# VISION-SJTU/UniDefense

Hardware: AMD Instinct MI355X
Metric: images/sec fwd+bwd (256x256, EffNet-b4) (higher is better)
Workload: dtype f32

## Files before the change

unidefense_amd/csrc/bnref.h:

```cpp
#pragma once
#include "colgeom.h"

namespace {

constexpr int NT = UD_COL_NT;

template <typename T> constexpr int kRowUnroll = sizeof(T) == 2 ? 8 : 4;

__device__ __forceinline__ void atomic_add_f64(double* p, double v) { unsafeAtomicAdd(p, v); }

struct Bn4 { f32x4 mu, is, ga, be; };

__device__ __forceinline__ Bn4 bn_load(const ud_bn_ref& b, int g, int C4, int c4, bool update) {
    Bn4 o;
    const long i0 = ((long)(b.G == 1 ? 0 : g) * C4 + c4) * 4;
#pragma unroll
    for (int e = 0; e < 4; ++e) {
        double m, v;
        ud_bn_moments(b, i0 + e, c4 * 4 + e, m, v);
        o.mu[e] = (float)m;
        o.is[e] = rsqrtf((float)(v + (double)b.eps));
        if (update && b.sum && b.running_mean) {
            const int c = c4 * 4 + e;
            b.running_mean[c] = (1.f - b.momentum) * b.running_mean[c] + b.momentum * (float)m;
            b.running_var[c] = (1.f - b.momentum) * b.running_var[c] + b.momentum * (float)(v * b.unbias);
        }
    }
    o.ga = reinterpret_cast<const f32x4*>(b.gamma)[c4];
    o.be = reinterpret_cast<const f32x4*>(b.beta)[c4];
    return o;
}

__device__ __forceinline__ f32x4 bn_apply(const f32x4& a, const Bn4& b, int act) {
    f32x4 o;
#pragma unroll
    for (int e = 0; e < 4; ++e) o[e] = ud_act_fast(b.ga[e] * ((a[e] - b.mu[e]) * b.is[e]) + b.be[e], act);
    return o;
}

__device__ __forceinline__ float gate_factor(const float* alpha, int mode) {
    if (mode == 0 || !alpha) return 1.f;
    const float a = ud_sigmoid(alpha[0]);
    return mode == 1 ? a : 1.f - a;
}

__global__ __launch_bounds__(NT) void partials_to_acc(int nq, int G, int C, int P, const double* __restrict__ part,
                                                      double* __restrict__ a1, double* __restrict__ a2) {
    __shared__ double sm[2][NT];
    const int cl = threadIdx.x & 7, pl = threadIdx.x >> 3;
    const int idx = blockIdx.x * 8 + cl;
    const bool ok = idx < G * C;
    const long plane = (long)G * P * C;
    double a = 0.0, b = 0.0;
    if (ok) {
        const int g = idx / C, c = idx % C;
        const long base = (long)g * P * C + c, step = 32L * C;
        int p = pl;
        for (; p + 96 < P; p += 128) {
            const long o = base + (long)p * C;
            a += (part[o] + part[o + step]) + (part[o + 2 * step] + part[o + 3 * step]);
            if (nq == 2) b += (part[plane + o] + part[plane + o + step]) + (part[plane + o + 2 * step] + part[plane + o + 3 * step]);
        }
        for (; p < P; p += 32) {
            const long o = base + (long)p * C;
            a += part[o];
            if (nq == 2) b += part[plane + o];
        }
    }
    sm[0][threadIdx.x] = a;
    sm[1][threadIdx.x] = b;
    __syncthreads();
    if (ok && pl == 0) {
        for (int k = 1; k < 32; ++k) {
            a += sm[0][k * 8 + cl];
            b += sm[1][k * 8 + cl];
        }
        a1[idx] += a;
        if (nq == 2) a2[idx] += b;
    }
}

}
```

unidefense_amd/csrc/fft.hip:

```cpp
#include "ud_common.h"

#include <stdlib.h>

#include <type_traits>

namespace {

constexpr int NT = 512;

__device__ __forceinline__ float gate_factor_f(const float* alpha, int mode) {
    if (mode == 0 || !alpha) return 1.f;
    const float a = ud_sigmoid(alpha[0]);
    return mode == 1 ? a : 1.f - a;
}

__device__ constexpr float TW_RE[32] = {
    1.000000000e+00f, 9.951847267e-01f, 9.807852804e-01f, 9.569403357e-01f, 9.238795325e-01f, 8.819212643e-01f,
    8.314696123e-01f, 7.730104534e-01f, 7.071067812e-01f, 6.343932842e-01f, 5.555702330e-01f, 4.713967368e-01f,
    3.826834324e-01f, 2.902846773e-01f, 1.950903220e-01f, 9.801714033e-02f, 0.0f, -9.801714033e-02f,
    -1.950903220e-01f, -2.902846773e-01f, -3.826834324e-01f, -4.713967368e-01f, -5.555702330e-01f, -6.343932842e-01f,
    -7.071067812e-01f, -7.730104534e-01f, -8.314696123e-01f, -8.819212643e-01f, -9.238795325e-01f, -9.569403357e-01f,
    -9.807852804e-01f, -9.951847267e-01f};
__device__ constexpr float TW_IM[32] = {
    0.0f, -9.801714033e-02f, -1.950903220e-01f, -2.902846773e-01f, -3.826834324e-01f, -4.713967368e-01f,
    -5.555702330e-01f, -6.343932842e-01f, -7.071067812e-01f, -7.730104534e-01f, -8.314696123e-01f, -8.819212643e-01f,
    -9.238795325e-01f, -9.569403357e-01f, -9.807852804e-01f, -9.951847267e-01f, -1.000000000e+00f, -9.951847267e-01f,
    -9.807852804e-01f, -9.569403357e-01f, -9.238795325e-01f, -8.819212643e-01f, -8.314696123e-01f, -7.730104534e-01f,
    -7.071067812e-01f, -6.343932842e-01f, -5.555702330e-01f, -4.713967368e-01f, -3.826834324e-01f, -2.902846773e-01f,
    -1.950903220e-01f, -9.801714033e-02f};

template <int S>
__device__ __forceinline__ constexpr int brev2(int i) {
    int r = 0;
    for (int b = 1; b < S; b <<= 1) {
        r = (r << 1) | (i & 1);
        i >>= 1;
    }
    return r;
}

__device__ constexpr float TW80_RE[80] = {
    1.000000000e+00f, 9.969173337e-01f, 9.876883406e-01f, 9.723699204e-01f, 9.510565163e-01f, 9.238795325e-01f,
    8.910065242e-01f, 8.526401644e-01f, 8.090169944e-01f, 7.604059656e-01f, 7.071067812e-01f, 6.494480483e-01f,
    5.877852523e-01f, 5.224985647e-01f, 4.539904997e-01f, 3.826834324e-01f, 3.090169944e-01f, 2.334453639e-01f,
    1.564344650e-01f, 7.845909573e-02f, 6.123233996e-17f, -7.845909573e-02f, -1.564344650e-01f, -2.334453639e-01f,
    -3.090169944e-01f, -3.826834324e-01f, -4.539904997e-01f, -5.224985647e-01f, -5.877852523e-01f, -6.494480483e-01f,
    -7.071067812e-01f, -7.604059656e-01f, -8.090169944e-01f, -8.526401644e-01f, -8.910065242e-01f, -9.238795325e-01f,
    -9.510565163e-01f, -9.723699204e-01f, -9.876883406e-01f, -9.969173337e-01f, -1.000000000e+00f, -9.969173337e-01f,
    -9.876883406e-01f, -9.723699204e-01f, -9.510565163e-01f, -9.238795325e-01f, -8.910065242e-01f, -8.526401644e-01f,
    -8.090169944e-01f, -7.604059656e-01f, -7.071067812e-01f, -6.494480483e-01f, -5.877852523e-01f, -5.224985647e-01f,
    -4.539904997e-01f, -3.826834324e-01f, -3.090169944e-01f, -2.334453639e-01f, -1.564344650e-01f, -7.845909573e-02f,
    -1.836970199e-16f, 7.845909573e-02f, 1.564344650e-01f, 2.334453639e-01f, 3.090169944e-01f, 3.826834324e-01f,
    4.539904997e-01f, 5.224985647e-01f, 5.877852523e-01f, 6.494480483e-01f, 7.071067812e-01f, 7.604059656e-01f,
    8.090169944e-01f, 8.526401644e-01f, 8.910065242e-01f, 9.238795325e-01f, 9.510565163e-01f, 9.723699204e-01f,
    9.876883406e-01f, 9.969173337e-01f};
__device__ constexpr float TW80_IM[80] = {
    -0.000000000e+00f, -7.845909573e-02f, -1.564344650e-01f, -2.334453639e-01f, -3.090169944e-01f, -3.826834324e-01f,
    -4.539904997e-01f, -5.224985647e-01f, -5.877852523e-01f, -6.494480483e-01f, -7.071067812e-01f, -7.604059656e-01f,
    -8.090169944e-01f, -8.526401644e-01f, -8.910065242e-01f, -9.238795325e-01f, -9.510565163e-01f, -9.723699204e-01f,
    -9.876883406e-01f, -9.969173337e-01f, -1.000000000e+00f, -9.969173337e-01f, -9.876883406e-01f, -9.723699204e-01f,
    -9.510565163e-01f, -9.238795325e-01f, -8.910065242e-01f, -8.526401644e-01f, -8.090169944e-01f, -7.604059656e-01f,
    -7.071067812e-01f, -6.494480483e-01f, -5.877852523e-01f, -5.224985647e-01f, -4.539904997e-01f, -3.826834324e-01f,
    -3.090169944e-01f, -2.334453639e-01f, -1.564344650e-01f, -7.845909573e-02f, -1.224646799e-16f, 7.845909573e-02f,
    1.564344650e-01f, 2.334453639e-01f, 3.090169944e-01f, 3.826834324e-01f, 4.539904997e-01f, 5.224985647e-01f,
    5.877852523e-01f, 6.494480483e-01f, 7.071067812e-01f, 7.604059656e-01f, 8.090169944e-01f, 8.526401644e-01f,
    8.910065242e-01f, 9.238795325e-01f, 9.510565163e-01f, 9.723699204e-01f, 9.876883406e-01f, 9.969173337e-01f,
    1.000000000e+00f, 9.969173337e-01f, 9.876883406e-01f, 9.723699204e-01f, 9.510565163e-01f, 9.238795325e-01f,
    8.910065242e-01f, 8.526401644e-01f, 8.090169944e-01f, 7.604059656e-01f, 7.071067812e-01f, 6.494480483e-01f,
    5.877852523e-01f, 5.224985647e-01f, 4.539904997e-01f, 3.826834324e-01f, 3.090169944e-01f, 2.334453639e-01f,
    1.564344650e-01f, 7.845909573e-02f};

__device__ constexpr float TW48_RE[48] = {
    1.000000000e+00f, 9.914448614e-01f, 9.659258263e-01f, 9.238795325e-01f, 8.660254038e-01f, 7.933533403e-01f,
    7.071067812e-01f, 6.087614290e-01f, 5.000000000e-01f, 3.826834324e-01f, 2.588190451e-01f, 1.305261922e-01f,
    6.123233996e-17f, -1.305261922e-01f, -2.588190451e-01f, -3.826834324e-01f, -5.000000000e-01f, -6.087614290e-01f,
    -7.071067812e-01f, -7.933533403e-01f, -8.660254038e-01f, -9.238795325e-01f, -9.659258263e-01f, -9.914448614e-01f,
    -1.000000000e+00f, -9.914448614e-01f, -9.659258263e-01f, -9.238795325e-01f, -8.660254038e-01f, -7.933533403e-01f,
    -7.071067812e-01f, -6.087614290e-01f, -5.000000000e-01f, -3.826834324e-01f, -2.588190451e-01f, -1.305261922e-01f,
    -1.836970199e-16f, 1.305261922e-01f, 2.588190451e-01f, 3.826834324e-01f, 5.000000000e-01f, 6.087614290e-01f,
    7.071067812e-01f, 7.933533403e-01f, 8.660254038e-01f, 9.238795325e-01f, 9.659258263e-01f, 9.914448614e-01f};
__device__ constexpr float TW48_IM[48] = {
    -0.000000000e+00f, -1.305261922e-01f, -2.588190451e-01f, -3.826834324e-01f, -5.000000000e-01f, -6.087614290e-01f,
    -7.071067812e-01f, -7.933533403e-01f, -8.660254038e-01f, -9.238795325e-01f, -9.659258263e-01f, -9.914448614e-01f,
    -1.000000000e+00f, -9.914448614e-01f, -9.659258263e-01f, -9.238795325e-01f, -8.660254038e-01f, -7.933533403e-01f,
    -7.071067812e-01f, -6.087614290e-01f, -5.000000000e-01f, -3.826834324e-01f, -2.588190451e-01f, -1.305261922e-01f,
    -1.224646799e-16f, 1.305261922e-01f, 2.588190451e-01f, 3.826834324e-01f, 5.000000000e-01f, 6.087614290e-01f,
    7.071067812e-01f, 7.933533403e-01f, 8.660254038e-01f, 9.238795325e-01f, 9.659258263e-01f, 9.914448614e-01f,
    1.000000000e+00f, 9.914448614e-01f, 9.659258263e-01f, 9.238795325e-01f, 8.660254038e-01f, 7.933533403e-01f,
    7.071067812e-01f, 6.087614290e-01f, 5.000000000e-01f, 3.826834324e-01f, 2.588190451e-01f, 1.305261922e-01f};

template <int S>
struct Radix {
    static constexpr int R = (S % 5 == 0) ? 5 : (S % 3 == 0) ? 3 : 1;
    static constexpr bool MIXED = R > 1;
    static constexpr int P = S / R;
    static constexpr int L = R == 5 ? 80 : 48;
};
template <int S> __device__ __forceinline__ constexpr float tw_re(int m) { return Radix<S>::R == 5 ? TW80_RE[m] : TW48_RE[m]; }
template <int S> __device__ __forceinline__ constexpr float tw_im(int m) { return Radix<S>::R == 5 ? TW80_IM[m] : TW48_IM[m]; }

template <int S>
__device__ __forceinline__ constexpr int brev(int i) {
    if (Radix<S>::MIXED) return (i % Radix<S>::R) * Radix<S>::P + brev2<Radix<S>::P>(i / Radix<S>::R);
    return brev2<S>(i);
}

template <int S, int P, int OFF, bool INV>
__device__ __forceinline__ void fft_pow2(float (&re)[S], float (&im)[S]) {
#pragma unroll
    for (int len = 2; len <= P; len <<= 1) {
        const int hl = len >> 1;
        const int tstep = 64 / len;
#pragma unroll
        for (int i = 0; i < P; i += len) {
#pragma unroll
            for (int j = 0; j < hl; ++j) {
                const float wr = TW_RE[j * tstep];
                const float wi = INV ? -TW_IM[j * tstep] : TW_IM[j * tstep];
                const float xr = re[OFF + i + j + hl], xi = im[OFF + i + j + hl];
                const float tr = wr * xr - wi * xi;
                const float ti = wr * xi + wi * xr;
                const float ur = re[OFF + i + j], ui = im[OFF + i + j];
                re[OFF + i + j] = ur + tr;
                im[OFF + i + j] = ui + ti;
                re[OFF + i + j + hl] = ur - tr;
                im[OFF + i + j + hl] = ui - ti;
            }
        }
    }
}

template <int S, int P, int RR, bool INV>
struct SubFfts {
    static __device__ __forceinline__ void run(float (&re)[S], float (&im)[S]) {
        SubFfts<S, P, RR - 1, INV>::run(re, im);
        fft_pow2<S, P, (RR - 1) * P, INV>(re, im);
    }
};
template <int S, int P, bool INV>
struct SubFfts<S, P, 0, INV> {
    static __device__ __forceinline__ void run(float (&)[S], float (&)[S]) {}
};

template <int S, bool INV>
__device__ __forceinline__ void fft_inreg(float (&re)[S], float (&im)[S]) {
    constexpr int P = Radix<S>::P, R = Radix<S>::R, L = Radix<S>::L;
    if constexpr (!Radix<S>::MIXED) {
        fft_pow2<S, P, 0, INV>(re, im);
    } else {
        SubFfts<S, P, R, INV>::run(re, im);
        constexpr int TS = L / S;
#pragma unroll
        for (int k2 = 0; k2 < P; ++k2) {
            float yr[R], yi[R];
#pragma unroll
            for (int r = 0; r < R; ++r) {
                const int m = (r * k2 * TS) % L;
                const float wr = tw_re<S>(m), wi = INV ? -tw_im<S>(m) : tw_im<S>(m);
                const float xr = re[r * P + k2], xi = im[r * P + k2];
                yr[r] = wr * xr - wi * xi;
                yi[r] = wr * xi + wi * xr;
            }
#pragma unroll
            for (int k1 = 0; k1 < R; ++k1) {
                float ar = yr[0], ai = yi[0];
#pragma unroll
                for (int r = 1; r < R; ++r) {
                    const int m = ((L / R) * r * k1) % L;
                    const float wr = tw_re<S>(m), wi = INV ? -tw_im<S>(m) : tw_im<S>(m);
                    ar += wr * yr[r] - wi * yi[r];
                    ai += wr * yi[r] + wi * yr[r];
                }
                re[k1 * P + k2] = ar;
                im[k1 * P + k2] = ai;
            }
        }
    }
}

__device__ __forceinline__ void work_item(int xcd_remap, int& cgroup, int& n) {
    const int ngroups = gridDim.x;
    if (!xcd_remap) {
        cgroup = blockIdx.x;
        n = blockIdx.y;
        return;
    }
    const int W = gridDim.x * gridDim.y, L = blockIdx.y * gridDim.x + blockIdx.x;
    const int q = W >> 3, r = W & 7, xcd = L & 7;
    const int w = (xcd < r ? xcd * (q + 1) : r * (q + 1) + (xcd - r) * q) + (L >> 3);
    cgroup = w % ngroups;
    n = w / ngroups;
}

template <int S, int CB>
struct Lds {
    static constexpr int WH = S / 2 + 1;
    static constexpr int KSTRIDE = S * CB + (CB < 32 ? CB : 0);
    static constexpr int PLANE = WH * KSTRIDE;
    static constexpr size_t BYTES = 2ull * PLANE * sizeof(float);
};

struct PlanesOut {
    uint16_t* buf;
    long panel, plane;
    float* inv_scale;
    float pre;
    const double* energy;
};

struct DwOut {
    const float* wt;
    void* out;
};

template <typename T, int S, int CB, bool EX, int DW = 0>
__global__ __launch_bounds__(NT) void rfft2_kernel(const T* __restrict__ x, T* __restrict__ Y, int C,
                                                   float scale, float w_int, ud_bn_ref bn, int has_bn,
                                                   T* __restrict__ act_out, const float* __restrict__ gate_alpha,
                                                   int gate_mode, const double* __restrict__ gate_acc,
                                                   float* __restrict__ gate_grad, int xcd_remap,
                                                   uint32_t* __restrict__ amax, PlanesOut po, DwOut dwo) {
    using L = Lds<S, CB>;
    static_assert(DW == 0 || (size_t)S * S * CB * sizeof(float) <= L::BYTES, "the activated plane fits the transform's LDS planes");
    __shared__ float po_red[NT / 64];
    const bool po_raw = po.pre < 0.f;
    if (EX && po.buf && !po_raw) {
        float gm = 0.f;
        for (int i = threadIdx.x; i < C; i += NT) {
            if (po.energy) gm = fmaxf(gm, (float)po.energy[i]);
            else gm = fmaxf(gm, bn.gamma[i] * bn.gamma[i] + bn.beta[i] * bn.beta[i]);
        }
        gm = ud_wave_max(gm);
        if ((threadIdx.x & 63) == 0) po_red[threadIdx.x >> 6] = gm;
    }
    if (EX && gate_grad && blockIdx.x == 0 && blockIdx.y == 0 && threadIdx.x < 64) {
        const double tot = ud_wave_sum_d(gate_acc[threadIdx.x]);
        if (threadIdx.x == 0) {
            const double a = 1.0 / (1.0 + exp(-(double)gate_alpha[0]));
            gate_grad[0] = (float)(tot * a * (1.0 - a));
        }
    }
    extern __shared__ __attribute__((aligned(16))) float lds[];
    float* Lre = lds;
    float* Lim = lds + L::PLANE;
    const int t = threadIdx.x;
    const int c = t % CB, q = t / CB;
    int cgroup, n;
    work_item(xcd_remap, cgroup, n);
    const int ch = cgroup * CB + c;
    const bool cok = ch < C;
    float re[S], im[S];
    float va[DW ? S : 1];
    if (q < S) {
        const int chl = cok ? ch : C - 1;
        const T* src = x + (((long)n * S + q) * S) * C + chl;
#pragma unroll
        for (int w = 0; w < S; ++w) re[brev<S>(w)] = (float)src[(long)w * C];
        float mu = 0.f, is = 1.f, ga = 1.f, be = 0.f;
        if (EX && has_bn) {
            double m, vv;
            ud_bn_moments(bn, chl, chl, m, vv);
            mu = (float)m;
            is = (float)(1.0 / sqrt(vv + (double)bn.eps));
            ga = bn.gamma[chl];
            be = bn.beta[chl];
            if (n == 0 && q == 0 && cok && bn.sum && bn.running_mean) {
                bn.running_mean[ch] = (1.f - bn.momentum) * bn.running_mean[ch] + bn.momentum * (float)m;
                bn.running_var[ch] = (1.f - bn.momentum) * bn.running_var[ch] + bn.momentum * (float)(vv * bn.unbias);
            }
        }
        T* aout = (EX && act_out) ? act_out + (((long)n * S + q) * S) * C + ch : nullptr;
#pragma unroll
        for (int w = 0; w < S; ++w) {
            float v = re[brev<S>(w)];
            if (EX && has_bn) {
                v = ud_rounded<T>(ud_act(ga * ((v - mu) * is) + be, bn.act));
                if (aout && cok) aout[(long)w * C] = (T)v;
            }
            re[brev<S>(w)] = cok ? v : 0.f;
            im[brev<S>(w)] = 0.f;
            if (DW) va[w] = cok ? v : 0.f;
        }
        fft_inreg<S, false>(re, im);
#pragma unroll
        for (int kx = 0; kx <= S / 2; ++kx) {
            Lre[kx * L::KSTRIDE + q * CB + c] = re[kx];
            Lim[kx * L::KSTRIDE + q * CB + c] = im[kx];
        }
    }
    __syncthreads();
    float mabs = 0.f;
    if (q <= S / 2 && cok) {
#pragma unroll
        for (int h = 0; h < S; ++h) {
            re[brev<S>(h)] = Lre[q * L::KSTRIDE + h * CB + c];
            im[brev<S>(h)] = Lim[q * L::KSTRIDE + h * CB + c];
        }
        fft_inreg<S, false>(re, im);
        float f = (q == 0 || q == S / 2) ? scale : scale * w_int;
        float gf = 1.f;
        if (EX && gate_mode != 0) {
            const float a = ud_sigmoid(gate_alpha[0]);
            gf = (gate_mode == 1) ? a : 1.f - a;
            f *= gf;
        }
        if (EX && po.buf) {
            float ps = 1.f, pinv = 1.f;
            if (!po_raw) {
                float gm = po_red[0];
#pragma unroll
                for (int i = 1; i < NT / 64; ++i) gm = fmaxf(gm, po_red[i]);
                ud_h2_scale(__float_as_uint(po.pre * gf * sqrtf(gm) * 1.002f), ps, pinv);
            }
            if (blockIdx.x == 0 && blockIdx.y == 0 && q == 0 && c == 0) *po.inv_scale = pinv;
            f *= ps;
            const long row0 = ((long)n * S) * L::WH + q;
            const int cim = C + ch;
            uint16_t* pre_ = po.buf + (long)(ch >> 5) * po.panel + row0 * 32 + (ch & 31);
            uint16_t* pim_ = po.buf + (long)(cim >> 5) * po.panel + row0 * 32 + (cim & 31);
#pragma unroll
            for (int ky = 0; ky < S; ++ky) {
                const long o = (long)ky * L::WH * 32;
                if (po_raw) {
                    pre_[o] = __builtin_bit_cast(uint16_t, (_Float16)(re[ky] * f));
                    pim_[o] = __builtin_bit_cast(uint16_t, (_Float16)(im[ky] * f));
                    continue;
                }
                uint16_t a0, a1, b0, b1;
                ud_split_h2(re[ky] * f, a0, a1);
                ud_split_h2(im[ky] * f, b0, b1);
                pre_[o] = a0;
                pre_[o + po.plane] = a1;
                pim_[o] = b0;
                pim_[o + po.plane] = b1;
            }
        } else {
            T* dst = Y + (((long)n * S) * L::WH + q) * (2L * C) + ch;
#pragma unroll
            for (int ky = 0; ky < S; ++ky) {
                dst[(long)ky * L::WH * 2 * C] = (T)(re[ky] * f);
                dst[(long)ky * L::WH * 2 * C + C] = (T)(im[ky] * f);
                if (EX) mabs = fmaxf(mabs, fmaxf(fabsf(re[ky] * f), fabsf(im[ky] * f)));
            }
        }
    }
    if (EX) ud_absmax_commit(mabs, amax);
    if constexpr (DW != 0) {
        constexpr int P = (DW - 1) / 2;
        __syncthreads();
        float* A = lds;
        if (q < S) {
#pragma unroll
            for (int w = 0; w < S; ++w) A[(q * S + w) * CB + c] = va[w];
        }
        __syncthreads();
        if (q < S && cok) {
            float tp[DW * DW];
#pragma unroll
            for (int i = 0; i < DW * DW; ++i) tp[i] = dwo.wt[(long)i * C + ch];
            float acc[S];
#pragma unroll
            for (int w = 0; w < S; ++w) acc[w] = 0.f;
#pragma unroll
            for (int i = 0; i < DW; ++i) {
                const int ih = q + i - P;
                if (ih < 0 || ih >= S) continue;
                float in[S + DW - 1];
#pragma unroll
                for (int j = 0; j < S + DW - 1; ++j) in[j] = (j >= P && j < S + P) ? A[(ih * S + j - P) * CB + c] : 0.f;
#pragma unroll
                for (int w = 0; w < S; ++w)
#pragma unroll
                    for (int j = 0; j < DW; ++j) acc[w] += in[w + j] * tp[i * DW + j];
            }
            T* o = reinterpret_cast<T*>(dwo.out) + (((long)n * S + q) * S) * C + ch;
#pragma unroll
            for (int w = 0; w < S; ++w) o[(long)w * C] = (T)acc[w];
        }
    }
}

template <typename T, int S, int CB, bool MIX>
__global__ __launch_bounds__(NT) void irfft2_kernel(const T* __restrict__ Y, T* __restrict__ x, int C,
                                                    float scale, float w_int, const T* __restrict__ spat,
                                                    const float* __restrict__ alpha, T* __restrict__ freq_out,
                                                    double* __restrict__ sum, double* __restrict__ sumsq, int xcd_remap) {
    using L = Lds<S, CB>;
    extern __shared__ __attribute__((aligned(16))) float lds[];
    float* Lre = lds;
    float* Lim = lds + L::PLANE;
    const int t = threadIdx.x;
    const int c = t % CB, q = t / CB;
    int cgroup, n;
    work_item(xcd_remap, cgroup, n);
    const int ch = cgroup * CB + c;
    const bool cok = ch < C;
    float re[S], im[S];
    constexpr int NHELP = S - (S / 2 + 1);
    if (q > S / 2 && q < S) {
        const int kx = q - (S / 2 + 1);
        const T* src = Y + (((long)n * S) * L::WH + kx) * (2L * C) + ch + C;
#pragma unroll
        for (int ky = 0; ky < S; ++ky) re[ky] = cok ? (float)src[(long)ky * L::WH * 2 * C] : 0.f;
#pragma unroll
        for (int ky = 0; ky < S; ++ky) Lim[kx * L::KSTRIDE + ky * CB + c] = re[ky];
    } else if (q <= S / 2) {
        const T* src = Y + (((long)n * S) * L::WH + q) * (2L * C) + ch;
#pragma unroll
        for (int ky = 0; ky < S; ++ky) re[brev<S>(ky)] = cok ? (float)src[(long)ky * L::WH * 2 * C] : 0.f;
        if (q >= NHELP) {
#pragma unroll
            for (int ky = 0; ky < S; ++ky) im[brev<S>(ky)] = cok ? (float)src[(long)ky * L::WH * 2 * C + C] : 0.f;
        }
    }
    __syncthreads();
    if (q <= S / 2) {
        const float f = (q == 0 || q == S / 2) ? 1.f : w_int;
        if (q < NHELP) {
#pragma unroll
            for (int ky = 0; ky < S; ++ky) im[brev<S>(ky)] = Lim[q * L::KSTRIDE + ky * CB + c];
        }
#pragma unroll
        for (int k = 0; k < S; ++k) {
            re[k] *= f;
            im[k] *= f;
        }
        fft_inreg<S, true>(re, im);
#pragma unroll
        for (int h = 0; h < S; ++h) {
            Lre[q * L::KSTRIDE + h * CB + c] = re[h];
            Lim[q * L::KSTRIDE + h * CB + c] = im[h];
        }
    }
    __syncthreads();
    double tot1 = 0.0, tot2 = 0.0;
    if (cok && q < S) {
#pragma unroll
        for (int kx = 0; kx <= S / 2; ++kx) {
            const float zr = Lre[kx * L::KSTRIDE + q * CB + c];
            const float zi = Lim[kx * L::KSTRIDE + q * CB + c];
            re[brev<S>(kx)] = zr;
            im[brev<S>(kx)] = (kx == 0 || kx == S / 2) ? 0.f : zi;
            if (kx > 0 && kx < S / 2) {
                re[brev<S>(S - kx)] = zr;
                im[brev<S>(S - kx)] = -zi;
            }
        }
        fft_inreg<S, true>(re, im);
        const long o0 = (((long)n * S + q) * S) * C + ch;
        T* dst = x + o0;
        if (!MIX) {
#pragma unroll
            for (int w = 0; w < S; ++w) dst[(long)w * C] = (T)(re[w] * scale);
        } else {
            const float a = ud_sigmoid(alpha[0]);
            const T* sp = spat + o0;
            T* fo = freq_out + o0;
#pragma unroll
            for (int w = 0; w < S; ++w) {
                const float fr = re[w] * scale, spv = (float)sp[(long)w * C];
                const float y = ud_rounded<T>(spv * (1.f - a) + fr * a);
                fo[(long)w * C] = (T)(fr - spv);
                dst[(long)w * C] = (T)y;
                tot1 += (double)y;
                tot2 += (double)y * (double)y;
            }
        }
    }
    if (MIX && sum) {
        __syncthreads();
        double* red = reinterpret_cast<double*>(lds);
        const bool own = cok && q < S;
        if (own) {
            red[(q * CB + c) * 2] = tot1;
            red[(q * CB + c) * 2 + 1] = tot2;
        }
        __syncthreads();
        if (cok && q == 0) {
            double t1 = 0.0, t2 = 0.0;
            for (int r = 0; r < S; ++r) {
                t1 += red[(r * CB + c) * 2];
                t2 += red[(r * CB + c) * 2 + 1];
            }
            unsafeAtomicAdd(sum + ch, t1);
            unsafeAtomicAdd(sumsq + ch, t2);
        }
    }
}

inline int xcd_remap_on(int run_bytes) {
    return run_bytes < 128;
}

template <int S, int CB, int K>
struct LdsBwd {
    using L = Lds<S, CB>;
    static constexpr size_t PLANES = 2ull * S * S * CB * sizeof(float);
    static constexpr size_t FOLD = (size_t)S * K * K * CB * sizeof(float);
    static constexpr size_t BYTES = L::BYTES > PLANES ? (L::BYTES > FOLD ? L::BYTES : FOLD) : (PLANES > FOLD ? PLANES : FOLD);
};

template <typename T, int S, int CB, int K>
__global__ __launch_bounds__(NT, 4) void irfft2_dwbwd_kernel(const T* __restrict__ Y, int C, float scale, float w_int,
                                                         const T* __restrict__ dd, const T* __restrict__ x,
                                                         ud_bn_ref bn, const float* __restrict__ wt,
                                                         const float* __restrict__ gate_alpha, int gate_mode,
                                                         T* __restrict__ dz, double* __restrict__ s1,
                                                         double* __restrict__ s2, double* __restrict__ s3,
                                                         float* __restrict__ wpart, int xcd_remap) {
    using L = Lds<S, CB>;
    static_assert(S * CB == NT, "one row-thread per (h, c)");
    constexpr int P = (K - 1) / 2;
    extern __shared__ __attribute__((aligned(16))) float lds[];
    float* Lre = lds;
    float* Lim = lds + L::PLANE;
    const int t = threadIdx.x;
    const int c = t % CB, q = t / CB;
    int cgroup, n;
    work_item(xcd_remap, cgroup, n);
    const int ch = cgroup * CB + c;
    const bool cok = ch < C;
    const int chl = cok ? ch : C - 1;
    float re[S], im[S];
    constexpr int NHELP = S - (S / 2 + 1);
    if (q > S / 2) {
        const int kx = q - (S / 2 + 1);
        const T* src = Y + (((long)n * S) * L::WH + kx) * (2L * C) + chl + C;
#pragma unroll
        for (int ky = 0; ky < S; ++ky) re[ky] = cok ? (float)src[(long)ky * L::WH * 2 * C] : 0.f;
#pragma unroll
        for (int ky = 0; ky < S; ++ky) Lim[kx * L::KSTRIDE + ky * CB + c] = re[ky];
    } else {
        const T* src = Y + (((long)n * S) * L::WH + q) * (2L * C) + chl;
#pragma unroll
        for (int ky = 0; ky < S; ++ky) re[brev<S>(ky)] = cok ? (float)src[(long)ky * L::WH * 2 * C] : 0.f;
        if (q >= NHELP) {
#pragma unroll
            for (int ky = 0; ky < S; ++ky) im[brev<S>(ky)] = cok ? (float)src[(long)ky * L::WH * 2 * C + C] : 0.f;
        }
    }
    float ddr[S], er[S];
    {
        const long o = (((long)n * S + q) * S) * C + chl;
#pragma unroll
        for (int w = 0; w < S; ++w) {
            ddr[w] = (float)dd[o + (long)w * C];
            er[w] = (float)x[o + (long)w * C];
        }
    }
    __syncthreads();
    if (q <= S / 2) {
        const float f = (q == 0 || q == S / 2) ? 1.f : w_int;
        if (q < NHELP) {
#pragma unroll
            for (int ky = 0; ky < S; ++ky) im[brev<S>(ky)] = Lim[q * L::KSTRIDE + ky * CB + c];
        }
#pragma unroll
        for (int k = 0; k < S; ++k) {
            re[k] *= f;
            im[k] *= f;
        }
        fft_inreg<S, true>(re, im);
#pragma unroll
        for (int h = 0; h < S; ++h) {
            Lre[q * L::KSTRIDE + h * CB + c] = re[h];
            Lim[q * L::KSTRIDE + h * CB + c] = im[h];
        }
    }
    __syncthreads();
    {
#pragma unroll
        for (int kx = 0; kx <= S / 2; ++kx) {
            const float zr = Lre[kx * L::KSTRIDE + q * CB + c];
            const float zi = Lim[kx * L::KSTRIDE + q * CB + c];
            re[brev<S>(kx)] = zr;
            im[brev<S>(kx)] = (kx == 0 || kx == S / 2) ? 0.f : zi;
            if (kx > 0 && kx < S / 2) {
                re[brev<S>(S - kx)] = zr;
                im[brev<S>(S - kx)] = -zi;
            }
        }
        fft_inreg<S, true>(re, im);
    }
    float mu, is, ga, be;
    {
        double m, vv;
        ud_bn_moments(bn, chl, chl, m, vv);
        mu = (float)m;
        is = (float)(1.0 / sqrt(vv + (double)bn.eps));
        ga = bn.gamma[chl];
        be = bn.beta[chl];
    }
    __syncthreads();
    float* A = lds;
    float* D = lds + S * S * CB;
#pragma unroll
    for (int w = 0; w < S; ++w) {
        A[(q * S + w) * CB + c] = cok ? ud_act(ga * ((er[w] - mu) * is) + be, bn.act) : 0.f;
        D[(q * S + w) * CB + c] = cok ? ddr[w] : 0.f;
    }
    __syncthreads();
    float tp[K * K];
#pragma unroll
    for (int i = 0; i < K * K; ++i) tp[i] = wt[(long)i * C + chl];
    double v1 = 0.0, v2 = 0.0;
    float v3 = 0.f;
    {
        float acc[S];
#pragma unroll
        for (int w = 0; w < S; ++w) acc[w] = 0.f;
#pragma unroll
        for (int i = 0; i < K; ++i) {
            const int ih = q + i - P;
            if (ih < 0 || ih >= S) continue;
            float in[S + K - 1];
#pragma unroll
            for (int j = 0; j < S + K - 1; ++j) in[j] = (j >= P && j < S + P) ? D[(ih * S + j - P) * CB + c] : 0.f;
#pragma unroll
            for (int w = 0; w < S; ++w)
#pragma unroll
                for (int j = 0; j < K; ++j) acc[w] += in[w + j] * tp[K * K - 1 - (i * K + j)];
        }
        const float gs = gate_factor_f(gate_alpha, gate_mode);
        if (cok) {
            T* o = dz + (((long)n * S + q) * S) * C + ch;
#pragma unroll
            for (int w = 0; w < S; ++w) {
                const float xh = (er[w] - mu) * is;
                float d = acc[w] * gs + re[w] * scale;
                if (bn.act) d *= ud_act_grad_fast(ga * xh + be, bn.act);
                d = ud_rounded<T>(d);
                o[(long)w * C] = (T)d;
                v1 += (double)d;
                v2 += (double)d * (double)xh;
                v3 += d * d;
            }
        }
    }
    float accw[K * K];
#pragma unroll
    for (int i = 0; i < K * K; ++i) accw[i] = 0.f;
#pragma unroll
    for (int i = 0; i < K; ++i) {
        const int ih = q + i - P;
        if (ih < 0 || ih >= S) continue;
        float in[S + K - 1];
#pragma unroll
        for (int j = 0; j < S + K - 1; ++j) in[j] = (j >= P && j < S + P) ? A[(ih * S + j - P) * CB + c] : 0.f;
#pragma unroll
        for (int j = 0; j < K; ++j)
#pragma unroll
            for (int w = 0; w < S; ++w) accw[i * K + j] += in[w + j] * ddr[w];
    }
    __syncthreads();
    float* F = lds;
#pragma unroll
    for (int i = 0; i < K * K; ++i) F[(q * K * K + i) * CB + c] = cok ? accw[i] : 0.f;
    __syncthreads();
    for (int i = t; i < K * K * CB; i += NT) {
        const int tap = i / CB, cc = i % CB;
        float sum = 0.f;
#pragma unroll
        for (int r = 0; r < S; ++r) sum += F[(r * K * K + tap) * CB + cc];
        if (cgroup * CB + cc < C) wpart[((long)n * K * K + tap) * C + cgroup * CB + cc] = sum;
    }
    __syncthreads();
    double* red = reinterpret_cast<double*>(lds);
    red[(q * CB + c) * 3] = v1;
    red[(q * CB + c) * 3 + 1] = v2;
    red[(q * CB + c) * 3 + 2] = (double)v3 * 1.0001;
    __syncthreads();
    if (cok && q == 0) {
        double t1 = 0.0, t2 = 0.0, t3 = 0.0;
        for (int r = 0; r < S; ++r) {
            t1 += red[(r * CB + c) * 3];
            t2 += red[(r * CB + c) * 3 + 1];
            t3 += red[(r * CB + c) * 3 + 2];
        }
        unsafeAtomicAdd(s1 + ch, t1);
        unsafeAtomicAdd(s2 + ch, t2);
        if (s3) unsafeAtomicAdd(s3 + ch, t3);
    }
}

template <typename T, int S, int CB, int K>
int launch_irfft2_dwbwd(const T* Y, int N, int C, float scale, float w_int, const T* dd, const T* x,
                        const ud_bn_ref& bn, const float* wt, const float* gate_alpha, int gate_mode, T* dz, double* s1,
                        double* s2, double* s3, float* wpart, hipStream_t s) {
    using LB = LdsBwd<S, CB, K>;
    static bool attr_set = false;
    if (LB::BYTES > 65536 && !attr_set) {
        hipError_t e = hipFuncSetAttribute(reinterpret_cast<const void*>(&irfft2_dwbwd_kernel<T, S, CB, K>),
                                           hipFuncAttributeMaxDynamicSharedMemorySize, (int)LB::BYTES);
        if (e != hipSuccess) return -(int)e;
        attr_set = true;
    }
    dim3 grid((unsigned)ud_cdiv(C, CB), (unsigned)N);
    hipLaunchKernelGGL((irfft2_dwbwd_kernel<T, S, CB, K>), grid, dim3(NT), LB::BYTES, s, Y, C, scale, w_int, dd, x, bn, wt,
                       gate_alpha, gate_mode, dz, s1, s2, s3, wpart, xcd_remap_on(CB * (int)sizeof(float)));
    UD_LAUNCH_CHECK();
    return 0;
}

struct RfftEx {
    const ud_bn_ref* bn;
    void* act_out;
    const float* gate_alpha;
    int gate_mode;
    const double* gate_acc;
    float* gate_grad;
    uint32_t* absmax;
    PlanesOut planes = PlanesOut{nullptr, 0, 0, nullptr, 0.f, nullptr};
    DwOut dw = DwOut{nullptr, nullptr};
};

template <typename T, int S, int CB, bool EX, int DW = 0>
int launch_rfft2_t(const T* x, T* Y, int N, int C, float scale, float w_int, const RfftEx& ex, hipStream_t s) {
    using L = Lds<S, CB>;
    static bool attr_set = false;
    if (L::BYTES > 65536 && !attr_set) {
        hipError_t e = hipFuncSetAttribute(reinterpret_cast<const void*>(&rfft2_kernel<T, S, CB, EX, DW>),
                                           hipFuncAttributeMaxDynamicSharedMemorySize, (int)L::BYTES);
        if (e != hipSuccess) return -(int)e;
        attr_set = true;
    }
    dim3 grid((unsigned)ud_cdiv(C, CB), (unsigned)N);
    ud_bn_ref none{};
    hipLaunchKernelGGL((rfft2_kernel<T, S, CB, EX, DW>), grid, dim3(NT), L::BYTES, s, x, Y, C, scale, w_int,
                       ex.bn ? *ex.bn : none, ex.bn ? 1 : 0, (T*)ex.act_out, ex.gate_alpha, ex.gate_mode, ex.gate_acc,
                       ex.gate_grad, xcd_remap_on(CB * (int)sizeof(T)), ex.absmax, ex.planes, ex.dw);
    UD_LAUNCH_CHECK();
    return 0;
}

template <typename T, int S, int CB>
int launch_rfft2(const T* x, T* Y, int N, int C, float scale, float w_int, const RfftEx* ex, hipStream_t s) {
    if (ex) return launch_rfft2_t<T, S, CB, true>(x, Y, N, C, scale, w_int, *ex, s);
    return launch_rfft2_t<T, S, CB, false>(x, Y, N, C, scale, w_int, RfftEx{nullptr, nullptr, nullptr, 0, nullptr, nullptr, nullptr, PlanesOut{nullptr, 0, 0, nullptr, 0.f, nullptr}, DwOut{nullptr, nullptr}}, s);
}

struct IrfftMix {
    const void* spat;
    const float* alpha;
    void* freq_out;
    double* sum;
    double* sumsq;
};

template <typename T, int S, int CB, bool MIX>
int launch_irfft2_t(const T* Y, T* x, int N, int C, float scale, float w_int, const IrfftMix& m, hipStream_t s) {
    using L = Lds<S, CB>;
    static_assert(!MIX || L::BYTES >= (size_t)S * CB * 2 * sizeof(double), "LDS planes hold the row totals");
    static bool attr_set = false;
    if (L::BYTES > 65536 && !attr_set) {
        hipError_t e = hipFuncSetAttribute(reinterpret_cast<const void*>(&irfft2_kernel<T, S, CB, MIX>),
                                           hipFuncAttributeMaxDynamicSharedMemorySize, (int)L::BYTES);
        if (e != hipSuccess) return -(int)e;
        attr_set = true;
    }
    dim3 grid((unsigned)ud_cdiv(C, CB), (unsigned)N);
    hipLaunchKernelGGL((irfft2_kernel<T, S, CB, MIX>), grid, dim3(NT), L::BYTES, s, Y, x, C, scale, w_int,
                       (const T*)m.spat, m.alpha, (T*)m.freq_out, m.sum, m.sumsq, xcd_remap_on(CB * (int)sizeof(T)));
    UD_LAUNCH_CHECK();
    return 0;
}

template <typename T, int S, int CB>
int launch_irfft2(const T* Y, T* x, int N, int C, float scale, float w_int, const IrfftMix* m, hipStream_t s) {
    if (m) return launch_irfft2_t<T, S, CB, true>(Y, x, N, C, scale, w_int, *m, s);
    return launch_irfft2_t<T, S, CB, false>(Y, x, N, C, scale, w_int, IrfftMix{nullptr, nullptr, nullptr, nullptr, nullptr}, s);
}

constexpr int NT2 = 256;
constexpr int RPT = 4;

template <typename T, int S, bool EX>
__global__ __launch_bounds__(NT2) void rows_fwd_kernel(const T* __restrict__ x, float* __restrict__ Z, int C, ud_bn_ref bn,
                                                       int has_bn, T* __restrict__ act_out,
                                                       const float* __restrict__ gate_alpha,
                                                       const double* __restrict__ gate_acc, float* __restrict__ gate_grad) {
    constexpr int WH = S / 2 + 1;
    if (EX && gate_grad && blockIdx.x == 0 && blockIdx.y == 0 && blockIdx.z == 0 && threadIdx.x < 64) {
        const double tot = ud_wave_sum_d(gate_acc[threadIdx.x]);
        if (threadIdx.x == 0) {
            const double a = 1.0 / (1.0 + exp(-(double)gate_alpha[0]));
            gate_grad[0] = (float)(tot * a * (1.0 - a));
        }
    }
    const int ch = blockIdx.x * 64 + (threadIdx.x & 63);
    const int h = blockIdx.y * 4 + (threadIdx.x >> 6);
    const int n = blockIdx.z;
    if (ch >= C || h >= S) return;
    float mu = 0.f, is = 1.f, ga = 1.f, be = 0.f;
    if (EX && has_bn) {
        double m, vv;
        ud_bn_moments(bn, ch, ch, m, vv);
        mu = (float)m;
        is = (float)(1.0 / sqrt(vv + (double)bn.eps));
        ga = bn.gamma[ch];
        be = bn.beta[ch];
        if (n == 0 && h == 0 && bn.sum && bn.running_mean) {
            bn.running_mean[ch] = (1.f - bn.momentum) * bn.running_mean[ch] + bn.momentum * (float)m;
            bn.running_var[ch] = (1.f - bn.momentum) * bn.running_var[ch] + bn.momentum * (float)(vv * bn.unbias);
        }
    }
    const long o0 = (((long)n * S + h) * S) * C + ch;
    const T* src = x + o0;
    T* aout = (EX && act_out) ? act_out + o0 : nullptr;
    float re[S], im[S];
#pragma unroll
    for (int w = 0; w < S; ++w) re[brev<S>(w)] = (float)src[(long)w * C];
#pragma unroll
    for (int w = 0; w < S; ++w) {
        if (EX && has_bn) {
            const float v = ud_rounded<T>(ud_act(ga * ((re[brev<S>(w)] - mu) * is) + be, bn.act));
            if (aout) aout[(long)w * C] = (T)v;
            re[brev<S>(w)] = v;
        }
        im[brev<S>(w)] = 0.f;
    }
    fft_inreg<S, false>(re, im);
    float* dst = Z + (((long)n * S + h) * WH) * (2L * C) + ch;
#pragma unroll
    for (int kx = 0; kx <= S / 2; ++kx) {
        dst[(long)kx * 2 * C] = re[kx];
        dst[(long)kx * 2 * C + C] = im[kx];
    }
}

template <typename T, int S, bool EX>
__global__ __launch_bounds__(NT2) void cols_fwd_kernel(const float* __restrict__ Z, T* __restrict__ Y, int C, float scale,
                                                       float w_int, const float* __restrict__ gate_alpha, int gate_mode,
                                                       uint32_t* __restrict__ amax) {
    constexpr int WH = S / 2 + 1;
    const int ch = blockIdx.x * 64 + (threadIdx.x & 63);
    const int kx = blockIdx.y * 4 + (threadIdx.x >> 6);
    const int n = blockIdx.z;
    if (ch >= C || kx >= WH) {
        ud_absmax_commit(0.f, amax);
        return;
    }
    float mabs = 0.f;
    const float* src = Z + (((long)n * S) * WH + kx) * (2L * C) + ch;
    float re[S], im[S];
#pragma unroll
    for (int h = 0; h < S; ++h) {
        re[brev<S>(h)] = src[(long)h * WH * 2 * C];
        im[brev<S>(h)] = src[(long)h * WH * 2 * C + C];
    }
    fft_inreg<S, false>(re, im);
    float f = (kx == 0 || kx == S / 2) ? scale : scale * w_int;
    if (EX && gate_mode != 0) {
        const float a = ud_sigmoid(gate_alpha[0]);
        f *= (gate_mode == 1) ? a : 1.f - a;
    }
    T* dst = Y + (((long)n * S) * WH + kx) * (2L * C) + ch;
#pragma unroll
    for (int ky = 0; ky < S; ++ky) {
        dst[(long)ky * WH * 2 * C] = (T)(re[ky] * f);
        dst[(long)ky * WH * 2 * C + C] = (T)(im[ky] * f);
        mabs = fmaxf(mabs, fmaxf(fabsf(re[ky] * f), fabsf(im[ky] * f)));
    }
    ud_absmax_commit(mabs, amax);
}

template <typename T, int S>
__global__ __launch_bounds__(NT2) void cols_inv_kernel(const T* __restrict__ Y, float* __restrict__ Z, int C, float w_int) {
    constexpr int WH = S / 2 + 1;
    const int ch = blockIdx.x * 64 + (threadIdx.x & 63);
    const int kx = blockIdx.y * 4 + (threadIdx.x >> 6);
    const int n = blockIdx.z;
    if (ch >= C || kx >= WH) return;
    const T* src = Y + (((long)n * S) * WH + kx) * (2L * C) + ch;
    const float f = (kx == 0 || kx == S / 2) ? 1.f : w_int;
    float re[S], im[S];
#pragma unroll
    for (int ky = 0; ky < S; ++ky) {
        re[brev<S>(ky)] = (float)src[(long)ky * WH * 2 * C];
        im[brev<S>(ky)] = (float)src[(long)ky * WH * 2 * C + C];
    }
#pragma unroll
    for (int k = 0; k < S; ++k) {
        re[k] *= f;
        im[k] *= f;
    }
    fft_inreg<S, true>(re, im);
    float* dst = Z + (((long)n * S) * WH + kx) * (2L * C) + ch;
#pragma unroll
    for (int h = 0; h < S; ++h) {
        dst[(long)h * WH * 2 * C] = re[h];
        dst[(long)h * WH * 2 * C + C] = im[h];
    }
}

template <typename T, int S, bool MIX>
__global__ __launch_bounds__(NT2) void rows_inv_kernel(const float* __restrict__ Z, T* __restrict__ x, int C, float scale,
                                                       const T* __restrict__ spat, const float* __restrict__ alpha,
                                                       T* __restrict__ freq_out, double* __restrict__ sum,
                                                       double* __restrict__ sumsq) {
    constexpr int WH = S / 2 + 1;
    __shared__ double red[MIX ? 2 * NT2 : 1];
    const int lane = threadIdx.x & 63, rg = threadIdx.x >> 6;
    const int ch = blockIdx.x * 64 + lane;
    const int n = blockIdx.z;
    const bool cok = ch < C;
    double tot1 = 0.0, tot2 = 0.0;
    float a = 0.f;
    if (MIX) a = ud_sigmoid(alpha[0]);
    if (cok) {
#pragma unroll 1
        for (int r = 0; r < RPT; ++r) {
            const int h = (blockIdx.y * 4 + rg) * RPT + r;
            if (h >= S) break;
            const float* src = Z + (((long)n * S + h) * WH) * (2L * C) + ch;
            float re[S], im[S];
#pragma unroll
            for (int kx = 0; kx <= S / 2; ++kx) {
                const float zr = src[(long)kx * 2 * C];
                const float zi = src[(long)kx * 2 * C + C];
                re[brev<S>(kx)] = zr;
                im[brev<S>(kx)] = (kx == 0 || kx == S / 2) ? 0.f : zi;
                if (kx > 0 && kx < S / 2) {
                    re[brev<S>(S - kx)] = zr;
                    im[brev<S>(S - kx)] = -zi;
                }
            }
            fft_inreg<S, true>(re, im);
            const long o0 = (((long)n * S + h) * S) * C + ch;
            T* dst = x + o0;
            if (!MIX) {
#pragma unroll
                for (int w = 0; w < S; ++w) dst[(long)w * C] = (T)(re[w] * scale);
            } else {
                const T* sp = spat + o0;
                T* fo = freq_out + o0;
#pragma unroll
                for (int w = 0; w < S; ++w) {
                    const float fr = re[w] * scale, spv = (float)sp[(long)w * C];
                    const float y = ud_rounded<T>(spv * (1.f - a) + fr * a);
                    fo[(long)w * C] = (T)(fr - spv);
                    dst[(long)w * C] = (T)y;
                    tot1 += (double)y;
                    tot2 += (double)y * (double)y;
                }
            }
        }
    }
    if (MIX && sum) {
        red[threadIdx.x * 2] = tot1;
        red[threadIdx.x * 2 + 1] = tot2;
        __syncthreads();
        if (rg == 0 && cok) {
            double t1 = 0.0, t2 = 0.0;
#pragma unroll
            for (int g = 0; g < 4; ++g) {
                t1 += red[(g * 64 + lane) * 2];
                t2 += red[(g * 64 + lane) * 2 + 1];
            }
            unsafeAtomicAdd(sum + ch, t1);
            unsafeAtomicAdd(sumsq + ch, t2);
        }
    }
}

template <typename T, int S>
int rfft2_two_pass(const T* x, T* Y, float* Z, int N, int C, float scale, float w_int, const RfftEx* ex, hipStream_t s) {
    constexpr int WH = S / 2 + 1;
    const dim3 gr((unsigned)ud_cdiv(C, 64), (unsigned)(S / 4), (unsigned)N);
    const dim3 gc((unsigned)ud_cdiv(C, 64), (unsigned)ud_cdiv(WH, 4), (unsigned)N);
    ud_bn_ref none{};
    if (ex) {
        hipLaunchKernelGGL((rows_fwd_kernel<T, S, true>), gr, dim3(NT2), 0, s, x, Z, C, ex->bn ? *ex->bn : none,
                           ex->bn ? 1 : 0, (T*)ex->act_out, ex->gate_alpha, ex->gate_acc, ex->gate_grad);
        hipLaunchKernelGGL((cols_fwd_kernel<T, S, true>), gc, dim3(NT2), 0, s, Z, Y, C, scale, w_int, ex->gate_alpha,
                           ex->gate_mode, ex->absmax);
    } else {
        hipLaunchKernelGGL((rows_fwd_kernel<T, S, false>), gr, dim3(NT2), 0, s, x, Z, C, none, 0, (T*)nullptr,
                           (const float*)nullptr, (const double*)nullptr, (float*)nullptr);
        hipLaunchKernelGGL((cols_fwd_kernel<T, S, false>), gc, dim3(NT2), 0, s, Z, Y, C, scale, w_int,
                           (const float*)nullptr, 0, (uint32_t*)nullptr);
    }
    UD_LAUNCH_CHECK();
    return 0;
}

template <typename T, int S>
int irfft2_two_pass(const T* Y, T* x, float* Z, int N, int C, float scale, float w_int, const IrfftMix* m, hipStream_t s) {
    constexpr int WH = S / 2 + 1;
    const dim3 gc((unsigned)ud_cdiv(C, 64), (unsigned)ud_cdiv(WH, 4), (unsigned)N);
    const dim3 gr((unsigned)ud_cdiv(C, 64), (unsigned)ud_cdiv(S, 4 * RPT), (unsigned)N);
    hipLaunchKernelGGL((cols_inv_kernel<T, S>), gc, dim3(NT2), 0, s, Y, Z, C, w_int);
    if (m)
        hipLaunchKernelGGL((rows_inv_kernel<T, S, true>), gr, dim3(NT2), 0, s, Z, x, C, scale, (const T*)m->spat, m->alpha,
                           (T*)m->freq_out, m->sum, m->sumsq);
    else
        hipLaunchKernelGGL((rows_inv_kernel<T, S, false>), gr, dim3(NT2), 0, s, Z, x, C, scale, (const T*)nullptr,
                           (const float*)nullptr, (T*)nullptr, (double*)nullptr, (double*)nullptr);
    UD_LAUNCH_CHECK();
    return 0;
}

constexpr int NTW = 1024;
constexpr int CBW = 32;
struct LdsW {
    static constexpr int KSTRIDE = 32 * CBW;
    static constexpr int PLANE = 17 * KSTRIDE;
    static constexpr size_t BYTES = 2ull * PLANE * sizeof(float);
};

template <bool INV>
__device__ __forceinline__ void fft32_pair(float (&re)[16], float (&im)[16], int hh) {
    fft_inreg<16, INV>(re, im);
#pragma unroll
    for (int k = 0; k < 16; ++k) {
        const float wr = TW_RE[2 * k], wi = INV ? -TW_IM[2 * k] : TW_IM[2 * k];
        const float tr = wr * re[k] - wi * im[k], ti = wr * im[k] + wi * re[k];
        const float ar = hh ? tr : re[k], ai = hh ? ti : im[k];
        const float br = __shfl_xor(ar, 32, 64), bi = __shfl_xor(ai, 32, 64);
        re[k] = hh ? br - ar : ar + br;
        im[k] = hh ? bi - ai : ai + bi;
    }
}

template <typename T, bool EX>
__global__ __launch_bounds__(NTW) void rfft2_wave_kernel(const T* __restrict__ x, T* __restrict__ Y, int C, float scale,
                                                         float w_int, ud_bn_ref bn, int has_bn, T* __restrict__ act_out,
                                                         const float* __restrict__ gate_alpha, int gate_mode,
                                                         const double* __restrict__ gate_acc, float* __restrict__ gate_grad,
                                                         uint32_t* __restrict__ amax) {
    constexpr int S = 32, WH = 17;
    using L = LdsW;
    if (EX && gate_grad && blockIdx.x == 0 && blockIdx.y == 0 && threadIdx.x < 64) {
        const double tot = ud_wave_sum_d(gate_acc[threadIdx.x]);
        if (threadIdx.x == 0) {
            const double a = 1.0 / (1.0 + exp(-(double)gate_alpha[0]));
            gate_grad[0] = (float)(tot * a * (1.0 - a));
        }
    }
    extern __shared__ __attribute__((aligned(16))) float lds[];
    float* Lre = lds;
    float* Lim = lds + L::PLANE;
    const int lane = threadIdx.x & 63, wave = threadIdx.x >> 6;
    const int c = lane & 31, hh = lane >> 5;
    const int n = blockIdx.y;
    const int ch = blockIdx.x * CBW + c;
    const bool cok = ch < C;
    const int chl = cok ? ch : C - 1;
    float re[16], im[16];
    float v[2][16];
#pragma unroll
    for (int it = 0; it < 2; ++it) {
        const T* src = x + (((long)n * S + wave + 16 * it) * S + hh) * C + chl;
#pragma unroll
        for (int j = 0; j < 16; ++j) v[it][j] = (float)src[(long)(2 * j) * C];
    }
    float mu = 0.f, is = 1.f, ga = 1.f, be = 0.f;
    if (EX && has_bn) {
        double m, vv;
        ud_bn_moments(bn, chl, chl, m, vv);
        mu = (float)m;
        is = (float)(1.0 / sqrt(vv + (double)bn.eps));
        ga = bn.gamma[chl];
        be = bn.beta[chl];
        if (n == 0 && wave == 0 && hh == 0 && cok && bn.sum && bn.running_mean) {
            bn.running_mean[ch] = (1.f - bn.momentum) * bn.running_mean[ch] + bn.momentum * (float)m;
            bn.running_var[ch] = (1.f - bn.momentum) * bn.running_var[ch] + bn.momentum * (float)(vv * bn.unbias);
        }
    }
#pragma unroll
    for (int it = 0; it < 2; ++it) {
        const int q = wave + 16 * it;
        T* aout = (EX && act_out) ? act_out + (((long)n * S + q) * S + hh) * C + ch : nullptr;
#pragma unroll
        for (int j = 0; j < 16; ++j) {
            float u = v[it][j];
            if (EX && has_bn) {
                u = ud_rounded<T>(ud_act(ga * ((u - mu) * is) + be, bn.act));
                if (aout && cok) {
                    *aout = (T)u;
                    aout += 2L * C;
                }
            }
            re[brev<16>(j)] = cok ? u : 0.f;
            im[brev<16>(j)] = 0.f;
        }
        fft32_pair<false>(re, im, hh);
#pragma unroll
        for (int k = 0; k < 16; ++k) {
            if (hh == 0 || k == 0) {
                Lre[(k + 16 * hh) * L::KSTRIDE + q * CBW + c] = re[k];
                Lim[(k + 16 * hh) * L::KSTRIDE + q * CBW + c] = im[k];
            }
        }
    }
    __syncthreads();
    float mabs = 0.f;
    float gf = 1.f;
    if (EX && gate_mode != 0) {
        const float a = ud_sigmoid(gate_alpha[0]);
        gf = (gate_mode == 1) ? a : 1.f - a;
    }
#pragma unroll 1
    for (int kx = wave; kx < WH; kx += 16) {
#pragma unroll
        for (int j = 0; j < 16; ++j) {
            re[brev<16>(j)] = Lre[kx * L::KSTRIDE + (2 * j + hh) * CBW + c];
            im[brev<16>(j)] = Lim[kx * L::KSTRIDE + (2 * j + hh) * CBW + c];
        }
        fft32_pair<false>(re, im, hh);
        const float f = ((kx == 0 || kx == S / 2) ? scale : scale * w_int) * gf;
        if (cok) {
            T* dst = Y + (((long)n * S + 16 * hh) * WH + kx) * (2L * C) + ch;
#pragma unroll
            for (int k = 0; k < 16; ++k) {
                dst[0] = (T)(re[k] * f);
                dst[C] = (T)(im[k] * f);
                dst += (long)WH * 2 * C;
                if (EX) mabs = fmaxf(mabs, fmaxf(fabsf(re[k] * f), fabsf(im[k] * f)));
            }
        }
    }
    if (EX) ud_absmax_commit(mabs, amax);
}

template <typename T, bool MIX>
__global__ __launch_bounds__(NTW) void irfft2_wave_kernel(const T* __restrict__ Y, T* __restrict__ x, int C, float scale,
                                                          float w_int, const T* __restrict__ spat,
                                                          const float* __restrict__ alpha, T* __restrict__ freq_out,
                                                          double* __restrict__ sum, double* __restrict__ sumsq) {
    constexpr int S = 32, WH = 17;
    using L = LdsW;
    extern __shared__ __attribute__((aligned(16))) float lds[];
    float* Lre = lds;
    float* Lim = lds + L::PLANE;
    const int lane = threadIdx.x & 63, wave = threadIdx.x >> 6;
    const int c = lane & 31, hh = lane >> 5;
    const int n = blockIdx.y;
    const int ch = blockIdx.x * CBW + c;
    const bool cok = ch < C;
    const int chl = cok ? ch : C - 1;
    float re[16], im[16];
#pragma unroll 1
    for (int kx = wave; kx < WH; kx += 16) {
        const T* src = Y + (((long)n * S + hh) * WH + kx) * (2L * C) + chl;
        const float f = (kx == 0 || kx == S / 2) ? 1.f : w_int;
#pragma unroll
        for (int j = 0; j < 16; ++j) {
            re[brev<16>(j)] = (float)src[(long)(2 * j) * WH * 2 * C];
            im[brev<16>(j)] = (float)src[(long)(2 * j) * WH * 2 * C + C];
        }
#pragma unroll
        for (int k = 0; k < 16; ++k) {
            re[k] = cok ? re[k] * f : 0.f;
            im[k] = cok ? im[k] * f : 0.f;
        }
        fft32_pair<true>(re, im, hh);
#pragma unroll
        for (int k = 0; k < 16; ++k) {
            Lre[kx * L::KSTRIDE + (k + 16 * hh) * CBW + c] = re[k];
            Lim[kx * L::KSTRIDE + (k + 16 * hh) * CBW + c] = im[k];
        }
    }
    __syncthreads();
    double tot1 = 0.0, tot2 = 0.0;
    float a = 0.f;
    if (MIX) a = ud_sigmoid(alpha[0]);
#pragma unroll 1
    for (int h = wave; h < S; h += 16) {
#pragma unroll
        for (int j = 0; j < 16; ++j) {
            const int kx = 2 * j + hh;
            const int kk = kx <= S / 2 ? kx : S - kx;
            const float zr = Lre[kk * L::KSTRIDE + h * CBW + c];
            float zi = Lim[kk * L::KSTRIDE + h * CBW + c];
            zi = (kk == 0 || kk == S / 2) ? 0.f : (kx <= S / 2 ? zi : -zi);
            re[brev<16>(j)] = zr;
            im[brev<16>(j)] = zi;
        }
        fft32_pair<true>(re, im, hh);
        if (cok) {
            const long plane = (long)n * S * S * C;
            unsigned o = (unsigned)((h * S + 16 * hh) * C + ch);
            T* dst = x + plane;
            if (!MIX) {
#pragma unroll
                for (int k = 0; k < 16; ++k) dst[o + (unsigned)(k * C)] = (T)(re[k] * scale);
            } else {
                const T* sp = spat + plane;
                T* fo = freq_out + plane;
#pragma unroll
                for (int k = 0; k < 16; ++k) {
                    const unsigned ok = o + (unsigned)(k * C);
                    const float fr = re[k] * scale, spv = (float)sp[ok];
                    const float y = ud_rounded<T>(spv * (1.f - a) + fr * a);
                    fo[ok] = (T)(fr - spv);
                    dst[ok] = (T)y;
                    tot1 += (double)y;
                    tot2 += (double)y * (double)y;
                }
            }
        }
    }
    if (MIX && sum) {
        tot1 += __shfl_xor(tot1, 32, 64);
        tot2 += __shfl_xor(tot2, 32, 64);
        __syncthreads();
        double* red = reinterpret_cast<double*>(lds);
        if (hh == 0) {
            red[(wave * CBW + c) * 2] = tot1;
            red[(wave * CBW + c) * 2 + 1] = tot2;
        }
        __syncthreads();
        if (wave == 0 && hh == 0 && cok) {
            double t1 = 0.0, t2 = 0.0;
            for (int r = 0; r < 16; ++r) {
                t1 += red[(r * CBW + c) * 2];
                t2 += red[(r * CBW + c) * 2 + 1];
            }
            unsafeAtomicAdd(sum + ch, t1);
            unsafeAtomicAdd(sumsq + ch, t2);
        }
    }
}

template <typename K>
int wave_lds_attr(K kernel) {
    hipError_t e = hipFuncSetAttribute(reinterpret_cast<const void*>(kernel), hipFuncAttributeMaxDynamicSharedMemorySize,
                                       (int)LdsW::BYTES);
    return e == hipSuccess ? 0 : -(int)e;
}

template <typename T, bool EX>
int launch_rfft2_wave_t(const T* x, T* Y, int N, int C, float scale, float w_int, const RfftEx& ex, hipStream_t s) {
    static int attr = wave_lds_attr(&rfft2_wave_kernel<T, EX>);
    if (attr) return attr;
    dim3 grid((unsigned)ud_cdiv(C, CBW), (unsigned)N);
    ud_bn_ref none{};
    hipLaunchKernelGGL((rfft2_wave_kernel<T, EX>), grid, dim3(NTW), LdsW::BYTES, s, x, Y, C, scale, w_int, ex.bn ? *ex.bn : none,
                       ex.bn ? 1 : 0, (T*)ex.act_out, ex.gate_alpha, ex.gate_mode, ex.gate_acc, ex.gate_grad, ex.absmax);
    UD_LAUNCH_CHECK();
    return 0;
}
template <typename T>
int launch_rfft2_wave(const T* x, T* Y, int N, int C, float scale, float w_int, const RfftEx* ex, hipStream_t s) {
    if (ex) return launch_rfft2_wave_t<T, true>(x, Y, N, C, scale, w_int, *ex, s);
    return launch_rfft2_wave_t<T, false>(x, Y, N, C, scale, w_int, RfftEx{nullptr, nullptr, nullptr, 0, nullptr, nullptr, nullptr, PlanesOut{nullptr, 0, 0, nullptr, 0.f, nullptr}, DwOut{nullptr, nullptr}}, s);
}
template <typename T, bool MIX>
int launch_irfft2_wave_t(const T* Y, T* x, int N, int C, float scale, float w_int, const IrfftMix& m, hipStream_t s) {
    static int attr = wave_lds_attr(&irfft2_wave_kernel<T, MIX>);
    if (attr) return attr;
    dim3 grid((unsigned)ud_cdiv(C, CBW), (unsigned)N);
    hipLaunchKernelGGL((irfft2_wave_kernel<T, MIX>), grid, dim3(NTW), LdsW::BYTES, s, Y, x, C, scale, w_int, (const T*)m.spat,
                       m.alpha, (T*)m.freq_out, m.sum, m.sumsq);
    UD_LAUNCH_CHECK();
    return 0;
}
template <typename T>
int launch_irfft2_wave(const T* Y, T* x, int N, int C, float scale, float w_int, const IrfftMix* m, hipStream_t s) {
    if (m) return launch_irfft2_wave_t<T, true>(Y, x, N, C, scale, w_int, *m, s);
    return launch_irfft2_wave_t<T, false>(Y, x, N, C, scale, w_int, IrfftMix{nullptr, nullptr, nullptr, nullptr, nullptr}, s);
}

int g_fft32_wave = [] {
    const char* e = getenv("UD_FFT32_WAVE");
    return (e && (e[0] == '0' || e[0] == '1')) ? e[0] - '0' : -1;
}();
inline bool fft32_wave_on(int N, int C) {
    if (g_fft32_wave >= 0) return g_fft32_wave != 0;
    return C % CBW == 0 && (long)N * (C / CBW) <= 256;
}

template <typename T>
int rfft2_dispatch(const T* x, T* Y, int N, int S, int C, float scale, float w_interior, const RfftEx* ex,
                   hipStream_t s) {
    switch (S) {
        case 8: return launch_rfft2<T, 8, 64>(x, Y, N, C, scale, w_interior, ex, s);
        case 16: return launch_rfft2<T, 16, 32>(x, Y, N, C, scale, w_interior, ex, s);
        case 32:
            if (fft32_wave_on(N, C) && !(ex && ex->planes.buf)) return launch_rfft2_wave<T>(x, Y, N, C, scale, w_interior, ex, s);
            return launch_rfft2<T, 32, 16>(x, Y, N, C, scale, w_interior, ex, s);
        case 64: return launch_rfft2<T, 64, 8>(x, Y, N, C, scale, w_interior, ex, s);
        case 12: return launch_rfft2<T, 12, 42>(x, Y, N, C, scale, w_interior, ex, s);
        case 24: return launch_rfft2<T, 24, 21>(x, Y, N, C, scale, w_interior, ex, s);
        case 48: return launch_rfft2<T, 48, 10>(x, Y, N, C, scale, w_interior, ex, s);
        default: break;
    }
    if constexpr (std::is_same<T, float>::value) {
        switch (S) {
            case 10: return launch_rfft2<T, 10, 51>(x, Y, N, C, scale, w_interior, ex, s);
            case 20: return launch_rfft2<T, 20, 25>(x, Y, N, C, scale, w_interior, ex, s);
            case 40: return launch_rfft2<T, 40, 12>(x, Y, N, C, scale, w_interior, ex, s);
            case 80: return launch_rfft2<T, 80, 5>(x, Y, N, C, scale, w_interior, ex, s);
            default: break;
        }
    }
    return UD_EINVAL;
}

template <typename T>
int irfft2_dispatch(const T* Y, T* x, int N, int S, int C, float scale, float w_interior, const IrfftMix* m,
                    hipStream_t s) {
    switch (S) {
        case 8: return launch_irfft2<T, 8, 64>(Y, x, N, C, scale, w_interior, m, s);
        case 16: return launch_irfft2<T, 16, 32>(Y, x, N, C, scale, w_interior, m, s);
        case 32:
            if (fft32_wave_on(N, C)) return launch_irfft2_wave<T>(Y, x, N, C, scale, w_interior, m, s);
            return launch_irfft2<T, 32, 16>(Y, x, N, C, scale, w_interior, m, s);
        case 64: return launch_irfft2<T, 64, 8>(Y, x, N, C, scale, w_interior, m, s);
        case 12: return launch_irfft2<T, 12, 42>(Y, x, N, C, scale, w_interior, m, s);
        case 24: return launch_irfft2<T, 24, 21>(Y, x, N, C, scale, w_interior, m, s);
        case 48: return launch_irfft2<T, 48, 10>(Y, x, N, C, scale, w_interior, m, s);
        default: break;
    }
    if constexpr (std::is_same<T, float>::value) {
        switch (S) {
            case 10: return launch_irfft2<T, 10, 51>(Y, x, N, C, scale, w_interior, m, s);
            case 20: return launch_irfft2<T, 20, 25>(Y, x, N, C, scale, w_interior, m, s);
            case 40: return launch_irfft2<T, 40, 12>(Y, x, N, C, scale, w_interior, m, s);
            case 80: return launch_irfft2<T, 80, 5>(Y, x, N, C, scale, w_interior, m, s);
            default: break;
        }
    }
    return UD_EINVAL;
}

}

extern "C" {

int ud_fft32_set_wave(int mode) {
    const int prev = g_fft32_wave < 0 ? 0 : g_fft32_wave == 0 ? 1 : 2;
    if (mode < 0 || mode > 2) return UD_EINVAL;
    g_fft32_wave = mode - 1 < 0 ? -1 : mode - 1;
    return prev;
}

int ud_rfft2(const void* x, void* Y, int N, int S, int C, float scale, float w_interior, int f16, ud_stream_t stream) {
    if (N < 1 || C < 1) return UD_EINVAL;
    UD_STORAGE_DISPATCH(f16, return rfft2_dispatch<T>((const T*)x, (T*)Y, N, S, C, scale, w_interior, nullptr,
                                                      (hipStream_t)stream));
}

int ud_irfft2(const void* Y, void* x, int N, int S, int C, float scale, float w_interior, int f16, ud_stream_t stream) {
    if (N < 1 || C < 1) return UD_EINVAL;
    UD_STORAGE_DISPATCH(f16, return irfft2_dispatch<T>((const T*)Y, (T*)x, N, S, C, scale, w_interior, nullptr,
                                                       (hipStream_t)stream));
}

int ud_rfft2_ex(const void* x, void* Y, int N, int S, int C, float scale, float w_interior, const ud_bn_ref* bn,
                void* act_out, const float* gate_alpha, int gate_mode, const double* gate_acc, float* gate_grad,
                int f16, uint32_t* absmax, ud_stream_t stream) {
    if (N < 1 || C < 1 || !x || !Y) return UD_EINVAL;
    if (gate_mode < 0 || gate_mode > 2 || (gate_mode != 0 && !gate_alpha)) return UD_EINVAL;
    if (bn && bn->G != 1) return UD_EINVAL;
    if (act_out && !bn) return UD_EINVAL;
    if (gate_grad && (!gate_acc || !gate_alpha)) return UD_EINVAL;
    RfftEx ex{bn, act_out, gate_alpha, gate_mode, gate_acc, gate_grad, absmax};
    UD_STORAGE_DISPATCH(f16, return rfft2_dispatch<T>((const T*)x, (T*)Y, N, S, C, scale, w_interior, &ex,
                                                      (hipStream_t)stream));
}

int ud_rfft2_ex_planes(const void* x, uint16_t* planes, long panel_stride, long plane_stride, float* inv_scale, float bound_pre,
                       const double* energy, int N, int S, int C, float scale, float w_interior, const ud_bn_ref* bn,
                       void* act_out, const float* gate_alpha, int gate_mode, const double* gate_acc, float* gate_grad,
                       const float* dw_wt, void* dw_out, int dw_k, ud_stream_t stream) {
    if (dw_k != 0 && (!dw_wt || !dw_out || (dw_k != 3 && dw_k != 5) || (S != 8 && S != 16 && S != 32))) return UD_EINVAL;
    if (N < 1 || C < 4 || (2 * C) % 32 || !x || !planes || !inv_scale || !(bound_pre > 0.f)) return UD_EINVAL;
    if (S != 8 && S != 16 && S != 32 && S != 12 && S != 24 && S != 48) return UD_EINVAL;
    if (gate_mode < 0 || gate_mode > 2 || (gate_mode != 0 && !gate_alpha)) return UD_EINVAL;
    if (bn && bn->G != 1) return UD_EINVAL;
    if (!bn && !energy) return UD_EINVAL;
    if (act_out && !bn) return UD_EINVAL;
    if (gate_grad && (!gate_acc || !gate_alpha)) return UD_EINVAL;
    const long rows = (long)N * S * (S / 2 + 1);
    if (panel_stride < rows * 32 || panel_stride % 8 || plane_stride % 8 || plane_stride < (long)(2 * C / 32) * panel_stride)
        return UD_EINVAL;
    RfftEx ex{bn, act_out, gate_alpha, gate_mode, gate_acc, gate_grad, nullptr,
              PlanesOut{planes, panel_stride, plane_stride, inv_scale, bound_pre, energy}, DwOut{dw_wt, dw_out}};
    hipStream_t st = (hipStream_t)stream;
    const float* xf = (const float*)x;
    if (dw_k == 3) {
        if (S == 8) return launch_rfft2_t<float, 8, 64, true, 3>(xf, nullptr, N, C, scale, w_interior, ex, st);
        if (S == 16) return launch_rfft2_t<float, 16, 32, true, 3>(xf, nullptr, N, C, scale, w_interior, ex, st);
        return launch_rfft2_t<float, 32, 16, true, 3>(xf, nullptr, N, C, scale, w_interior, ex, st);
    }
    if (dw_k == 5) {
        if (S == 8) return launch_rfft2_t<float, 8, 64, true, 5>(xf, nullptr, N, C, scale, w_interior, ex, st);
        if (S == 16) return launch_rfft2_t<float, 16, 32, true, 5>(xf, nullptr, N, C, scale, w_interior, ex, st);
        return launch_rfft2_t<float, 32, 16, true, 5>(xf, nullptr, N, C, scale, w_interior, ex, st);
    }
    return rfft2_dispatch<float>(xf, (float*)nullptr, N, S, C, scale, w_interior, &ex, st);
}

int ud_rfft2_ex_plane_half(const void* x, uint16_t* plane, long panel_stride, float* inv_scale, int N, int S, int C, float scale,
                           float w_interior, const ud_bn_ref* bn, void* act_out, const float* gate_alpha, int gate_mode,
                           const double* gate_acc, float* gate_grad, const float* dw_wt, void* dw_out, int dw_k,
                           ud_stream_t stream) {
    if (dw_k != 0 && (!dw_wt || !dw_out || (dw_k != 3 && dw_k != 5) || (S != 8 && S != 16 && S != 32))) return UD_EINVAL;
    if (N < 1 || C < 4 || (2 * C) % 32 || !x || !plane || !inv_scale) return UD_EINVAL;
    if (S != 8 && S != 16 && S != 32 && S != 12 && S != 24 && S != 48) return UD_EINVAL;
    if (gate_mode < 0 || gate_mode > 2 || (gate_mode != 0 && !gate_alpha)) return UD_EINVAL;
    if (bn && bn->G != 1) return UD_EINVAL;
    if (act_out && !bn) return UD_EINVAL;
    if (gate_grad && (!gate_acc || !gate_alpha)) return UD_EINVAL;
    const long rows = (long)N * S * (S / 2 + 1);
    if (panel_stride < rows * 32 || panel_stride % 8) return UD_EINVAL;
    RfftEx ex{bn, act_out, gate_alpha, gate_mode, gate_acc, gate_grad, nullptr,
              PlanesOut{plane, panel_stride, 0, inv_scale, -1.f, nullptr}, DwOut{dw_wt, dw_out}};
    hipStream_t st = (hipStream_t)stream;
    const _Float16* xh = (const _Float16*)x;
    if (dw_k == 3) {
        if (S == 8) return launch_rfft2_t<_Float16, 8, 64, true, 3>(xh, nullptr, N, C, scale, w_interior, ex, st);
        if (S == 16) return launch_rfft2_t<_Float16, 16, 32, true, 3>(xh, nullptr, N, C, scale, w_interior, ex, st);
        return launch_rfft2_t<_Float16, 32, 16, true, 3>(xh, nullptr, N, C, scale, w_interior, ex, st);
    }
    if (dw_k == 5) {
        if (S == 8) return launch_rfft2_t<_Float16, 8, 64, true, 5>(xh, nullptr, N, C, scale, w_interior, ex, st);
        if (S == 16) return launch_rfft2_t<_Float16, 16, 32, true, 5>(xh, nullptr, N, C, scale, w_interior, ex, st);
        return launch_rfft2_t<_Float16, 32, 16, true, 5>(xh, nullptr, N, C, scale, w_interior, ex, st);
    }
    return rfft2_dispatch<_Float16>(xh, (_Float16*)nullptr, N, S, C, scale, w_interior, &ex, st);
}

int ud_irfft2_dwbwd(const void* Y, int N, int S, int C, float scale, float w_interior, const void* dd, const void* x,
                    const ud_bn_ref* bn, const float* wt, int K, const float* gate_alpha, int gate_mode, void* dz, double* s1,
                    double* s2, double* s3, float* wpart, int f16, ud_stream_t stream) {
    if (ud_bn_eval_form(bn)) return UD_EINVAL;
    if (N < 1 || C < 1 || !Y || !dd || !x || !bn || bn->G != 1 || !wt || !dz || !s1 || !s2 || !wpart) return UD_EINVAL;
    if (gate_mode < 0 || gate_mode > 2 || (gate_mode != 0 && !gate_alpha)) return UD_EINVAL;
    hipStream_t st = (hipStream_t)stream;
#define UD_IDW(SS, CC, KK)                                                                                                       \
    UD_STORAGE_DISPATCH(f16, return (launch_irfft2_dwbwd<T, SS, CC, KK>((const T*)Y, N, C, scale, w_interior, (const T*)dd,     \
                                                                        (const T*)x, *bn, wt, gate_alpha, gate_mode, (T*)dz, s1, \
                                                                        s2, s3, wpart, st)))
    if (S == 8 && K == 5) UD_IDW(8, 64, 5);
    if (S == 8 && K == 3) UD_IDW(8, 64, 3);
    if (S == 16 && K == 5) UD_IDW(16, 32, 5);
    if (S == 16 && K == 3) UD_IDW(16, 32, 3);
#undef UD_IDW
    return UD_EINVAL;
}

int ud_irfft2_mix(const void* Y, void* y, int N, int S, int C, float scale, float w_interior, const void* spat,
                  const float* alpha, void* freq_out, double* sum, double* sumsq, int f16, ud_stream_t stream) {
    if (N < 1 || C < 1 || !Y || !y || !spat || !alpha || !freq_out || !sum != !sumsq) return UD_EINVAL;
    IrfftMix m{spat, alpha, freq_out, sum, sumsq};
    UD_STORAGE_DISPATCH(f16, return irfft2_dispatch<T>((const T*)Y, (T*)y, N, S, C, scale, w_interior, &m,
                                                       (hipStream_t)stream));
}

long ud_fft2_two_pass_ws_floats(int N, int S, int C) {
    if (N < 1 || C < 1 || (S != 32 && S != 64)) return 0;
    return (long)N * S * (S / 2 + 1) * 2 * C;
}

int ud_rfft2_two_pass(const void* x, void* Y, float* ws, int N, int S, int C, float scale, float w_interior,
                      const ud_bn_ref* bn, void* act_out, const float* gate_alpha, int gate_mode, const double* gate_acc,
                      float* gate_grad, int f16, uint32_t* absmax, ud_stream_t stream) {
    if (N < 1 || C < 1 || !x || !Y || !ws || (S != 32 && S != 64)) return UD_EINVAL;
    if (gate_mode < 0 || gate_mode > 2 || (gate_mode != 0 && !gate_alpha)) return UD_EINVAL;
    if (bn && bn->G != 1) return UD_EINVAL;
    if (act_out && !bn) return UD_EINVAL;
    if (gate_grad && (!gate_acc || !gate_alpha)) return UD_EINVAL;
    RfftEx exv{bn, act_out, gate_alpha, gate_mode, gate_acc, gate_grad, absmax};
    const RfftEx* ex = (bn || gate_mode != 0 || gate_grad || absmax) ? &exv : nullptr;
    hipStream_t s = (hipStream_t)stream;
    UD_STORAGE_DISPATCH(f16, if (S == 64) return rfft2_two_pass<T, 64>((const T*)x, (T*)Y, ws, N, C, scale, w_interior, ex, s);
                        return rfft2_two_pass<T, 32>((const T*)x, (T*)Y, ws, N, C, scale, w_interior, ex, s));
}

int ud_irfft2_two_pass(const void* Y, void* y, float* ws, int N, int S, int C, float scale, float w_interior,
                       const void* spat, const float* alpha, void* freq_out, double* sum, double* sumsq, int f16,
                       ud_stream_t stream) {
    if (N < 1 || C < 1 || !Y || !y || !ws || (S != 32 && S != 64)) return UD_EINVAL;
    if (spat && (!alpha || !freq_out || !sum != !sumsq)) return UD_EINVAL;
    IrfftMix mv{spat, alpha, freq_out, sum, sumsq};
    const IrfftMix* m = spat ? &mv : nullptr;
    hipStream_t s = (hipStream_t)stream;
    UD_STORAGE_DISPATCH(f16, if (S == 64) return irfft2_two_pass<T, 64>((const T*)Y, (T*)y, ws, N, C, scale, w_interior, m, s);
                        return irfft2_two_pass<T, 32>((const T*)Y, (T*)y, ws, N, C, scale, w_interior, m, s));
}

}
```

unidefense_amd/csrc/fused.hip:

```cpp
#include "bnref.h"

namespace {

struct Rows {
    int r, r_end;
    long idx, step;
};
__device__ __forceinline__ Rows rows_of(const RedGeom& q, int ri, int c4) {
    Rows w;
    const int g = blockIdx.z, p = blockIdx.x;
    const int r_begin = p * q.rows_per_chunk;
    w.r_end = r_begin + q.rows_per_chunk;
    if (w.r_end > q.R) w.r_end = q.R;
    w.step = (long)q.rpi * q.C4;
    w.r = r_begin + ri;
    w.idx = (long)g * q.R * q.C4 + (long)w.r * q.C4 + c4;
    return w;
}

__device__ __forceinline__ bool is_updater(int ri) { return blockIdx.x == 0 && blockIdx.z == 0 && ri == 0; }

template <int NQ>
__device__ __forceinline__ void red_out(const RedGeom& q, int ri, bool active, int c4, double (&v)[8], double* a1,
                                        double* a2, double* part, bool per_group) {
    block_fold<NQ>(q, ri, active, v);
    if (!(active && ri == 0)) return;
    if (part) {
        const long o = (((long)blockIdx.z * q.P + blockIdx.x) * q.C4 + c4) * 4;
        const long plane = (long)q.G * q.P * q.C4 * 4;
#pragma unroll
        for (int e = 0; e < 4; ++e) {
            part[o + e] = v[e];
            if (NQ == 8) part[plane + o + e] = v[4 + e];
        }
    } else {
        const long o = ((long)(per_group ? blockIdx.z : 0) * q.C4 + c4) * 4;
#pragma unroll
        for (int e = 0; e < 4; ++e) {
            atomic_add_f64(a1 + o + e, v[e]);
            if (NQ == 8) atomic_add_f64(a2 + o + e, v[4 + e]);
        }
    }
}

template <typename T>
__global__ __launch_bounds__(NT) void colstats_kernel(RedGeom q, const T* __restrict__ x, double* __restrict__ sum,
                                                      double* __restrict__ sumsq, double* __restrict__ part) {
    int ri, c4;
    const bool active = thread_coords(q, ri, c4);
    const In4<T> x4{x};
    double v[8] = {0, 0, 0, 0, 0, 0, 0, 0};
    if (active) {
        Rows w = rows_of(q, ri, c4);
        for (; w.r + 3 * q.rpi < w.r_end; w.r += 4 * q.rpi, w.idx += 4 * w.step) {
            f32x4 a0 = x4[w.idx], a1 = x4[w.idx + w.step], a2 = x4[w.idx + 2 * w.step], a3 = x4[w.idx + 3 * w.step];
#pragma unroll
            for (int e = 0; e < 4; ++e) {
                const double d0 = a0[e], d1 = a1[e], d2 = a2[e], d3 = a3[e];
                v[e] += (d0 + d1) + (d2 + d3);
                v[4 + e] += (d0 * d0 + d1 * d1) + (d2 * d2 + d3 * d3);
            }
        }
        for (; w.r < w.r_end; w.r += q.rpi, w.idx += w.step) {
            f32x4 a = x4[w.idx];
#pragma unroll
            for (int e = 0; e < 4; ++e) {
                const double d = a[e];
                v[e] += d;
                v[4 + e] += d * d;
            }
        }
    }
    red_out<8>(q, ri, active, c4, v, sum, sumsq, part, true);
}

template <typename T, bool DOT>
__global__ __launch_bounds__(NT) void colsum_bn_kernel(RedGeom q, const T* __restrict__ x,
                                                       const T* __restrict__ dy, ud_bn_ref bn,
                                                       double* __restrict__ out, double* __restrict__ part,
                                                       uint32_t* __restrict__ amax) {
    int ri, c4;
    const bool active = thread_coords(q, ri, c4);
    const In4<T> x4{x}, d4{dy};
    double v[8] = {0, 0, 0, 0, 0, 0, 0, 0};
    float mo = 0.f;
    if (active) {
        const Bn4 cb = bn_load(bn, blockIdx.z, q.C4, c4, !DOT && is_updater(ri));
        Rows w = rows_of(q, ri, c4);
#pragma unroll kRowUnroll<T>
        for (; w.r < w.r_end; w.r += q.rpi, w.idx += w.step) {
            f32x4 a = bn_apply(x4[w.idx], cb, bn.act);
            if (DOT) {
                f32x4 d = d4[w.idx];
#pragma unroll
                for (int e = 0; e < 4; ++e) v[e] += (double)d[e] * (double)a[e];
            } else {
#pragma unroll
                for (int e = 0; e < 4; ++e) v[e] += (double)a[e];
                mo = fmaxf(mo, fmaxf(fmaxf(fabsf(a[0]), fabsf(a[1])), fmaxf(fabsf(a[2]), fabsf(a[3]))));
            }
        }
    }
    red_out<4>(q, ri, active, c4, v, out, nullptr, part, true);
    if (!DOT) ud_absmax_commit(mo, amax);
}

__global__ __launch_bounds__(NT) void fc_fwd_d_kernel(const double* __restrict__ xsum, float xscale,
                                                      const float* __restrict__ W, const float* __restrict__ b,
                                                      float* __restrict__ y, int N, int I, int O) {
    const int wave = (blockIdx.x * NT + threadIdx.x) >> 6, lane = threadIdx.x & 63;
    if (wave >= N * O) return;
    const int n = wave / O, o = wave % O;
    float acc = 0.f;
#pragma unroll 4
    for (int i = lane; i < I; i += 64) acc += ((float)xsum[(long)n * I + i] * xscale) * W[(long)o * I + i];
    acc = ud_wave_sum(acc);
    if (lane == 0) y[(long)n * O + o] = acc + (b ? b[o] : 0.f);
}

template <typename T>
__global__ __launch_bounds__(NT) void se_scale_bn_kernel(RedGeom q, const T* __restrict__ x, ud_bn_ref bn,
                                                         const float* __restrict__ s, T* __restrict__ y,
                                                         uint32_t* __restrict__ amax) {
    int ri, c4;
    float m = 0.f;
    if (thread_coords(q, ri, c4)) {
        const In4<T> x4{x};
        const Out4<T> y4{y};
        const Bn4 cb = bn_load(bn, blockIdx.z, q.C4, c4, false);
        f32x4 gate = reinterpret_cast<const f32x4*>(s)[(long)blockIdx.z * q.C4 + c4];
#pragma unroll
        for (int e = 0; e < 4; ++e) gate[e] = ud_sigmoid_fast(gate[e]);
        Rows w = rows_of(q, ri, c4);
#pragma unroll kRowUnroll<T>
        for (; w.r < w.r_end; w.r += q.rpi, w.idx += w.step) {
            const f32x4 v = bn_apply(x4[w.idx], cb, bn.act) * gate;
            y4.st(w.idx, v);
            m = fmaxf(m, fmaxf(fmaxf(fabsf(v[0]), fabsf(v[1])), fmaxf(fabsf(v[2]), fabsf(v[3]))));
        }
    }
    ud_absmax_commit(m, amax);
}

__global__ __launch_bounds__(NT) void se_scale_bn_planes_kernel(RedGeom q, const float* __restrict__ x, ud_bn_ref bn,
                                                                const float* __restrict__ s, uint16_t* __restrict__ planes,
                                                                long panel, long plane, const uint32_t* __restrict__ amax_in,
                                                                float* __restrict__ inv_scale) {
    uint32_t mb = 0;
#pragma unroll
    for (int i = 0; i < 4; ++i) mb = max(mb, amax_in[(threadIdx.x & 63) + 64 * i]);
#pragma unroll
    for (int o = 32; o > 0; o >>= 1) mb = max(mb, (uint32_t)__shfl_xor((int)mb, o, 64));
    float ps, pinv;
    ud_h2_scale(mb, ps, pinv);
    if (blockIdx.x == 0 && blockIdx.y == 0 && blockIdx.z == 0 && threadIdx.x == 0) *inv_scale = pinv;
    int ri, c4;
    if (!thread_coords(q, ri, c4)) return;
    const In4<float> x4{x};
    const Bn4 cb = bn_load(bn, blockIdx.z, q.C4, c4, false);
    f32x4 gate = reinterpret_cast<const f32x4*>(s)[(long)blockIdx.z * q.C4 + c4];
#pragma unroll
    for (int e = 0; e < 4; ++e) gate[e] = ud_sigmoid_fast(gate[e]) * ps;
    Rows w = rows_of(q, ri, c4);
    uint16_t* o = planes + (long)(c4 >> 3) * panel + (c4 & 7) * 4;
    long row = (long)blockIdx.z * q.R + w.r;
#pragma unroll 4
    for (; w.r < w.r_end; w.r += q.rpi, w.idx += w.step, row += q.rpi) {
        const f32x4 v = bn_apply(x4[w.idx], cb, bn.act) * gate;
        uint16_t h0[4], h1[4];
#pragma unroll
        for (int e = 0; e < 4; ++e) ud_split_h2(v[e], h0[e], h1[e]);
        typedef unsigned short u16x4 __attribute__((ext_vector_type(4)));
        *reinterpret_cast<u16x4*>(o + row * 32) = u16x4{h0[0], h0[1], h0[2], h0[3]};
        *reinterpret_cast<u16x4*>(o + row * 32 + plane) = u16x4{h1[0], h1[1], h1[2], h1[3]};
    }
}

__global__ __launch_bounds__(NT) void se_scale_bn_plane_half_kernel(RedGeom q, const _Float16* __restrict__ x, ud_bn_ref bn,
                                                                    const float* __restrict__ s, uint16_t* __restrict__ plane,
                                                                    long panel, float* __restrict__ inv_scale) {
    if (blockIdx.x == 0 && blockIdx.y == 0 && blockIdx.z == 0 && threadIdx.x == 0) *inv_scale = 1.f;
    int ri, c4;
    if (!thread_coords(q, ri, c4)) return;
    typedef unsigned short u16x4 __attribute__((ext_vector_type(4)));
    const In4<_Float16> x4{x};
    const Bn4 cb = bn_load(bn, blockIdx.z, q.C4, c4, false);
    f32x4 gate = reinterpret_cast<const f32x4*>(s)[(long)blockIdx.z * q.C4 + c4];
#pragma unroll
    for (int e = 0; e < 4; ++e) gate[e] = ud_sigmoid_fast(gate[e]);
    Rows w = rows_of(q, ri, c4);
    uint16_t* o = plane + (long)(c4 >> 3) * panel + (c4 & 7) * 4;
    const int npad = (c4 == q.C4 - 1) ? 7 - (c4 & 7) : 0;
    long row = (long)blockIdx.z * q.R + w.r;
#pragma unroll 4
    for (; w.r < w.r_end; w.r += q.rpi, w.idx += w.step, row += q.rpi) {
        const f32x4 v = bn_apply(x4[w.idx], cb, bn.act) * gate;
        Quad<_Float16>::st(reinterpret_cast<_Float16*>(o + row * 32), 0, v);
        for (int z = 1; z <= npad; ++z) *reinterpret_cast<u16x4*>(o + row * 32 + 4 * z) = u16x4{0, 0, 0, 0};
    }
}

struct ResPlanes {
    uint16_t* buf;
    long panel, plane;
    float* inv_scale;
    const uint32_t* skip_amax;
};

template <typename T, int PL = 0>
__global__ __launch_bounds__(NT) void residual_bn_kernel(RedGeom q, const T* __restrict__ x, ud_bn_ref bn,
                                                         const float* __restrict__ keep, float inv_keep,
                                                         const T* __restrict__ skip, T* __restrict__ out,
                                                         uint32_t* __restrict__ amax, ResPlanes rp) {
    float ps = 1.f;
    if constexpr (PL == 1) {
        __shared__ float pl_red[NT / 64];
        const float rc = sqrtf((float)(1.0 / bn.inv_count));
        float gm = 0.f;
        for (int i = threadIdx.x; i < q.C4 * 4; i += NT) gm = fmaxf(gm, fabsf(bn.gamma[i]) * rc + fabsf(bn.beta[i]));
        gm *= keep ? inv_keep : 1.f;
        gm = ud_wave_max(gm);
        if ((threadIdx.x & 63) == 0) pl_red[threadIdx.x >> 6] = gm;
        __syncthreads();
        gm = pl_red[0];
#pragma unroll
        for (int i = 1; i < NT / 64; ++i) gm = fmaxf(gm, pl_red[i]);
        float sk = 0.f;
        if (rp.skip_amax) {
            uint32_t mb = rp.skip_amax[threadIdx.x & 255];
            sk = __uint_as_float(mb);
            sk = ud_wave_max(sk);
            __syncthreads();
            if ((threadIdx.x & 63) == 0) pl_red[threadIdx.x >> 6] = sk;
            __syncthreads();
            sk = pl_red[0];
#pragma unroll
            for (int i = 1; i < NT / 64; ++i) sk = fmaxf(sk, pl_red[i]);
        }
        float pinv;
        ud_h2_scale(__float_as_uint((gm + sk) * 1.001f), ps, pinv);
        if (blockIdx.x == 0 && blockIdx.y == 0 && blockIdx.z == 0 && threadIdx.x == 0) *rp.inv_scale = pinv;
    }
    int ri, c4;
    float m = 0.f;
    if (thread_coords(q, ri, c4)) {
        const In4<T> x4{x}, k4{skip};
        const Out4<T> o4{out};
        const Bn4 cb = bn_load(bn, blockIdx.z, q.C4, c4, is_updater(ri));
        const float sc = keep ? keep[blockIdx.z] * inv_keep : 1.f;
        Rows w = rows_of(q, ri, c4);
        uint16_t* po = PL ? rp.buf + (long)(c4 >> 3) * rp.panel + (c4 & 7) * 4 : nullptr;
        const int npad = (PL && c4 == q.C4 - 1) ? 7 - (c4 & 7) : 0;
        long prow = (long)blockIdx.z * q.R + w.r;
#pragma unroll kRowUnroll<T>
        for (; w.r < w.r_end; w.r += q.rpi, w.idx += w.step, prow += q.rpi) {
            f32x4 v = bn_apply(x4[w.idx], cb, bn.act) * sc;
            if (skip) v += k4[w.idx];
            o4.st(w.idx, v);
            m = fmaxf(m, fmaxf(fmaxf(fabsf(v[0]), fabsf(v[1])), fmaxf(fabsf(v[2]), fabsf(v[3]))));
            if constexpr (PL == 1) {
                typedef unsigned short u16x4 __attribute__((ext_vector_type(4)));
                uint16_t h0[4], h1[4];
#pragma unroll
                for (int e = 0; e < 4; ++e) ud_split_h2(v[e] * ps, h0[e], h1[e]);
                *reinterpret_cast<u16x4*>(po + prow * 32) = u16x4{h0[0], h0[1], h0[2], h0[3]};
                *reinterpret_cast<u16x4*>(po + prow * 32 + rp.plane) = u16x4{h1[0], h1[1], h1[2], h1[3]};
                for (int z = 1; z <= npad; ++z) {
                    *reinterpret_cast<u16x4*>(po + prow * 32 + 4 * z) = u16x4{0, 0, 0, 0};
                    *reinterpret_cast<u16x4*>(po + prow * 32 + 4 * z + rp.plane) = u16x4{0, 0, 0, 0};
                }
            }
        }
    }
    ud_absmax_commit(m, amax);
}

template <typename T>
__global__ __launch_bounds__(NT) void bn_apply_kernel(RedGeom q, const T* __restrict__ x, ud_bn_ref bn,
                                                      T* __restrict__ y) {
    int ri, c4;
    if (!thread_coords(q, ri, c4)) return;
    const In4<T> x4{x};
    const Out4<T> y4{y};
    const Bn4 cb = bn_load(bn, blockIdx.z, q.C4, c4, is_updater(ri));
    Rows w = rows_of(q, ri, c4);
#pragma unroll kRowUnroll<T>
    for (; w.r < w.r_end; w.r += q.rpi, w.idx += w.step) y4.st(w.idx, bn_apply(x4[w.idx], cb, bn.act));
}

__device__ __forceinline__ void dz_terms(const f32x4& a, const f32x4& d, const Bn4& cb, int act, bool is_dz, float sc,
                                         f32x4& dz, f32x4& xh) {
#pragma unroll
    for (int e = 0; e < 4; ++e) {
        xh[e] = (a[e] - cb.mu[e]) * cb.is[e];
        float g = d[e];
        if (!is_dz) {
            g *= sc;
            if (act) g *= ud_act_grad_fast(cb.ga[e] * xh[e] + cb.be[e], act);
        }
        dz[e] = g;
    }
}

template <typename T>
__global__ __launch_bounds__(NT) void normbwd_sums_kernel(RedGeom q, const T* __restrict__ x,
                                                          const T* __restrict__ dy, const float* __restrict__ keep,
                                                          float inv_keep, ud_bn_ref bn, int dy_is_dz,
                                                          double* __restrict__ s1, double* __restrict__ s2,
                                                          double* __restrict__ s3, double* __restrict__ part) {
    int ri, c4;
    const bool active = thread_coords(q, ri, c4);
    const In4<T> x4{x}, d4{dy};
    double v[8] = {0, 0, 0, 0, 0, 0, 0, 0};
    f32x4 en = {0.f, 0.f, 0.f, 0.f};
    if (active) {
        const Bn4 cb = bn_load(bn, blockIdx.z, q.C4, c4, false);
        const float sc = keep ? keep[blockIdx.z] * inv_keep : 1.f;
        Rows w = rows_of(q, ri, c4);
#pragma unroll kRowUnroll<T>
        for (; w.r < w.r_end; w.r += q.rpi, w.idx += w.step) {
            f32x4 dz, xh;
            dz_terms(x4[w.idx], d4[w.idx], cb, bn.act, dy_is_dz != 0, sc, dz, xh);
#pragma unroll
            for (int e = 0; e < 4; ++e) {
                v[e] += (double)dz[e];
                v[4 + e] += (double)dz[e] * (double)xh[e];
            }
            en += dz * dz;
        }
    }
    if (s3) {
        double ev[8] = {(double)en[0] * 1.0001, (double)en[1] * 1.0001, (double)en[2] * 1.0001, (double)en[3] * 1.0001, 0, 0, 0, 0};
        block_fold<4>(q, ri, active, ev);
        if (active && ri == 0) {
#pragma unroll
            for (int e = 0; e < 4; ++e) atomic_add_f64(s3 + (long)c4 * 4 + e, ev[e]);
        }
    }
    red_out<8>(q, ri, active, c4, v, s1, s2, part, false);
}

struct PlanesDst {
    uint16_t* buf;
    long panel, plane;
    float* inv_scale;
    const double* energy;
};

template <typename T, bool MIX, int PL = 0>
__global__ __launch_bounds__(NT) void normbwd_apply_kernel(RedGeom q, const T* __restrict__ x,
                                                           const T* __restrict__ dy, const float* __restrict__ keep,
                                                           float inv_keep, ud_bn_ref bn, int dy_is_dz,
                                                           const double* __restrict__ s1, const double* __restrict__ s2,
                                                           const double* __restrict__ s1l, const double* __restrict__ s2l,
                                                           const T* __restrict__ freq,
                                                           T* __restrict__ dx, double* __restrict__ dalpha_acc,
                                                           float* __restrict__ dgamma, float* __restrict__ dbeta,
                                                           uint32_t* __restrict__ amax, double* __restrict__ energy,
                                                           PlanesDst pd) {
    float ps = 1.f;
    if constexpr (PL == 2) {
        if (blockIdx.x == 0 && blockIdx.y == 0 && blockIdx.z == 0 && threadIdx.x == 0) *pd.inv_scale = 1.f;
    }
    if constexpr (PL == 1) {
        __shared__ float pl_red[NT / 64];
        float gm = 0.f;
        for (int i = threadIdx.x; i < q.C4 * 4; i += NT) {
            const double m = bn.sum[i] * bn.inv_count;
            double vv = bn.sumsq[i] * bn.inv_count - m * m;
            if (vv < 0.0) vv = 0.0;
            const float gi = bn.gamma[i] * rsqrtf((float)(vv + (double)bn.eps));
            gm = fmaxf(gm, gi * gi * (float)pd.energy[i]);
        }
        gm = ud_wave_max(gm);
        if ((threadIdx.x & 63) == 0) pl_red[threadIdx.x >> 6] = gm;
        __syncthreads();
        gm = pl_red[0];
#pragma unroll
        for (int i = 1; i < NT / 64; ++i) gm = fmaxf(gm, pl_red[i]);
        float pinv;
        ud_h2_scale(__float_as_uint(sqrtf(gm) * 1.002f), ps, pinv);
        if (blockIdx.x == 0 && blockIdx.y == 0 && blockIdx.z == 0 && threadIdx.x == 0) *pd.inv_scale = pinv;
    }
    int ri, c4;
    const bool active = thread_coords(q, ri, c4);
    const In4<T> x4{x}, d4{dy}, fr4{freq};
    const Out4<T> o4{dx};
    double acc = 0.0;
    float mo = 0.f;
    f32x4 en = {0.f, 0.f, 0.f, 0.f};
    if (active) {
        const Bn4 cb = bn_load(bn, blockIdx.z, q.C4, c4, false);
        const float sc = keep ? keep[blockIdx.z] * inv_keep : 1.f;
        f32x4 t1, t2;
#pragma unroll
        for (int e = 0; e < 4; ++e) {
            t1[e] = (float)s1[c4 * 4 + e] * (float)bn.inv_count;
            t2[e] = (float)s2[c4 * 4 + e] * (float)bn.inv_count;
        }
        if (is_updater(ri)) {
#pragma unroll
            for (int e = 0; e < 4; ++e) {
                if (dbeta) dbeta[c4 * 4 + e] = (float)s1l[c4 * 4 + e];
                if (dgamma) dgamma[c4 * 4 + e] = (float)s2l[c4 * 4 + e];
            }
        }
        Rows w = rows_of(q, ri, c4);
        uint16_t* po = PL ? pd.buf + (long)(c4 >> 3) * pd.panel + (c4 & 7) * 4 : nullptr;
        const int npad = (PL && c4 == q.C4 - 1) ? 7 - (c4 & 7) : 0;
        long prow = (long)blockIdx.z * q.R + w.r;
#pragma unroll kRowUnroll<T>
        for (; w.r < w.r_end; w.r += q.rpi, w.idx += w.step, prow += q.rpi) {
            f32x4 dz, xh, o;
            dz_terms(x4[w.idx], d4[w.idx], cb, bn.act, dy_is_dz != 0, sc, dz, xh);
#pragma unroll
            for (int e = 0; e < 4; ++e) o[e] = cb.ga[e] * cb.is[e] * (dz[e] - t1[e] - xh[e] * t2[e]);
            if constexpr (PL == 2) {
                typedef unsigned short u16x4 __attribute__((ext_vector_type(4)));
                Quad<T>::st(reinterpret_cast<T*>(po + prow * 32), 0, o);
                for (int z = 1; z <= npad; ++z) *reinterpret_cast<u16x4*>(po + prow * 32 + 4 * z) = u16x4{0, 0, 0, 0};
                continue;
            }
            if constexpr (PL == 1) {
                typedef unsigned short u16x4 __attribute__((ext_vector_type(4)));
                uint16_t h0[4], h1[4];
#pragma unroll
                for (int e = 0; e < 4; ++e) ud_split_h2(o[e] * ps, h0[e], h1[e]);
                *reinterpret_cast<u16x4*>(po + prow * 32) = u16x4{h0[0], h0[1], h0[2], h0[3]};
                *reinterpret_cast<u16x4*>(po + prow * 32 + pd.plane) = u16x4{h1[0], h1[1], h1[2], h1[3]};
                for (int z = 1; z <= npad; ++z) {
                    *reinterpret_cast<u16x4*>(po + prow * 32 + 4 * z) = u16x4{0, 0, 0, 0};
                    *reinterpret_cast<u16x4*>(po + prow * 32 + 4 * z + pd.plane) = u16x4{0, 0, 0, 0};
                }
                continue;
            }
            o4.st(w.idx, o);
            mo = fmaxf(mo, fmaxf(fmaxf(fabsf(o[0]), fabsf(o[1])), fmaxf(fabsf(o[2]), fabsf(o[3]))));
            if (MIX) {
                f32x4 f = fr4[w.idx];
#pragma unroll
                for (int e = 0; e < 4; ++e) acc += (double)ud_rounded<T>(o[e]) * (double)f[e];
                en += o * o;
            }
        }
    }
    if (MIX && energy) {
        double v[8] = {(double)en[0] * 1.0001, (double)en[1] * 1.0001, (double)en[2] * 1.0001, (double)en[3] * 1.0001, 0, 0, 0, 0};
        block_fold<4>(q, ri, active, v);
        if (active && ri == 0) {
#pragma unroll
            for (int e = 0; e < 4; ++e) atomic_add_f64(energy + (long)c4 * 4 + e, v[e]);
        }
    }
    if (MIX) {
        __shared__ double sm[NT / 64];
        acc = ud_wave_sum_d(acc);
        if ((threadIdx.x & 63) == 0) sm[threadIdx.x >> 6] = acc;
        __syncthreads();
        if (threadIdx.x == 0) {
            double tot = 0.0;
            for (int i = 0; i < NT / 64; ++i) tot += sm[i];
            atomic_add_f64(dalpha_acc + ((blockIdx.x + 7 * blockIdx.y + 13 * blockIdx.z) & 63), tot);
        }
    }
    ud_absmax_commit(mo, amax);
}

__global__ void gate_grad_from_acc_kernel(const double* __restrict__ acc, const float* __restrict__ alpha,
                                          float* __restrict__ out) {
    double t = ud_wave_sum_d(acc[threadIdx.x]);
    if (threadIdx.x == 0) {
        const double a = 1.0 / (1.0 + exp(-(double)alpha[0]));
        out[0] = (float)(t * a * (1.0 - a));
    }
}

template <typename T>
__global__ __launch_bounds__(NT) void se_scale_bwd_bn_kernel(RedGeom q, const T* __restrict__ dc,
                                                             const T* __restrict__ x, ud_bn_ref bn,
                                                             const float* __restrict__ s, const float* __restrict__ dpool,
                                                             float inv_hw, T* __restrict__ dzo,
                                                             double* __restrict__ s1, double* __restrict__ s2,
                                                             double* __restrict__ part) {
    int ri, c4;
    const bool active = thread_coords(q, ri, c4);
    const In4<T> x4{x}, d4{dc};
    const Out4<T> o4{dzo};
    double v[8] = {0, 0, 0, 0, 0, 0, 0, 0};
    if (active) {
        const Bn4 cb = bn_load(bn, blockIdx.z, q.C4, c4, false);
        f32x4 gate = reinterpret_cast<const f32x4*>(s)[(long)blockIdx.z * q.C4 + c4];
        f32x4 dp = reinterpret_cast<const f32x4*>(dpool)[(long)blockIdx.z * q.C4 + c4] * inv_hw;
#pragma unroll
        for (int e = 0; e < 4; ++e) gate[e] = ud_sigmoid_fast(gate[e]);
        Rows w = rows_of(q, ri, c4);
#pragma unroll kRowUnroll<T>
        for (; w.r < w.r_end; w.r += q.rpi, w.idx += w.step) {
            f32x4 a = x4[w.idx], d = d4[w.idx], dz;
#pragma unroll
            for (int e = 0; e < 4; ++e) {
                const float xh = (a[e] - cb.mu[e]) * cb.is[e];
                float g = d[e] * gate[e] + dp[e];
                if (bn.act) g *= ud_act_grad_fast(cb.ga[e] * xh + cb.be[e], bn.act);
                g = ud_rounded<T>(g);
                dz[e] = g;
                v[e] += (double)g;
                v[4 + e] += (double)g * (double)xh;
            }
            o4.st(w.idx, dz);
        }
    }
    red_out<8>(q, ri, active, c4, v, s1, s2, part, false);
}

template <typename T>
__global__ __launch_bounds__(NT) void se_scale_bwd_bn_eval_kernel(RedGeom q, const T* __restrict__ dc, const T* __restrict__ x,
                                                                  ud_bn_ref bn, const float* __restrict__ s,
                                                                  const float* __restrict__ dpool, float inv_hw,
                                                                  T* __restrict__ ddo) {
    int ri, c4;
    if (!thread_coords(q, ri, c4)) return;
    const In4<T> x4{x}, d4{dc};
    const Out4<T> o4{ddo};
    const Bn4 cb = bn_load(bn, blockIdx.z, q.C4, c4, false);
    f32x4 gate = reinterpret_cast<const f32x4*>(s)[(long)blockIdx.z * q.C4 + c4];
    const f32x4 dp = reinterpret_cast<const f32x4*>(dpool)[(long)blockIdx.z * q.C4 + c4] * inv_hw;
    const f32x4 k = cb.ga * cb.is;
#pragma unroll
    for (int e = 0; e < 4; ++e) gate[e] = ud_sigmoid_fast(gate[e]);
    Rows w = rows_of(q, ri, c4);
#pragma unroll kRowUnroll<T>
    for (; w.r < w.r_end; w.r += q.rpi, w.idx += w.step) {
        const f32x4 a = x4[w.idx], d = d4[w.idx];
        f32x4 o;
#pragma unroll
        for (int e = 0; e < 4; ++e) {
            float g = d[e] * gate[e] + dp[e];
            if (bn.act) g *= ud_act_grad_fast(cb.ga[e] * ((a[e] - cb.mu[e]) * cb.is[e]) + cb.be[e], bn.act);
            o[e] = g * k[e];
        }
        o4.st(w.idx, o);
    }
}

template <typename T>
__global__ __launch_bounds__(NT) void bn_eval_bwd_kernel(RedGeom q, const T* __restrict__ dy, const T* __restrict__ x, ud_bn_ref bn,
                                                         T* __restrict__ dx) {
    int ri, c4;
    if (!thread_coords(q, ri, c4)) return;
    const In4<T> x4{x}, d4{dy};
    const Out4<T> o4{dx};
    const Bn4 cb = bn_load(bn, blockIdx.z, q.C4, c4, false);
    const f32x4 k = cb.ga * cb.is;
    Rows w = rows_of(q, ri, c4);
    if (bn.act) {
#pragma unroll kRowUnroll<T>
        for (; w.r < w.r_end; w.r += q.rpi, w.idx += w.step) {
            const f32x4 a = x4[w.idx];
            f32x4 o = d4[w.idx] * k;
#pragma unroll
            for (int e = 0; e < 4; ++e) o[e] *= ud_act_grad_fast(cb.ga[e] * ((a[e] - cb.mu[e]) * cb.is[e]) + cb.be[e], bn.act);
            o4.st(w.idx, o);
        }
    } else {
#pragma unroll kRowUnroll<T>
        for (; w.r < w.r_end; w.r += q.rpi, w.idx += w.step) o4.st(w.idx, d4[w.idx] * k);
    }
}

__device__ __forceinline__ float dpre_of(const double* dgate, const float* s2, long i) {
    const float g = ud_sigmoid_fast(s2[i]);
    return (float)dgate[i] * g * (1.f - g);
}

template <int IP>
__global__ __launch_bounds__(NT) void se_bwd_a_kernel(const double* __restrict__ dgate, const float* __restrict__ s2,
                                                      const float* __restrict__ s1, const float* __restrict__ We,
                                                      double* __restrict__ ds1_acc, float* __restrict__ dWe,
                                                      float* __restrict__ dbe, int N, int C, int Cs) {
    constexpr int NSL = NT / IP;
    constexpr int CH = 32 * NSL;
    __shared__ float sh[NT];
    __shared__ float red[NT];
    const int i = threadIdx.x % IP, sl = threadIdx.x / IP;
    const int chunks = (C + CH - 1) / CH;
    if ((int)blockIdx.x < N * chunks) {
        const int n = blockIdx.x / chunks, c0 = (blockIdx.x % chunks) * CH;
        const int cn = min(CH, C - c0);
        if ((int)threadIdx.x < cn) sh[threadIdx.x] = dpre_of(dgate, s2, (long)n * C + c0 + threadIdx.x);
        __syncthreads();
        float acc = 0.f;
        if (i < Cs) {
#pragma unroll 4
            for (int c = sl; c < cn; c += NSL) acc += sh[c] * We[(long)(c0 + c) * Cs + i];
        }
        red[threadIdx.x] = acc;
        __syncthreads();
        if (sl == 0 && i < Cs) {
            for (int k = 1; k < NSL; ++k) acc += red[k * IP + i];
            unsafeAtomicAdd(ds1_acc + (long)n * Cs + i, (double)acc);
        }
        return;
    }
    const int wb = blockIdx.x - N * chunks;
    const int c = wb * NSL + sl;
    const bool own = c < C && i < Cs;
    float acc = 0.f, accb = 0.f;
    for (int n0 = 0; n0 < N; n0 += IP) {
        const int nn = min(IP, N - n0);
        __syncthreads();
        {
            const int cc = c;
            sh[sl * IP + i] = (cc < C && i < nn) ? dpre_of(dgate, s2, (long)(n0 + i) * C + cc) : 0.f;
        }
        __syncthreads();
        if (own) {
#pragma unroll 8
            for (int n = 0; n < nn; ++n) {
                const float g = sh[sl * IP + n];
                acc += g * ud_act_fast(s1[(long)(n0 + n) * Cs + i], 1);
                accb += g;
            }
        }
    }
    if (!own) return;
    dWe[(long)c * Cs + i] = acc;
    if (i == 0) dbe[c] = accb;
}

__global__ __launch_bounds__(NT) void se_bwd_b_kernel(const double* __restrict__ ds1_acc, const float* __restrict__ s1,
                                                      const float* __restrict__ Wr, const double* __restrict__ pool,
                                                      float pool_scale, float* __restrict__ dpool,
                                                      float* __restrict__ dWr, float* __restrict__ dbr, int N, int C,
                                                      int Cs) {
    __shared__ float sh[NT];
    const int c = blockIdx.x * NT + threadIdx.x;
    if ((int)blockIdx.y < N) {
        const int n = blockIdx.y;
        if ((int)threadIdx.x < Cs)
            sh[threadIdx.x] = (float)ds1_acc[(long)n * Cs + threadIdx.x] * ud_act_grad_fast(s1[(long)n * Cs + threadIdx.x], 1);
        __syncthreads();
        if (c >= C) return;
        float acc = 0.f;
#pragma unroll 8
        for (int i = 0; i < Cs; ++i) acc += sh[i] * Wr[(long)i * C + c];
        dpool[(long)n * C + c] = acc;
        return;
    }
    const int i = blockIdx.y - N;
    if ((int)threadIdx.x < N)
        sh[threadIdx.x] = (float)ds1_acc[(long)threadIdx.x * Cs + i] * ud_act_grad_fast(s1[(long)threadIdx.x * Cs + i], 1);
    __syncthreads();
    if (blockIdx.x == 0 && threadIdx.x == 0) {
        float b = 0.f;
        for (int n = 0; n < N; ++n) b += sh[n];
        dbr[i] = b;
    }
    if (c >= C) return;
    float acc = 0.f;
#pragma unroll 8
    for (int n = 0; n < N; ++n) acc += sh[n] * ((float)pool[(long)n * C + c] * pool_scale);
    dWr[(long)i * C + c] = acc;
}

struct DwGeom {
    int N, H, W, C4, Ho, Wo, stride, pad_t, pad_l;
};
constexpr int TW = 8;

template <typename T, int K, bool STRIP, bool BN>
__global__ __launch_bounds__(NT) void dw_bwd_data_ex_kernel(RedGeom q, DwGeom d, const T* __restrict__ dy,
                                                            const float* __restrict__ gate_alpha, int gate_mode,
                                                            const float* __restrict__ wt, const T* __restrict__ add,
                                                            const T* __restrict__ x, ud_bn_ref bn,
                                                            T* __restrict__ out, double* __restrict__ s1,
                                                            double* __restrict__ s2, double* __restrict__ part) {
    constexpr int TWB = STRIP ? TW : 1;
    constexpr int NCOL = TWB + K - 1;
    int ri, c4;
    const bool active = thread_coords(q, ri, c4);
    const In4<T> dy4{dy}, add4{add}, x4{x};
    const f32x4* w4 = reinterpret_cast<const f32x4*>(wt);
    const Out4<T> o4{out};
    double v[8] = {0, 0, 0, 0, 0, 0, 0, 0};
    if (active) {
        Bn4 cb;
        if (BN) cb = bn_load(bn, 0, q.C4, c4, false);
        const float gs = gate_factor(gate_alpha, gate_mode);
        const int WB = (d.W + TWB - 1) / TWB;
        Rows it = rows_of(q, ri, c4);
        for (; it.r < it.r_end; it.r += q.rpi) {
            const int wb = it.r % WB;
            const int t2 = it.r / WB;
            const int h = t2 % d.H, n = t2 / d.H;
            const int w0 = wb * TWB;
            f32x4 acc[TWB];
#pragma unroll
            for (int t = 0; t < TWB; ++t) acc[t] = f32x4{0, 0, 0, 0};
            if (STRIP) {
                const int col0 = w0 + d.pad_l - (K - 1);
#pragma unroll
                for (int kh = 0; kh < K; ++kh) {
                    const int ho = h + d.pad_t - kh;
                    if (ho < 0 || ho >= d.Ho) continue;
                    const In4<T> row = dy4 + ((((long)n * d.Ho + ho) * d.Wo) * q.C4 + c4);
                    f32x4 g[NCOL], w[K];
#pragma unroll
                    for (int j = 0; j < NCOL; ++j) {
                        const int wo = col0 + j;
                        g[j] = (wo >= 0 && wo < d.Wo) ? row[(long)wo * q.C4] : f32x4{0, 0, 0, 0};
                    }
#pragma unroll
                    for (int kw = 0; kw < K; ++kw) w[kw] = w4[(kh * K + kw) * q.C4 + c4];
#pragma unroll
                    for (int t = 0; t < TWB; ++t)
#pragma unroll
                        for (int kw = 0; kw < K; ++kw) acc[t] += g[t - kw + K - 1] * w[kw];
                }
            } else {
#pragma unroll
                for (int kh = 0; kh < K; ++kh) {
                    const int th = h + d.pad_t - kh;
                    if (th < 0 || (th % d.stride) != 0) continue;
                    const int ho = th / d.stride;
                    if (ho >= d.Ho) continue;
#pragma unroll
                    for (int kw = 0; kw < K; ++kw) {
                        const int tw = w0 + d.pad_l - kw;
                        if (tw < 0 || (tw % d.stride) != 0) continue;
                        const int wo = tw / d.stride;
                        if (wo >= d.Wo) continue;
                        acc[0] += dy4[(((long)n * d.Ho + ho) * d.Wo + wo) * q.C4 + c4] * w4[(kh * K + kw) * q.C4 + c4];
                    }
                }
            }
            const long o0 = (((long)n * d.H + h) * d.W + w0) * q.C4 + c4;
#pragma unroll
            for (int t = 0; t < TWB; ++t) {
                if (w0 + t >= d.W) continue;
                const long o = o0 + (long)t * q.C4;
                f32x4 da = acc[t] * gs;
                if (add) da += add4[o];
                if (BN) {
                    const f32x4 a = x4[o];
#pragma unroll
                    for (int e = 0; e < 4; ++e) {
                        const float xh = (a[e] - cb.mu[e]) * cb.is[e];
                        float g = da[e];
                        if (bn.act) g *= ud_act_grad_fast(cb.ga[e] * xh + cb.be[e], bn.act);
                        g = ud_rounded<T>(g);
                        da[e] = g;
                        v[e] += (double)g;
                        v[4 + e] += (double)g * (double)xh;
                    }
                }
                o4.st(o, da);
            }
        }
    }
    if (BN) red_out<8>(q, ri, active, c4, v, s1, s2, part, false);
}

template <typename T, int K, int S>
__global__ __launch_bounds__(NT) void dw_bwd_weight_rows_ex(DwGeom q, int C, int rows_per_group, const T* __restrict__ x,
                                      const T* __restrict__ dy, float* __restrict__ part) {
    constexpr int CPL = sizeof(T) == 2 ? 2 : 1;
    typedef T VT __attribute__((ext_vector_type(CPL == 2 ? 2 : 1)));
    typedef float VF __attribute__((ext_vector_type(CPL == 2 ? 2 : 1)));
    const int c = (blockIdx.y * blockDim.x + threadIdx.x) * CPL;
    if (c >= C) return;
    const int p = blockIdx.x;
    const int rows_total = q.N * q.Ho;
    const int row0 = p * rows_per_group;
    int row1 = row0 + rows_per_group;
    if (row1 > rows_total) row1 = rows_total;
    const VF zero = {};
    auto ld = [](const T* ptr) { return __builtin_convertvector(*reinterpret_cast<const VT*>(ptr), VF); };
    VF acc[K * K];
#pragma unroll
    for (int i = 0; i < K * K; ++i) acc[i] = zero;
    for (int row = row0; row < row1; ++row) {
        const int n = row / q.Ho, ho = row % q.Ho;
        const int ih0 = ho * S - q.pad_t;
        const T* xr[K];
        bool vh[K];
#pragma unroll
        for (int kh = 0; kh < K; ++kh) {
            const int ih = ih0 + kh;
            vh[kh] = (ih >= 0) && (ih < q.H);
            xr[kh] = x + (((long)n * q.H + (vh[kh] ? ih : 0)) * q.W) * C + c;
        }
        VF w[K][K];
#pragma unroll
        for (int kh = 0; kh < K; ++kh)
#pragma unroll
            for (int kw = 0; kw < K; ++kw) {
                const int iw = kw - q.pad_l;
                w[kh][kw] = (vh[kh] && iw >= 0 && iw < q.W) ? ld(xr[kh] + (long)iw * C) : zero;
            }
        const T* dyr = dy + ((long)row * q.Wo) * C + c;
#pragma unroll 4
        for (int wo = 0; wo < q.Wo; ++wo) {
            const VF g = ld(dyr + (long)wo * C);
#pragma unroll
            for (int kh = 0; kh < K; ++kh)
#pragma unroll
                for (int kw = 0; kw < K; ++kw) acc[kh * K + kw] += g * w[kh][kw];
#pragma unroll
            for (int kh = 0; kh < K; ++kh) {
#pragma unroll
                for (int kw = 0; kw + S < K; ++kw) w[kh][kw] = w[kh][kw + S];
#pragma unroll
                for (int j = 0; j < S; ++j) {
                    const int iw = (wo + 1) * S - q.pad_l + (K - S) + j;
                    w[kh][K - S + j] = (vh[kh] && iw >= 0 && iw < q.W) ? ld(xr[kh] + (long)iw * C) : zero;
                }
            }
        }
    }
    float* out = part + (long)p * (K * K) * C + c;
#pragma unroll
    for (int i = 0; i < K * K; ++i) *reinterpret_cast<VF*>(out + (long)i * C) = acc[i];
}

__global__ __launch_bounds__(NT) void dw_bwd_weight_finalize_ex(int nparts, int KK, int C, const float* __restrict__ part,
                                                                const float* __restrict__ gate_alpha, int gate_mode,
                                                                float* __restrict__ dw) {
    const int KKC = KK * C;
    __shared__ double sm[16][16][4];
    const int lane = threadIdx.x & 15, sl = threadIdx.x >> 4;
    const int i = (blockIdx.x * 16 + lane) * 4;
    double a[4] = {0.0, 0.0, 0.0, 0.0};
    if (i < KKC) {
        const f32x4* p4 = reinterpret_cast<const f32x4*>(part + i);
        const long step = (long)KKC / 4;
        int p = sl;
        for (; p + 48 < nparts; p += 64) {
            const f32x4 v0 = p4[(long)p * step], v1 = p4[(long)(p + 16) * step];
            const f32x4 v2 = p4[(long)(p + 32) * step], v3 = p4[(long)(p + 48) * step];
#pragma unroll
            for (int e = 0; e < 4; ++e) a[e] += ((double)v0[e] + (double)v1[e]) + ((double)v2[e] + (double)v3[e]);
        }
        for (; p < nparts; p += 16) {
            const f32x4 v = p4[(long)p * step];
#pragma unroll
            for (int e = 0; e < 4; ++e) a[e] += (double)v[e];
        }
    }
#pragma unroll
    for (int e = 0; e < 4; ++e) sm[sl][lane][e] = a[e];
    __syncthreads();
    if (sl < 4 && i < KKC) {
        double t = 0.0;
#pragma unroll
        for (int k = 0; k < 16; ++k) t += sm[k][lane][sl];
        const int o = i + sl, tap = o / C, c = o % C;
        dw[(long)c * KK + tap] = (float)(t * (double)gate_factor(gate_alpha, gate_mode));
    }
}

inline bool dw_geom_ok(const DwGeom& q, int K) {
    return q.N > 0 && q.H > 0 && q.W > 0 && q.C4 > 0 && q.Ho > 0 && q.Wo > 0 && (q.stride == 1 || q.stride == 2) &&
           (K == 3 || K == 5);
}

inline bool shape_ok(int G, int R, int C) { return G >= 1 && R >= 1 && C >= 4 && C % 4 == 0; }

struct RedPlan {
    RedGeom q;
    bool use_part;
};
inline RedPlan plan_reduce(int G, int R, int C, bool per_group, const double* ws, int min_rows = 8,
                           int row_elems = 1) {
    constexpr int lim = 64;
    constexpr long big_elems = 1L << 20;
    RedGeom qa = make_geom_ex(G, R, C, 1024, lim, min_rows);
    const long contrib = per_group ? qa.P : (long)qa.G * qa.P;
    const bool big = !per_group && (long)G * R * row_elems * (C / 4) >= big_elems;
    if ((contrib <= lim && !big) || !ws) return RedPlan{qa, false};
    return RedPlan{make_geom_ex(G, R, C, 2048, 512, min_rows), true};
}
inline int finish_reduce(const RedPlan& pl, int nq, bool per_group, int C, const double* ws, double* a1, double* a2,
                         hipStream_t s) {
    if (!pl.use_part) return 0;
    const int G = per_group ? pl.q.G : 1;
    const int P = per_group ? pl.q.P : pl.q.G * pl.q.P;
    hipLaunchKernelGGL(partials_to_acc, dim3(ud_cdiv((long)G * C, 8)), dim3(NT), 0, s, nq, G, C, P, ws, a1, a2);
    UD_LAUNCH_CHECK();
    return 0;
}
inline RedGeom geom_ew(int G, int R, int C, int min_rows = 4) { return make_geom_ex(G, R, C, 2048, 4096, min_rows, 128); }

}

extern "C" {

long ud_fused_reduce_ws_doubles(int G, int R, int C, int per_group, int min_rows) {
    if (!shape_ok(G, R, C) || min_rows < 1) return UD_EINVAL;
    static double dummy;
    RedPlan pl = plan_reduce(G, R, C, per_group != 0, &dummy, min_rows);
    return pl.use_part ? 2L * pl.q.G * pl.q.P * C : 0;
}

int ud_stat_slots_fold(const double* slot_sum, const double* slot_sumsq, int slots, int N, double* acc_sum,
                       double* acc_sumsq, ud_stream_t stream) {
    if (!slot_sum || !slot_sumsq || slots < 1 || N < 1 || !acc_sum || !acc_sumsq) return UD_EINVAL;
    hipStream_t s = (hipStream_t)stream;
    if (slot_sumsq == slot_sum + (long)slots * N) {
        hipLaunchKernelGGL(partials_to_acc, dim3(ud_cdiv(N, 8)), dim3(NT), 0, s, 2, 1, N, slots, slot_sum, acc_sum, acc_sumsq);
    } else {
        hipLaunchKernelGGL(partials_to_acc, dim3(ud_cdiv(N, 8)), dim3(NT), 0, s, 1, 1, N, slots, slot_sum, acc_sum, nullptr);
        hipLaunchKernelGGL(partials_to_acc, dim3(ud_cdiv(N, 8)), dim3(NT), 0, s, 1, 1, N, slots, slot_sumsq, acc_sumsq, nullptr);
    }
    UD_LAUNCH_CHECK();
    return 0;
}

int ud_colstats(const void* x, int G, int R, int C, double* sum, double* sumsq, double* ws, int f16,
                ud_stream_t stream) {
    if (!shape_ok(G, R, C) || !x || !sum || !sumsq) return UD_EINVAL;
    hipStream_t s = (hipStream_t)stream;
    RedPlan pl = plan_reduce(G, R, C, G != 1, ws);
    UD_STORAGE_DISPATCH(f16, hipLaunchKernelGGL(colstats_kernel<T>, red_grid(pl.q), dim3(NT), 0, s, pl.q, (const T*)x, sum,
                                                sumsq, pl.use_part ? ws : nullptr));
    UD_LAUNCH_CHECK();
    return finish_reduce(pl, 2, G != 1, C, ws, sum, sumsq, s);
}

int ud_colsum_bn(const void* x, const ud_bn_ref* bn, int G, int R, int C, double* out, double* ws, int f16,
                 ud_stream_t stream) {
    if (!shape_ok(G, R, C) || !x || !bn || !out) return UD_EINVAL;
    hipStream_t s = (hipStream_t)stream;
    RedPlan pl = plan_reduce(G, R, C, true, ws);
    UD_STORAGE_DISPATCH(f16, hipLaunchKernelGGL((colsum_bn_kernel<T, false>), red_grid(pl.q), dim3(NT), 0, s, pl.q,
                                                (const T*)x, (const T*)nullptr, *bn, out, pl.use_part ? ws : nullptr,
                                                (uint32_t*)nullptr));
    UD_LAUNCH_CHECK();
    return finish_reduce(pl, 1, true, C, ws, out, nullptr, s);
}

int ud_colsum_bn_amax(const void* x, const ud_bn_ref* bn, int G, int R, int C, double* out, double* ws, uint32_t* absmax,
                      ud_stream_t stream) {
    if (!shape_ok(G, R, C) || !x || !bn || !out || !absmax) return UD_EINVAL;
    hipStream_t s = (hipStream_t)stream;
    RedPlan pl = plan_reduce(G, R, C, true, ws);
    hipLaunchKernelGGL((colsum_bn_kernel<float, false>), red_grid(pl.q), dim3(NT), 0, s, pl.q, (const float*)x,
                       (const float*)nullptr, *bn, out, pl.use_part ? ws : nullptr, absmax);
    UD_LAUNCH_CHECK();
    return finish_reduce(pl, 1, true, C, ws, out, nullptr, s);
}

int ud_coldot_bn(const void* dy, const void* x, const ud_bn_ref* bn, int G, int R, int C, double* out, double* ws,
                 int f16, ud_stream_t stream) {
    if (ud_bn_eval_form(bn)) return UD_EINVAL;
    if (!shape_ok(G, R, C) || !x || !dy || !bn || !out) return UD_EINVAL;
    hipStream_t s = (hipStream_t)stream;
    RedPlan pl = plan_reduce(G, R, C, true, ws);
    UD_STORAGE_DISPATCH(f16, hipLaunchKernelGGL((colsum_bn_kernel<T, true>), red_grid(pl.q), dim3(NT), 0, s, pl.q,
                                                (const T*)x, (const T*)dy, *bn, out, pl.use_part ? ws : nullptr,
                                                (uint32_t*)nullptr));
    UD_LAUNCH_CHECK();
    return finish_reduce(pl, 1, true, C, ws, out, nullptr, s);
}

int ud_fc_fwd_d(const double* xsum, float xscale, const float* W, const float* b, float* y, int N, int I, int O,
                ud_stream_t stream) {
    if (N < 1 || I < 1 || O < 1 || !xsum || !W || !y) return UD_EINVAL;
    long waves = (long)N * O;
    hipLaunchKernelGGL(fc_fwd_d_kernel, dim3(ud_cdiv(waves * 64, NT)), dim3(NT), 0, (hipStream_t)stream, xsum, xscale, W,
                       b, y, N, I, O);
    UD_LAUNCH_CHECK();
    return 0;
}

int ud_bn_apply(const void* x, const ud_bn_ref* bn, void* y, int G, int R, int C, int f16, ud_stream_t stream) {
    if (!shape_ok(G, R, C) || !x || !bn || !y) return UD_EINVAL;
    RedGeom q = geom_ew(G, R, C);
    UD_STORAGE_DISPATCH(f16, hipLaunchKernelGGL(bn_apply_kernel<T>, red_grid(q), dim3(NT), 0, (hipStream_t)stream, q,
                                                (const T*)x, *bn, (T*)y));
    UD_LAUNCH_CHECK();
    return 0;
}

int ud_se_scale_bn(const void* x, const ud_bn_ref* bn, const float* s, void* y, int G, int R, int C, int f16,
                   uint32_t* absmax, ud_stream_t stream) {
    if (!shape_ok(G, R, C) || !x || !bn || !s || !y) return UD_EINVAL;
    RedGeom q = geom_ew(G, R, C);
    UD_STORAGE_DISPATCH(f16, hipLaunchKernelGGL(se_scale_bn_kernel<T>, red_grid(q), dim3(NT), 0, (hipStream_t)stream, q,
                                                (const T*)x, *bn, s, (T*)y, absmax));
    UD_LAUNCH_CHECK();
    return 0;
}

int ud_se_scale_bn_planes(const void* x, const ud_bn_ref* bn, const float* s, uint16_t* planes, long panel_stride,
                          long plane_stride, float* inv_scale, const uint32_t* amax_in, int G, int R, int C,
                          ud_stream_t stream) {
    if (!shape_ok(G, R, C) || C % 32 || !x || !bn || !s || !planes || !inv_scale || !amax_in) return UD_EINVAL;
    if (panel_stride < (long)G * R * 32 || panel_stride % 8 || plane_stride % 8 || plane_stride < (long)(C / 32) * panel_stride)
        return UD_EINVAL;
    RedGeom q = geom_ew(G, R, C);
    hipLaunchKernelGGL(se_scale_bn_planes_kernel, red_grid(q), dim3(NT), 0, (hipStream_t)stream, q, (const float*)x, *bn, s,
                       planes, panel_stride, plane_stride, amax_in, inv_scale);
    UD_LAUNCH_CHECK();
    return 0;
}

int ud_residual_bn(const void* x, const ud_bn_ref* bn, const float* keep, float inv_keep, const void* skip,
                   void* out, int G, int R, int C, int f16, uint32_t* absmax, ud_stream_t stream) {
    if (!shape_ok(G, R, C) || !x || !bn || !out) return UD_EINVAL;
    RedGeom q = geom_ew(G, R, C);
    UD_STORAGE_DISPATCH(f16, hipLaunchKernelGGL(residual_bn_kernel<T>, red_grid(q), dim3(NT), 0, (hipStream_t)stream, q,
                                                (const T*)x, *bn, keep, inv_keep, (const T*)skip, (T*)out, absmax, ResPlanes{}));
    UD_LAUNCH_CHECK();
    return 0;
}

int ud_residual_bn_planes(const float* x, const ud_bn_ref* bn, const float* keep, float inv_keep, const float* skip,
                          const uint32_t* skip_absmax, float* out, uint16_t* planes, long panel_stride, long plane_stride,
                          float* inv_scale, int G, int R, int C, uint32_t* absmax, ud_stream_t stream) {
    if (!shape_ok(G, R, C) || !x || !bn || !out || !planes || !inv_scale || panel_stride < 32L * G * R ||
        plane_stride < panel_stride * ((C + 31) / 32) || (skip && !skip_absmax))
        return UD_EINVAL;
    RedGeom q = geom_ew(G, R, C);
    hipLaunchKernelGGL((residual_bn_kernel<float, 1>), red_grid(q), dim3(NT), 0, (hipStream_t)stream, q, x, *bn, keep, inv_keep,
                       skip, out, absmax, ResPlanes{planes, panel_stride, plane_stride, inv_scale, skip ? skip_absmax : nullptr});
    UD_LAUNCH_CHECK();
    return 0;
}

int ud_se_scale_bn_plane_half(const void* x, const ud_bn_ref* bn, const float* s, uint16_t* plane, long panel_stride,
                              float* inv_scale, int G, int R, int C, ud_stream_t stream) {
    if (!shape_ok(G, R, C) || !x || !bn || !s || !plane || !inv_scale || (bn->G != 1 && bn->G != G)) return UD_EINVAL;
    if (panel_stride < 32L * G * R) return UD_EINVAL;
    RedGeom q = geom_ew(G, R, C);
    hipLaunchKernelGGL(se_scale_bn_plane_half_kernel, red_grid(q), dim3(NT), 0, (hipStream_t)stream, q, (const _Float16*)x, *bn, s,
                       plane, panel_stride, inv_scale);
    UD_LAUNCH_CHECK();
    return 0;
}

int ud_normbwd_sums(const void* x, const void* dy, const float* keep, float inv_keep, const ud_bn_ref* bn,
                    int dy_is_dz, int G, int R, int C, double* s1, double* s2, double* s3, double* ws, int f16,
                    ud_stream_t stream) {
    if (ud_bn_eval_form(bn)) return UD_EINVAL;
    if (!shape_ok(G, R, C) || !x || !dy || !bn || !s1 || !s2 || bn->G != 1) return UD_EINVAL;
    hipStream_t s = (hipStream_t)stream;
    RedPlan pl = plan_reduce(G, R, C, false, ws);
    UD_STORAGE_DISPATCH(f16, hipLaunchKernelGGL(normbwd_sums_kernel<T>, red_grid(pl.q), dim3(NT), 0, s, pl.q, (const T*)x,
                                                (const T*)dy, keep, inv_keep, *bn, dy_is_dz, s1, s2, s3,
                                                pl.use_part ? ws : nullptr));
    UD_LAUNCH_CHECK();
    return finish_reduce(pl, 2, false, C, ws, s1, s2, s);
}

int ud_normbwd_apply(const void* x, const void* dy, const float* keep, float inv_keep, const ud_bn_ref* bn,
                     int dy_is_dz, const double* s1, const double* s2, const double* s1_local,
                     const double* s2_local, int G, int R, int C, void* dx, float* dgamma, float* dbeta, int f16,
                     uint32_t* absmax, ud_stream_t stream) {
    if (ud_bn_eval_form(bn)) return UD_EINVAL;
    if (!shape_ok(G, R, C) || !x || !dy || !bn || !s1 || !s2 || !dx || bn->G != 1) return UD_EINVAL;
    if ((dgamma || dbeta) && (!s1_local || !s2_local)) return UD_EINVAL;
    RedGeom q = geom_ew(G, R, C);
    UD_STORAGE_DISPATCH(f16, hipLaunchKernelGGL((normbwd_apply_kernel<T, false>), red_grid(q), dim3(NT), 0,
                                                (hipStream_t)stream, q, (const T*)x, (const T*)dy, keep, inv_keep, *bn,
                                                dy_is_dz, s1, s2, s1_local, s2_local, (const T*)nullptr, (T*)dx,
                                                (double*)nullptr, dgamma, dbeta, absmax, (double*)nullptr,
                                                PlanesDst{nullptr, 0, 0, nullptr, nullptr}));
    UD_LAUNCH_CHECK();
    return 0;
}

int ud_normbwd_apply_planes(const float* x, const float* dy, const float* keep, float inv_keep, const ud_bn_ref* bn,
                            int dy_is_dz, const double* s1, const double* s2, const double* s1_local,
                            const double* s2_local, const double* energy, int G, int R, int C, uint16_t* planes,
                            long panel_stride, long plane_stride, float* inv_scale, float* dgamma, float* dbeta,
                            ud_stream_t stream) {
    if (ud_bn_eval_form(bn)) return UD_EINVAL;
    if (!shape_ok(G, R, C) || !x || !dy || !bn || !s1 || !s2 || !energy || !planes || !inv_scale || bn->G != 1 || !bn->gamma)
        return UD_EINVAL;
    if ((dgamma || dbeta) && (!s1_local || !s2_local)) return UD_EINVAL;
    const long rows = (long)G * R;
    if (panel_stride < 32 * rows || plane_stride < (long)ud_cdiv(C, 32) * panel_stride) return UD_EINVAL;
    RedGeom q = geom_ew(G, R, C);
    hipLaunchKernelGGL((normbwd_apply_kernel<float, false, 1>), red_grid(q), dim3(NT), 0, (hipStream_t)stream, q, x, dy, keep,
                       inv_keep, *bn, dy_is_dz, s1, s2, s1_local, s2_local, (const float*)nullptr, (float*)nullptr,
                       (double*)nullptr, dgamma, dbeta, (uint32_t*)nullptr, (double*)nullptr,
                       PlanesDst{planes, panel_stride, plane_stride, inv_scale, energy});
    UD_LAUNCH_CHECK();
    return 0;
}

int ud_normbwd_apply_plane_half(const void* x, const void* dy, const float* keep, float inv_keep, const ud_bn_ref* bn,
                                int dy_is_dz, const double* s1, const double* s2, const double* s1_local,
                                const double* s2_local, int G, int R, int C, uint16_t* plane, long panel_stride,
                                float* inv_scale, float* dgamma, float* dbeta, ud_stream_t stream) {
    if (ud_bn_eval_form(bn)) return UD_EINVAL;
    if (!shape_ok(G, R, C) || !x || !dy || !bn || !s1 || !s2 || !plane || !inv_scale || bn->G != 1) return UD_EINVAL;
    if ((dgamma || dbeta) && (!s1_local || !s2_local)) return UD_EINVAL;
    if (panel_stride < 32L * G * R) return UD_EINVAL;
    RedGeom q = geom_ew(G, R, C);
    hipLaunchKernelGGL((normbwd_apply_kernel<_Float16, false, 2>), red_grid(q), dim3(NT), 0, (hipStream_t)stream, q,
                       (const _Float16*)x, (const _Float16*)dy, keep, inv_keep, *bn, dy_is_dz, s1, s2, s1_local, s2_local,
                       (const _Float16*)nullptr, (_Float16*)nullptr, (double*)nullptr, dgamma, dbeta, (uint32_t*)nullptr,
                       (double*)nullptr, PlanesDst{plane, panel_stride, 0, inv_scale, nullptr});
    UD_LAUNCH_CHECK();
    return 0;
}

int ud_normbwd_apply_mix(const void* x, const void* dz, const ud_bn_ref* bn, const double* s1, const double* s2,
                         const double* s1_local, const double* s2_local, const void* diff, int G, int R, int C,
                         void* dd, double* dalpha_acc, float* dgamma, float* dbeta, double* energy, int f16,
                         ud_stream_t stream) {
    if (ud_bn_eval_form(bn)) return UD_EINVAL;
    if (!shape_ok(G, R, C) || !x || !dz || !bn || !s1 || !s2 || !dd || !diff || !dalpha_acc || bn->G != 1)
        return UD_EINVAL;
    if ((dgamma || dbeta) && (!s1_local || !s2_local)) return UD_EINVAL;
    RedGeom q = make_geom_ex(G, R, C, 512, 4096, 4);
    UD_STORAGE_DISPATCH(f16, hipLaunchKernelGGL((normbwd_apply_kernel<T, true>), red_grid(q), dim3(NT), 0,
                                                (hipStream_t)stream, q, (const T*)x, (const T*)dz, (const float*)nullptr,
                                                1.f, *bn, 1, s1, s2, s1_local, s2_local, (const T*)diff, (T*)dd,
                                                dalpha_acc, dgamma, dbeta, (uint32_t*)nullptr, energy,
                                                PlanesDst{nullptr, 0, 0, nullptr, nullptr}));
    UD_LAUNCH_CHECK();
    return 0;
}

int ud_gate_grad_from_acc(const double* acc, const float* alpha, float* out, ud_stream_t stream) {
    if (!acc || !alpha || !out) return UD_EINVAL;
    hipLaunchKernelGGL(gate_grad_from_acc_kernel, dim3(1), dim3(64), 0, (hipStream_t)stream, acc, alpha, out);
    UD_LAUNCH_CHECK();
    return 0;
}

int ud_se_bwd_a(const double* dgate, const float* s2, const float* s1, const float* We, double* ds1_acc, float* dWe,
                float* dbe, int N, int C, int Cs, ud_stream_t stream) {
    if (N < 1 || C < 1 || Cs < 1 || Cs > 128 || !dgate || !s2 || !s1 || !We || !ds1_acc || (!dWe != !dbe)) return UD_EINVAL;
    hipStream_t s = (hipStream_t)stream;
    const int role1 = N * ud_cdiv(C, Cs <= 64 ? 32 * (NT / 64) : 32 * (NT / 128));
    const bool wg = dWe != nullptr;
    if (Cs <= 64) {
        dim3 grid((unsigned)(role1 + (wg ? ud_cdiv(C, NT / 64) : 0)));
        hipLaunchKernelGGL(se_bwd_a_kernel<64>, grid, dim3(NT), 0, s, dgate, s2, s1, We, ds1_acc, dWe, dbe, N, C, Cs);
    } else {
        dim3 grid((unsigned)(role1 + (wg ? ud_cdiv(C, NT / 128) : 0)));
        hipLaunchKernelGGL(se_bwd_a_kernel<128>, grid, dim3(NT), 0, s, dgate, s2, s1, We, ds1_acc, dWe, dbe, N, C, Cs);
    }
    UD_LAUNCH_CHECK();
    return 0;
}

int ud_se_bwd_b(const double* ds1_acc, const float* s1, const float* Wr, const double* pool, float pool_scale,
                float* dpool, float* dWr, float* dbr, int N, int C, int Cs, ud_stream_t stream) {
    const bool wg = dWr != nullptr;
    if (N < 1 || N > NT || C < 1 || Cs < 1 || Cs > NT || !ds1_acc || !s1 || !Wr || !dpool || (!dWr != !dbr) || (wg && !pool))
        return UD_EINVAL;
    dim3 grid((unsigned)ud_cdiv(C, NT), (unsigned)(N + (wg ? Cs : 0)));
    hipLaunchKernelGGL(se_bwd_b_kernel, grid, dim3(NT), 0, (hipStream_t)stream, ds1_acc, s1, Wr, pool, pool_scale, dpool,
                       dWr, dbr, N, C, Cs);
    UD_LAUNCH_CHECK();
    return 0;
}

int ud_se_scale_bwd_bn(const void* dc, const void* x, const ud_bn_ref* bn, const float* s, const float* dpool,
                       float inv_hw, void* dz, double* s1, double* s2, double* ws, int G, int R, int C, int f16,
                       ud_stream_t stream) {
    if (ud_bn_eval_form(bn)) return UD_EINVAL;
    if (!shape_ok(G, R, C) || !dc || !x || !bn || !s || !dpool || !dz || !s1 || !s2 || bn->G != 1) return UD_EINVAL;
    hipStream_t st = (hipStream_t)stream;
    RedPlan pl = plan_reduce(G, R, C, false, ws);
    UD_STORAGE_DISPATCH(f16, hipLaunchKernelGGL(se_scale_bwd_bn_kernel<T>, red_grid(pl.q), dim3(NT), 0, st, pl.q,
                                                (const T*)dc, (const T*)x, *bn, s, dpool, inv_hw, (T*)dz, s1, s2,
                                                pl.use_part ? ws : nullptr));
    UD_LAUNCH_CHECK();
    return finish_reduce(pl, 2, false, C, ws, s1, s2, st);
}

static RedGeom coldot_eval_geom(int G, int R, int C) { return make_geom_ex(G, R, C, 1024, 64, 8); }

long ud_coldot_bn_eval_ws_doubles(int G, int R, int C) {
    if (!shape_ok(G, R, C)) return UD_EINVAL;
    const RedGeom q = coldot_eval_geom(G, R, C);
    return q.P > 1 ? (long)q.G * q.P * C : 0;
}

int ud_coldot_bn_eval(const void* dy, const void* x, const ud_bn_ref* bn, int G, int R, int C, double* out, double* ws,
                      int f16, ud_stream_t stream) {
    if (!ud_bn_eval_form(bn) || bn->G != 1) return UD_EINVAL;
    if (!shape_ok(G, R, C) || !x || !dy || !out) return UD_EINVAL;
    const RedGeom q = coldot_eval_geom(G, R, C);
    const bool use_part = q.P > 1;
    if (use_part && !ws) return UD_EINVAL;
    hipStream_t s = (hipStream_t)stream;
    UD_STORAGE_DISPATCH(f16, hipLaunchKernelGGL((colsum_bn_kernel<T, true>), red_grid(q), dim3(NT), 0, s, q, (const T*)x,
                                                (const T*)dy, *bn, out, use_part ? ws : nullptr, (uint32_t*)nullptr));
    UD_LAUNCH_CHECK();
    if (use_part) {
        hipLaunchKernelGGL(partials_to_acc, dim3(ud_cdiv((long)G * C, 8)), dim3(NT), 0, s, 1, G, C, q.P, ws, out, nullptr);
        UD_LAUNCH_CHECK();
    }
    return 0;
}

int ud_se_scale_bwd_bn_eval(const void* dc, const void* x, const ud_bn_ref* bn, const float* s, const float* dpool,
                            float inv_hw, void* dd, int G, int R, int C, int f16, ud_stream_t stream) {
    if (!ud_bn_eval_form(bn) || bn->G != 1) return UD_EINVAL;
    if (!shape_ok(G, R, C) || !dc || !x || !s || !dpool || !dd) return UD_EINVAL;
    RedGeom q = geom_ew(G, R, C);
    UD_STORAGE_DISPATCH(f16, hipLaunchKernelGGL(se_scale_bwd_bn_eval_kernel<T>, red_grid(q), dim3(NT), 0, (hipStream_t)stream, q,
                                                (const T*)dc, (const T*)x, *bn, s, dpool, inv_hw, (T*)dd));
    UD_LAUNCH_CHECK();
    return 0;
}

int ud_bn_eval_bwd(const void* dy, const void* x, const ud_bn_ref* bn, void* dx, int G, int R, int C, int f16,
                   ud_stream_t stream) {
    if (!ud_bn_eval_form(bn) || bn->G != 1) return UD_EINVAL;
    if (!shape_ok(G, R, C) || !dy || !dx || (bn->act && !x) || bn->act < 0 || bn->act > 2) return UD_EINVAL;
    RedGeom q = geom_ew(G, R, C);
    UD_STORAGE_DISPATCH(f16, hipLaunchKernelGGL(bn_eval_bwd_kernel<T>, red_grid(q), dim3(NT), 0, (hipStream_t)stream, q,
                                                (const T*)dy, (const T*)x, *bn, (T*)dx));
    UD_LAUNCH_CHECK();
    return 0;
}

static long dw_bwd_items(int N, int H, int W, int stride) {
    return stride == 1 ? (long)N * H * ((W + TW - 1) / TW) : (long)N * H * W;
}
long ud_dwconv_bwd_data_bn_ws_doubles(int N, int H, int W, int C, int stride) {
    const long items = dw_bwd_items(N, H, W, stride);
    if (items < 1 || items > 0x7fffffffL || C % 4 || C < 4) return UD_EINVAL;
    static double dummy;
    RedPlan pl = plan_reduce(1, (int)items, C, false, &dummy, stride == 1 ? 1 : 4, stride == 1 ? TW : 1);
    return pl.use_part ? 2L * pl.q.G * pl.q.P * C : 0;
}

}

template <typename T>
static int dw_bwd_data_launch(const T* dy, const float* gate_alpha, int gate_mode, const float* wt, const T* add,
                              const T* x, const ud_bn_ref* bn, T* out, double* s1, double* s2, double* ws, int N,
                              int H, int W, int C, int Ho, int Wo, int K, int stride, int pad_t, int pad_l, hipStream_t s) {
    if (C % 4 || !dy || !wt || !out) return UD_EINVAL;
    DwGeom d{N, H, W, C / 4, Ho, Wo, stride, pad_t, pad_l};
    if (!dw_geom_ok(d, K)) return UD_EINVAL;
    const bool strip = stride == 1;
    const long items = dw_bwd_items(N, H, W, stride);
    if (items > 0x7fffffffL) return UD_EINVAL;
    ud_bn_ref none{};
    const bool has_bn = bn != nullptr;
    if (has_bn && (!x || !s1 || !s2 || bn->G != 1)) return UD_EINVAL;
    RedPlan pl{make_geom_ex(1, (int)items, C, 2048, 8192, strip ? 1 : 4), false};
    if (has_bn) pl = plan_reduce(1, (int)items, C, false, ws, strip ? 1 : 4, strip ? TW : 1);
    const RedGeom& q = pl.q;
    double* part = pl.use_part ? ws : nullptr;
    const ud_bn_ref& b = has_bn ? *bn : none;
#define UD_DW_BWD(KK, ST, BB)                                                                                        \
    hipLaunchKernelGGL((dw_bwd_data_ex_kernel<T, KK, ST, BB>), red_grid(q), dim3(NT), 0, s, q, d, dy, gate_alpha,    \
                       gate_mode, wt, add, x, b, out, s1, s2, part)
    if (K == 3) {
        if (strip) { if (has_bn) UD_DW_BWD(3, true, true); else UD_DW_BWD(3, true, false); }
        else { if (has_bn) UD_DW_BWD(3, false, true); else UD_DW_BWD(3, false, false); }
    } else {
        if (strip) { if (has_bn) UD_DW_BWD(5, true, true); else UD_DW_BWD(5, true, false); }
        else { if (has_bn) UD_DW_BWD(5, false, true); else UD_DW_BWD(5, false, false); }
    }
#undef UD_DW_BWD
    UD_LAUNCH_CHECK();
    return has_bn ? finish_reduce(pl, 2, false, C, ws, s1, s2, s) : 0;
}

extern "C" {

int ud_dwconv_bwd_data_bn(const void* dy, const float* gate_alpha, int gate_mode, const float* wt, const void* add,
                          const void* x, const ud_bn_ref* bn, void* dz, double* s1, double* s2, double* ws, int N,
                          int H, int W, int C, int Ho, int Wo, int K, int stride, int pad_t, int pad_l, int f16,
                          ud_stream_t stream) {
    if (ud_bn_eval_form(bn)) return UD_EINVAL;
    if (!bn) return UD_EINVAL;
    UD_STORAGE_DISPATCH(f16, return dw_bwd_data_launch<T>((const T*)dy, gate_alpha, gate_mode, wt, (const T*)add,
                                                          (const T*)x, bn, (T*)dz, s1, s2, ws, N, H, W, C, Ho, Wo, K,
                                                          stride, pad_t, pad_l, (hipStream_t)stream));
}

int ud_dwconv_bwd_data_ex(const void* dy, const float* gate_alpha, int gate_mode, const float* wt, const void* add,
                          void* dx, int N, int H, int W, int C, int Ho, int Wo, int K, int stride, int pad_t,
                          int pad_l, int f16, ud_stream_t stream) {
    UD_STORAGE_DISPATCH(f16, return dw_bwd_data_launch<T>((const T*)dy, gate_alpha, gate_mode, wt, (const T*)add,
                                                          (const T*)nullptr, nullptr, (T*)dx, nullptr, nullptr, nullptr,
                                                          N, H, W, C, Ho, Wo, K, stride, pad_t, pad_l,
                                                          (hipStream_t)stream));
}

int ud_dwconv_bwd_weight_ex(const void* x, const void* dy, const float* gate_alpha, int gate_mode, float* dwt,
                            float* part, int chunks, int N, int H, int W, int C, int Ho, int Wo, int K, int stride,
                            int pad_t, int pad_l, int f16, ud_stream_t stream) {
    if (C % 4 || chunks < 1 || !x || !dy || !dwt || !part) return UD_EINVAL;
    DwGeom q{N, H, W, C / 4, Ho, Wo, stride, pad_t, pad_l};
    if (!dw_geom_ok(q, K)) return UD_EINVAL;
    hipStream_t s = (hipStream_t)stream;
    const int rows_total = N * Ho;
    if (chunks > rows_total) return UD_EINVAL;
    const int rpg = (rows_total + chunks - 1) / chunks;
    const int lanes = f16 ? C / 2 : C;
    int bt = ((lanes < NT ? lanes : NT) + 63) / 64 * 64;
    dim3 grid((unsigned)chunks, (unsigned)ud_cdiv(lanes, bt), 1);
#define UD_DW_WG(KK, SS)                                                                                              \
    UD_STORAGE_DISPATCH(f16, hipLaunchKernelGGL((dw_bwd_weight_rows_ex<T, KK, SS>), grid, dim3(bt), 0, s, q, C, rpg,         \
                                                (const T*)x, (const T*)dy, part))
    if (K == 3 && stride == 1) UD_DW_WG(3, 1);
    else if (K == 3) UD_DW_WG(3, 2);
    else if (stride == 1) UD_DW_WG(5, 1);
    else UD_DW_WG(5, 2);
#undef UD_DW_WG
    UD_LAUNCH_CHECK();
    const int KKC = K * K * C;
    hipLaunchKernelGGL(dw_bwd_weight_finalize_ex, dim3(ud_cdiv(KKC, 64)), dim3(NT), 0, s, chunks, K * K, C, part,
                       gate_alpha, gate_mode, dwt);
    UD_LAUNCH_CHECK();
    return 0;
}

}
```

Baseline: 1361.

## Overlap BN stat loads with first row-group loads and specialize activation

BN parameter loading is split into an issue phase (raw sums, gamma, beta) and a finish phase, so the first group of row loads is in flight before the moments and rsqrt are computed. Row loops are rewritten as explicit groups of four loads followed by compute, with a scalar tail. The activation type becomes a compile-time template via a switch, which removes the runtime branch from inner loops. Running-stat updates move out of the hot path and gamma/beta loads are issued earlier in the FFT kernels. The cost is more code and register pressure from the grouped loads and extra template instantiations, and the contract-off multiplies slightly change rounding.

Measured after the change: 1394, median of 6. 2.4% higher.

```diff
diff --git a/unidefense_amd/csrc/bnref.h b/unidefense_amd/csrc/bnref.h
--- a/unidefense_amd/csrc/bnref.h
+++ b/unidefense_amd/csrc/bnref.h
@@ -5,37 +5,162 @@
 
 constexpr int NT = UD_COL_NT;
 
-template <typename T> constexpr int kRowUnroll = sizeof(T) == 2 ? 8 : 4;
+constexpr int kRowGroup = 4;
 
 __device__ __forceinline__ void atomic_add_f64(double* p, double v) { unsafeAtomicAdd(p, v); }
 
 struct Bn4 { f32x4 mu, is, ga, be; };
 
+#define UD_LAMBDA_INLINE __attribute__((always_inline))
+
+__device__ __forceinline__ float mul_rn(float a, float b) {
+#pragma clang fp contract(off)
+    return a * b;
+}
+__device__ __forceinline__ f32x4 mul_rn(const f32x4& a, const f32x4& b) {
+#pragma clang fp contract(off)
+    return a * b;
+}
+__device__ __forceinline__ f32x4 mul_rn(const f32x4& a, float b) {
+#pragma clang fp contract(off)
+    return a * b;
+}
+
+struct BnRaw {
+    double s[4], ss[4];
+    float rm[4], rv[4];
+    f32x4 ga, be;
+};
+
+__device__ __forceinline__ BnRaw bn_issue(const ud_bn_ref& b, int g, int C4, int c4) {
+    BnRaw r;
+    if (b.sum) {
+        const long i0 = ((long)(b.G == 1 ? 0 : g) * C4 + c4) * 4;
+#pragma unroll
+        for (int e = 0; e < 4; ++e) r.s[e] = b.sum[i0 + e];
+#pragma unroll
+        for (int e = 0; e < 4; ++e) r.ss[e] = b.sumsq[i0 + e];
+#pragma unroll
+        for (int e = 0; e < 4; ++e) r.rm[e] = r.rv[e] = 0.f;
+    } else {
+#pragma unroll
+        for (int e = 0; e < 4; ++e) r.rm[e] = b.running_mean[c4 * 4 + e];
+#pragma unroll
+        for (int e = 0; e < 4; ++e) r.rv[e] = b.running_var[c4 * 4 + e];
+#pragma unroll
+        for (int e = 0; e < 4; ++e) r.s[e] = r.ss[e] = 0.0;
+    }
+    r.ga = reinterpret_cast<const f32x4*>(b.gamma)[c4];
+    r.be = reinterpret_cast<const f32x4*>(b.beta)[c4];
+    return r;
+}
+
+__device__ __forceinline__ void bn_moments4(const ud_bn_ref& b, const BnRaw& r, double (&m)[4], double (&v)[4]) {
+    const bool train = b.sum != nullptr;
+#pragma unroll
+    for (int e = 0; e < 4; ++e) {
+        const double mt = r.s[e] * b.inv_count;
+        double vt = r.ss[e] * b.inv_count - mt * mt;
+        if (vt < 0.0) vt = 0.0;
+        m[e] = train ? mt : (double)r.rm[e];
+        v[e] = train ? vt : (double)r.rv[e];
+    }
+}
+
+__device__ __forceinline__ Bn4 bn_finish(const ud_bn_ref& b, const BnRaw& r) {
+    Bn4 o;
+    double m[4], v[4];
+    bn_moments4(b, r, m, v);
+#pragma unroll
+    for (int e = 0; e < 4; ++e) {
+        o.mu[e] = (float)m[e];
+        o.is[e] = rsqrtf((float)(v[e] + (double)b.eps));
+    }
+    o.ga = r.ga;
+    o.be = r.be;
+    return o;
+}
+
+__device__ __forceinline__ void bn_update_running(const ud_bn_ref& b, int g, int C4, int c4) {
+    if (!(b.sum && b.running_mean)) return;
+    const BnRaw r = bn_issue(b, g, C4, c4);
+    float rm[4], rv[4];
+#pragma unroll
+    for (int e = 0; e < 4; ++e) rm[e] = b.running_mean[c4 * 4 + e];
+#pragma unroll
+    for (int e = 0; e < 4; ++e) rv[e] = b.running_var[c4 * 4 + e];
+    double m[4], v[4];
+    bn_moments4(b, r, m, v);
+#pragma unroll
+    for (int e = 0; e < 4; ++e) {
+        rm[e] = mul_rn(1.f - b.momentum, rm[e]) + mul_rn(b.momentum, (float)m[e]);
+        rv[e] = mul_rn(1.f - b.momentum, rv[e]) + mul_rn(b.momentum, (float)(v[e] * b.unbias));
+    }
+#pragma unroll
+    for (int e = 0; e < 4; ++e) b.running_mean[c4 * 4 + e] = rm[e];
+#pragma unroll
+    for (int e = 0; e < 4; ++e) b.running_var[c4 * 4 + e] = rv[e];
+}
+
 __device__ __forceinline__ Bn4 bn_load(const ud_bn_ref& b, int g, int C4, int c4, bool update) {
-    Bn4 o;
-    const long i0 = ((long)(b.G == 1 ? 0 : g) * C4 + c4) * 4;
-#pragma unroll
-    for (int e = 0; e < 4; ++e) {
-        double m, v;
-        ud_bn_moments(b, i0 + e, c4 * 4 + e, m, v);
-        o.mu[e] = (float)m;
-        o.is[e] = rsqrtf((float)(v + (double)b.eps));
-        if (update && b.sum && b.running_mean) {
-            const int c = c4 * 4 + e;
-            b.running_mean[c] = (1.f - b.momentum) * b.running_mean[c] + b.momentum * (float)m;
-            b.running_var[c] = (1.f - b.momentum) * b.running_var[c] + b.momentum * (float)(v * b.unbias);
-        }
-    }
-    o.ga = reinterpret_cast<const f32x4*>(b.gamma)[c4];
-    o.be = reinterpret_cast<const f32x4*>(b.beta)[c4];
-    return o;
-}
-
+    const Bn4 o = bn_finish(b, bn_issue(b, g, C4, c4));
+    if (update) bn_update_running(b, g, C4, c4);
+    return o;
+}
+
+template <int ACT>
+__device__ __forceinline__ f32x4 bn_apply(const f32x4& a, const Bn4& b) {
+    f32x4 o;
+#pragma unroll
+    for (int e = 0; e < 4; ++e) o[e] = ud_act_fast(b.ga[e] * ((a[e] - b.mu[e]) * b.is[e]) + b.be[e], ACT);
+    return o;
+}
 __device__ __forceinline__ f32x4 bn_apply(const f32x4& a, const Bn4& b, int act) {
     f32x4 o;
 #pragma unroll
     for (int e = 0; e < 4; ++e) o[e] = ud_act_fast(b.ga[e] * ((a[e] - b.mu[e]) * b.is[e]) + b.be[e], act);
     return o;
+}
+
+template <int A> struct ActC { static constexpr int value = A; };
+template <typename F>
+__device__ __forceinline__ void act_switch(int act, F&& f) {
+    if (act == 1) f(ActC<1>{});
+    else if (act == 2) f(ActC<2>{});
+    else f(ActC<0>{});
+}
+
+template <typename T, int NIN, typename Fin, typename Body>
+__device__ __forceinline__ void for_rows(int r, int r_end, int rs, long idx, long step, const In4<T> (&in)[NIN], Fin&& fin,
+                                         Body&& body) {
+    constexpr int U = kRowGroup;
+    f32x4 v[U][NIN];
+    auto load = [&]() UD_LAMBDA_INLINE {
+#pragma unroll
+        for (int u = 0; u < U; ++u)
+#pragma unroll
+            for (int t = 0; t < NIN; ++t) v[u][t] = in[t][idx + u * step];
+    };
+    auto compute = [&]() UD_LAMBDA_INLINE {
+#pragma unroll
+        for (int u = 0; u < U; ++u) body(idx + u * step, r + u * rs, v[u]);
+        r += U * rs;
+        idx += U * step;
+    };
+    const bool full = r + (U - 1) * rs < r_end;
+    if (full) load();
+    fin();
+    if (full) compute();
+    while (r + (U - 1) * rs < r_end) {
+        load();
+        compute();
+    }
+    for (; r < r_end; r += rs, idx += step) {
+        f32x4 t[NIN];
+#pragma unroll
+        for (int k = 0; k < NIN; ++k) t[k] = in[k][idx];
+        body(idx, r, t);
+    }
 }
 
 __device__ __forceinline__ float gate_factor(const float* alpha, int mode) {
diff --git a/unidefense_amd/csrc/fft.hip b/unidefense_amd/csrc/fft.hip
--- a/unidefense_amd/csrc/fft.hip
+++ b/unidefense_amd/csrc/fft.hip
@@ -259,11 +259,11 @@
         float mu = 0.f, is = 1.f, ga = 1.f, be = 0.f;
         if (EX && has_bn) {
             double m, vv;
+            ga = bn.gamma[chl];
+            be = bn.beta[chl];
             ud_bn_moments(bn, chl, chl, m, vv);
             mu = (float)m;
             is = (float)(1.0 / sqrt(vv + (double)bn.eps));
-            ga = bn.gamma[chl];
-            be = bn.beta[chl];
             if (n == 0 && q == 0 && cok && bn.sum && bn.running_mean) {
                 bn.running_mean[ch] = (1.f - bn.momentum) * bn.running_mean[ch] + bn.momentum * (float)m;
                 bn.running_var[ch] = (1.f - bn.momentum) * bn.running_var[ch] + bn.momentum * (float)(vv * bn.unbias);
@@ -585,11 +585,11 @@
     float mu, is, ga, be;
     {
         double m, vv;
+        ga = bn.gamma[chl];
+        be = bn.beta[chl];
         ud_bn_moments(bn, chl, chl, m, vv);
         mu = (float)m;
         is = (float)(1.0 / sqrt(vv + (double)bn.eps));
-        ga = bn.gamma[chl];
-        be = bn.beta[chl];
     }
     __syncthreads();
     float* A = lds;
@@ -794,11 +794,11 @@
     float mu = 0.f, is = 1.f, ga = 1.f, be = 0.f;
     if (EX && has_bn) {
         double m, vv;
+        ga = bn.gamma[ch];
+        be = bn.beta[ch];
         ud_bn_moments(bn, ch, ch, m, vv);
         mu = (float)m;
         is = (float)(1.0 / sqrt(vv + (double)bn.eps));
-        ga = bn.gamma[ch];
-        be = bn.beta[ch];
         if (n == 0 && h == 0 && bn.sum && bn.running_mean) {
             bn.running_mean[ch] = (1.f - bn.momentum) * bn.running_mean[ch] + bn.momentum * (float)m;
             bn.running_var[ch] = (1.f - bn.momentum) * bn.running_var[ch] + bn.momentum * (float)(vv * bn.unbias);
@@ -1057,11 +1057,11 @@
     float mu = 0.f, is = 1.f, ga = 1.f, be = 0.f;
     if (EX && has_bn) {
         double m, vv;
+        ga = bn.gamma[chl];
+        be = bn.beta[chl];
         ud_bn_moments(bn, chl, chl, m, vv);
         mu = (float)m;
         is = (float)(1.0 / sqrt(vv + (double)bn.eps));
-        ga = bn.gamma[chl];
-        be = bn.beta[chl];
         if (n == 0 && wave == 0 && hh == 0 && cok && bn.sum && bn.running_mean) {
             bn.running_mean[ch] = (1.f - bn.momentum) * bn.running_mean[ch] + bn.momentum * (float)m;
             bn.running_var[ch] = (1.f - bn.momentum) * bn.running_var[ch] + bn.momentum * (float)(vv * bn.unbias);
diff --git a/unidefense_amd/csrc/fused.hip b/unidefense_amd/csrc/fused.hip
--- a/unidefense_amd/csrc/fused.hip
+++ b/unidefense_amd/csrc/fused.hip
@@ -85,21 +85,30 @@
     double v[8] = {0, 0, 0, 0, 0, 0, 0, 0};
     float mo = 0.f;
     if (active) {
-        const Bn4 cb = bn_load(bn, blockIdx.z, q.C4, c4, !DOT && is_updater(ri));
-        Rows w = rows_of(q, ri, c4);
-#pragma unroll kRowUnroll<T>
-        for (; w.r < w.r_end; w.r += q.rpi, w.idx += w.step) {
-            f32x4 a = bn_apply(x4[w.idx], cb, bn.act);
-            if (DOT) {
-                f32x4 d = d4[w.idx];
-#pragma unroll
-                for (int e = 0; e < 4; ++e) v[e] += (double)d[e] * (double)a[e];
+        const BnRaw raw = bn_issue(bn, blockIdx.z, q.C4, c4);
+        Bn4 cb;
+        const Rows w = rows_of(q, ri, c4);
+        auto fin = [&]() UD_LAMBDA_INLINE { cb = bn_finish(bn, raw); };
+        act_switch(bn.act, [&](auto ac) UD_LAMBDA_INLINE {
+            constexpr int ACT = decltype(ac)::value;
+            if constexpr (DOT) {
+                const In4<T> in[2] = {x4, d4};
+                for_rows<T, 2>(w.r, w.r_end, q.rpi, w.idx, w.step, in, fin, [&](long, int, const f32x4(&t)[2]) UD_LAMBDA_INLINE {
+                    const f32x4 a = bn_apply<ACT>(t[0], cb);
+#pragma unroll
+                    for (int e = 0; e < 4; ++e) v[e] += (double)t[1][e] * (double)a[e];
+                });
             } else {
-#pragma unroll
-                for (int e = 0; e < 4; ++e) v[e] += (double)a[e];
-                mo = fmaxf(mo, fmaxf(fmaxf(fabsf(a[0]), fabsf(a[1])), fmaxf(fabsf(a[2]), fabsf(a[3]))));
-            }
-        }
+                const In4<T> in[1] = {x4};
+                for_rows<T, 1>(w.r, w.r_end, q.rpi, w.idx, w.step, in, fin, [&](long, int, const f32x4(&t)[1]) UD_LAMBDA_INLINE {
+                    const f32x4 a = bn_apply<ACT>(t[0], cb);
+#pragma unroll
+                    for (int e = 0; e < 4; ++e) v[e] += (double)a[e];
+                    mo = fmaxf(mo, fmaxf(fmaxf(fabsf(a[0]), fabsf(a[1])), fmaxf(fabsf(a[2]), fabsf(a[3]))));
+                });
+            }
+        });
+        if (!DOT && is_updater(ri)) bn_update_running(bn, blockIdx.z, q.C4, c4);
     }
     red_out<4>(q, ri, active, c4, v, out, nullptr, part, true);
     if (!DOT) ud_absmax_commit(mo, amax);
@@ -127,17 +136,24 @@
     if (thread_coords(q, ri, c4)) {
         const In4<T> x4{x};
         const Out4<T> y4{y};
-        const Bn4 cb = bn_load(bn, blockIdx.z, q.C4, c4, false);
+        const BnRaw raw = bn_issue(bn, blockIdx.z, q.C4, c4);
         f32x4 gate = reinterpret_cast<const f32x4*>(s)[(long)blockIdx.z * q.C4 + c4];
-#pragma unroll
-        for (int e = 0; e < 4; ++e) gate[e] = ud_sigmoid_fast(gate[e]);
-        Rows w = rows_of(q, ri, c4);
-#pragma unroll kRowUnroll<T>
-        for (; w.r < w.r_end; w.r += q.rpi, w.idx += w.step) {
-            const f32x4 v = bn_apply(x4[w.idx], cb, bn.act) * gate;
-            y4.st(w.idx, v);
-            m = fmaxf(m, fmaxf(fmaxf(fabsf(v[0]), fabsf(v[1])), fmaxf(fabsf(v[2]), fabsf(v[3]))));
-        }
+        Bn4 cb;
+        const Rows w = rows_of(q, ri, c4);
+        const In4<T> in[1] = {x4};
+        auto fin = [&]() UD_LAMBDA_INLINE {
+            cb = bn_finish(bn, raw);
+#pragma unroll
+            for (int e = 0; e < 4; ++e) gate[e] = ud_sigmoid_fast(gate[e]);
+        };
+        act_switch(bn.act, [&](auto ac) UD_LAMBDA_INLINE {
+            constexpr int ACT = decltype(ac)::value;
+            for_rows<T, 1>(w.r, w.r_end, q.rpi, w.idx, w.step, in, fin, [&](long idx, int, const f32x4(&t)[1]) UD_LAMBDA_INLINE {
+                const f32x4 v = bn_apply<ACT>(t[0], cb) * gate;
+                y4.st(idx, v);
+                m = fmaxf(m, fmaxf(fmaxf(fabsf(v[0]), fabsf(v[1])), fmaxf(fabsf(v[2]), fabsf(v[3]))));
+            });
+        });
     }
     ud_absmax_commit(m, amax);
 }
@@ -146,6 +162,14 @@
                                                                 const float* __restrict__ s, uint16_t* __restrict__ planes,
                                                                 long panel, long plane, const uint32_t* __restrict__ amax_in,
                                                                 float* __restrict__ inv_scale) {
+    int ri, c4;
+    const bool active = thread_coords(q, ri, c4);
+    BnRaw raw{};
+    f32x4 gate = {0.f, 0.f, 0.f, 0.f};
+    if (active) {
+        raw = bn_issue(bn, blockIdx.z, q.C4, c4);
+        gate = reinterpret_cast<const f32x4*>(s)[(long)blockIdx.z * q.C4 + c4];
+    }
     uint32_t mb = 0;
 #pragma unroll
     for (int i = 0; i < 4; ++i) mb = max(mb, amax_in[(threadIdx.x & 63) + 64 * i]);
@@ -154,26 +178,36 @@
     float ps, pinv;
     ud_h2_scale(mb, ps, pinv);
     if (blockIdx.x == 0 && blockIdx.y == 0 && blockIdx.z == 0 && threadIdx.x == 0) *inv_scale = pinv;
-    int ri, c4;
-    if (!thread_coords(q, ri, c4)) return;
-    const In4<float> x4{x};
-    const Bn4 cb = bn_load(bn, blockIdx.z, q.C4, c4, false);
-    f32x4 gate = reinterpret_cast<const f32x4*>(s)[(long)blockIdx.z * q.C4 + c4];
-#pragma unroll
-    for (int e = 0; e < 4; ++e) gate[e] = ud_sigmoid_fast(gate[e]) * ps;
-    Rows w = rows_of(q, ri, c4);
+    if (!active) return;
+    const In4<float> in[1] = {In4<float>{x}};
+    Bn4 cb;
+    const Rows w = rows_of(q, ri, c4);
     uint16_t* o = planes + (long)(c4 >> 3) * panel + (c4 & 7) * 4;
-    long row = (long)blockIdx.z * q.R + w.r;
-#pragma unroll 4
-    for (; w.r < w.r_end; w.r += q.rpi, w.idx += w.step, row += q.rpi) {
-        const f32x4 v = bn_apply(x4[w.idx], cb, bn.act) * gate;
-        uint16_t h0[4], h1[4];
-#pragma unroll
-        for (int e = 0; e < 4; ++e) ud_split_h2(v[e], h0[e], h1[e]);
-        typedef unsigned short u16x4 __attribute__((ext_vector_type(4)));
-        *reinterpret_cast<u16x4*>(o + row * 32) = u16x4{h0[0], h0[1], h0[2], h0[3]};
-        *reinterpret_cast<u16x4*>(o + row * 32 + plane) = u16x4{h1[0], h1[1], h1[2], h1[3]};
-    }
+    const long row0 = (long)blockIdx.z * q.R;
+    auto fin = [&]() UD_LAMBDA_INLINE {
+        cb = bn_finish(bn, raw);
+#pragma unroll
+        for (int e = 0; e < 4; ++e) gate[e] = ud_sigmoid_fast(gate[e]) * ps;
+    };
+    act_switch(bn.act, [&](auto ac) UD_LAMBDA_INLINE {
+        constexpr int ACT = decltype(ac)::value;
+        for_rows<float, 1>(w.r, w.r_end, q.rpi, w.idx, w.step, in, fin, [&](long, int r, const f32x4(&t)[1]) UD_LAMBDA_INLINE {
+            const f32x4 a = bn_apply<ACT>(t[0], cb);
+            const long row = row0 + r;
+            uint16_t h0[4], h1[4];
+#pragma unroll
+            for (int e = 0; e < 2; ++e) ud_split_h2(mul_rn(a[e], gate[e]), h0[e], h1[e]);
+#pragma unroll
+            for (int e = 2; e < 4; ++e) {
+                const _Float16 top = (_Float16)mul_rn(a[e], gate[e]);
+                h0[e] = __builtin_bit_cast(uint16_t, top);
+                h1[e] = __builtin_bit_cast(uint16_t, (_Float16)mul_rn(__builtin_fmaf(a[e], gate[e], -(float)top), 2048.f));
+            }
+            typedef unsigned short u16x4 __attribute__((ext_vector_type(4)));
+            *reinterpret_cast<u16x4*>(o + row * 32) = u16x4{h0[0], h0[1], h0[2], h0[3]};
+            *reinterpret_cast<u16x4*>(o + row * 32 + plane) = u16x4{h1[0], h1[1], h1[2], h1[3]};
+        });
+    });
 }
 
 __global__ __launch_bounds__(NT) void se_scale_bn_plane_half_kernel(RedGeom q, const _Float16* __restrict__ x, ud_bn_ref bn,
@@ -183,21 +217,28 @@
     int ri, c4;
     if (!thread_coords(q, ri, c4)) return;
     typedef unsigned short u16x4 __attribute__((ext_vector_type(4)));
-    const In4<_Float16> x4{x};
-    const Bn4 cb = bn_load(bn, blockIdx.z, q.C4, c4, false);
+    const In4<_Float16> in[1] = {In4<_Float16>{x}};
+    const BnRaw raw = bn_issue(bn, blockIdx.z, q.C4, c4);
     f32x4 gate = reinterpret_cast<const f32x4*>(s)[(long)blockIdx.z * q.C4 + c4];
-#pragma unroll
-    for (int e = 0; e < 4; ++e) gate[e] = ud_sigmoid_fast(gate[e]);
-    Rows w = rows_of(q, ri, c4);
+    Bn4 cb;
+    const Rows w = rows_of(q, ri, c4);
     uint16_t* o = plane + (long)(c4 >> 3) * panel + (c4 & 7) * 4;
     const int npad = (c4 == q.C4 - 1) ? 7 - (c4 & 7) : 0;
-    long row = (long)blockIdx.z * q.R + w.r;
-#pragma unroll 4
-    for (; w.r < w.r_end; w.r += q.rpi, w.idx += w.step, row += q.rpi) {
-        const f32x4 v = bn_apply(x4[w.idx], cb, bn.act) * gate;
-        Quad<_Float16>::st(reinterpret_cast<_Float16*>(o + row * 32), 0, v);
-        for (int z = 1; z <= npad; ++z) *reinterpret_cast<u16x4*>(o + row * 32 + 4 * z) = u16x4{0, 0, 0, 0};
-    }
+    const long row0 = (long)blockIdx.z * q.R;
+    auto fin = [&]() UD_LAMBDA_INLINE {
+        cb = bn_finish(bn, raw);
+#pragma unroll
+        for (int e = 0; e < 4; ++e) gate[e] = ud_sigmoid_fast(gate[e]);
+    };
+    act_switch(bn.act, [&](auto ac) UD_LAMBDA_INLINE {
+        constexpr int ACT = decltype(ac)::value;
+        for_rows<_Float16, 1>(w.r, w.r_end, q.rpi, w.idx, w.step, in, fin, [&](long, int r, const f32x4(&t)[1]) UD_LAMBDA_INLINE {
+            const f32x4 v = bn_apply<ACT>(t[0], cb) * gate;
+            const long row = row0 + r;
+            Quad<_Float16>::st(reinterpret_cast<_Float16*>(o + row * 32), 0, v);
+            for (int z = 1; z <= npad; ++z) *reinterpret_cast<u16x4*>(o + row * 32 + 4 * z) = u16x4{0, 0, 0, 0};
+        });
+    });
 }
 
 struct ResPlanes {
@@ -212,6 +253,14 @@
                                                          const float* __restrict__ keep, float inv_keep,
                                                          const T* __restrict__ skip, T* __restrict__ out,
                                                          uint32_t* __restrict__ amax, ResPlanes rp) {
+    int ri, c4;
+    const bool active = thread_coords(q, ri, c4);
+    BnRaw raw{};
+    float kraw = 0.f;
+    if (active) {
+        raw = bn_issue(bn, blockIdx.z, q.C4, c4);
+        if (keep) kraw = keep[blockIdx.z];
+    }
     float ps = 1.f;
     if constexpr (PL == 1) {
         __shared__ float pl_red[NT / 64];
@@ -241,25 +290,28 @@
         ud_h2_scale(__float_as_uint((gm + sk) * 1.001f), ps, pinv);
         if (blockIdx.x == 0 && blockIdx.y == 0 && blockIdx.z == 0 && threadIdx.x == 0) *rp.inv_scale = pinv;
     }
-    int ri, c4;
     float m = 0.f;
-    if (thread_coords(q, ri, c4)) {
-        const In4<T> x4{x}, k4{skip};
+    if (active) {
         const Out4<T> o4{out};
-        const Bn4 cb = bn_load(bn, blockIdx.z, q.C4, c4, is_updater(ri));
-        const float sc = keep ? keep[blockIdx.z] * inv_keep : 1.f;
-        Rows w = rows_of(q, ri, c4);
+        Bn4 cb;
+        float sc = 1.f;
+        const Rows w = rows_of(q, ri, c4);
         uint16_t* po = PL ? rp.buf + (long)(c4 >> 3) * rp.panel + (c4 & 7) * 4 : nullptr;
         const int npad = (PL && c4 == q.C4 - 1) ? 7 - (c4 & 7) : 0;
-        long prow = (long)blockIdx.z * q.R + w.r;
-#pragma unroll kRowUnroll<T>
-        for (; w.r < w.r_end; w.r += q.rpi, w.idx += w.step, prow += q.rpi) {
-            f32x4 v = bn_apply(x4[w.idx], cb, bn.act) * sc;
-            if (skip) v += k4[w.idx];
-            o4.st(w.idx, v);
+        const long prow0 = (long)blockIdx.z * q.R;
+        auto fin = [&]() UD_LAMBDA_INLINE {
+            cb = bn_finish(bn, raw);
+            if (keep) sc = kraw * inv_keep;
+        };
+        auto row = [&](auto ac, const f32x4& t, const f32x4* k, long idx, int r) UD_LAMBDA_INLINE {
+            constexpr int ACT = decltype(ac)::value;
+            f32x4 v = mul_rn(bn_apply<ACT>(t, cb), sc);
+            if (k) v += *k;
+            o4.st(idx, v);
             m = fmaxf(m, fmaxf(fmaxf(fabsf(v[0]), fabsf(v[1])), fmaxf(fabsf(v[2]), fabsf(v[3]))));
             if constexpr (PL == 1) {
                 typedef unsigned short u16x4 __attribute__((ext_vector_type(4)));
+                const long prow = prow0 + r;
                 uint16_t h0[4], h1[4];
 #pragma unroll
                 for (int e = 0; e < 4; ++e) ud_split_h2(v[e] * ps, h0[e], h1[e]);
@@ -270,7 +322,21 @@
                     *reinterpret_cast<u16x4*>(po + prow * 32 + 4 * z + rp.plane) = u16x4{0, 0, 0, 0};
                 }
             }
-        }
+        };
+        act_switch(bn.act, [&](auto ac) UD_LAMBDA_INLINE {
+            if (skip) {
+                const In4<T> in[2] = {In4<T>{x}, In4<T>{skip}};
+                for_rows<T, 2>(w.r, w.r_end, q.rpi, w.idx, w.step, in, fin, [&](long idx, int r, const f32x4(&t)[2]) UD_LAMBDA_INLINE {
+                    row(ac, t[0], &t[1], idx, r);
+                });
+            } else {
+                const In4<T> in[1] = {In4<T>{x}};
+                for_rows<T, 1>(w.r, w.r_end, q.rpi, w.idx, w.step, in, fin, [&](long idx, int r, const f32x4(&t)[1]) UD_LAMBDA_INLINE {
+                    row(ac, t[0], nullptr, idx, r);
+                });
+            }
+        });
+        if (is_updater(ri)) bn_update_running(bn, blockIdx.z, q.C4, c4);
     }
     ud_absmax_commit(m, amax);
 }
@@ -280,26 +346,38 @@
                                                       T* __restrict__ y) {
     int ri, c4;
     if (!thread_coords(q, ri, c4)) return;
-    const In4<T> x4{x};
+    const In4<T> in[1] = {In4<T>{x}};
     const Out4<T> y4{y};
-    const Bn4 cb = bn_load(bn, blockIdx.z, q.C4, c4, is_updater(ri));
-    Rows w = rows_of(q, ri, c4);
-#pragma unroll kRowUnroll<T>
-    for (; w.r < w.r_end; w.r += q.rpi, w.idx += w.step) y4.st(w.idx, bn_apply(x4[w.idx], cb, bn.act));
-}
-
-__device__ __forceinline__ void dz_terms(const f32x4& a, const f32x4& d, const Bn4& cb, int act, bool is_dz, float sc,
-                                         f32x4& dz, f32x4& xh) {
+    const BnRaw raw = bn_issue(bn, blockIdx.z, q.C4, c4);
+    Bn4 cb;
+    const Rows w = rows_of(q, ri, c4);
+    auto fin = [&]() UD_LAMBDA_INLINE { cb = bn_finish(bn, raw); };
+    act_switch(bn.act, [&](auto ac) UD_LAMBDA_INLINE {
+        constexpr int ACT = decltype(ac)::value;
+        for_rows<T, 1>(w.r, w.r_end, q.rpi, w.idx, w.step, in, fin,
+                       [&](long idx, int, const f32x4(&t)[1]) UD_LAMBDA_INLINE { y4.st(idx, bn_apply<ACT>(t[0], cb)); });
+    });
+    if (is_updater(ri)) bn_update_running(bn, blockIdx.z, q.C4, c4);
+}
+
+constexpr int kDz = -1;
+template <int MODE>
+__device__ __forceinline__ void dz_terms(const f32x4& a, const f32x4& d, const Bn4& cb, float sc, f32x4& dz, f32x4& xh) {
 #pragma unroll
     for (int e = 0; e < 4; ++e) {
         xh[e] = (a[e] - cb.mu[e]) * cb.is[e];
         float g = d[e];
-        if (!is_dz) {
-            g *= sc;
-            if (act) g *= ud_act_grad_fast(cb.ga[e] * xh[e] + cb.be[e], act);
+        if (MODE != kDz) {
+            g = mul_rn(g, sc);
+            if (MODE) g = mul_rn(g, ud_act_grad_fast(cb.ga[e] * xh[e] + cb.be[e], MODE));
         }
         dz[e] = g;
     }
+}
+template <typename F>
+__device__ __forceinline__ void dz_switch(int dy_is_dz, int act, F&& f) {
+    if (dy_is_dz) f(ActC<kDz>{});
+    else act_switch(act, f);
 }
 
 template <typename T>
@@ -314,20 +392,29 @@
     double v[8] = {0, 0, 0, 0, 0, 0, 0, 0};
     f32x4 en = {0.f, 0.f, 0.f, 0.f};
     if (active) {
-        const Bn4 cb = bn_load(bn, blockIdx.z, q.C4, c4, false);
-        const float sc = keep ? keep[blockIdx.z] * inv_keep : 1.f;
-        Rows w = rows_of(q, ri, c4);
-#pragma unroll kRowUnroll<T>
-        for (; w.r < w.r_end; w.r += q.rpi, w.idx += w.step) {
-            f32x4 dz, xh;
-            dz_terms(x4[w.idx], d4[w.idx], cb, bn.act, dy_is_dz != 0, sc, dz, xh);
-#pragma unroll
-            for (int e = 0; e < 4; ++e) {
-                v[e] += (double)dz[e];
-                v[4 + e] += (double)dz[e] * (double)xh[e];
-            }
-            en += dz * dz;
-        }
+        const BnRaw raw = bn_issue(bn, blockIdx.z, q.C4, c4);
+        const float kraw = keep ? keep[blockIdx.z] : 0.f;
+        Bn4 cb;
+        float sc = 1.f;
+        const Rows w = rows_of(q, ri, c4);
+        const In4<T> in[2] = {x4, d4};
+        auto fin = [&]() UD_LAMBDA_INLINE {
+            cb = bn_finish(bn, raw);
+            if (keep) sc = kraw * inv_keep;
+        };
+        dz_switch(dy_is_dz, bn.act, [&](auto mc) UD_LAMBDA_INLINE {
+            constexpr int MODE = decltype(mc)::value;
+            for_rows<T, 2>(w.r, w.r_end, q.rpi, w.idx, w.step, in, fin, [&](long, int, const f32x4(&t)[2]) UD_LAMBDA_INLINE {
+                f32x4 dz, xh;
+                dz_terms<MODE>(t[0], t[1], cb, sc, dz, xh);
+#pragma unroll
+                for (int e = 0; e < 4; ++e) {
+                    v[e] += (double)dz[e];
+                    v[4 + e] += (double)dz[e] * (double)xh[e];
+                }
+                en += dz * dz;
+            });
+        });
     }
     if (s3) {
         double ev[8] = {(double)en[0] * 1.0001, (double)en[1] * 1.0001, (double)en[2] * 1.0001, (double)en[3] * 1.0001, 0, 0, 0, 0};
@@ -358,6 +445,19 @@
                                                            float* __restrict__ dgamma, float* __restrict__ dbeta,
                                                            uint32_t* __restrict__ amax, double* __restrict__ energy,
                                                            PlanesDst pd) {
+    int ri, c4;
+    const bool active = thread_coords(q, ri, c4);
+    BnRaw raw{};
+    double t1d[4] = {0, 0, 0, 0}, t2d[4] = {0, 0, 0, 0};
+    float kraw = 0.f;
+    if (active) {
+        raw = bn_issue(bn, blockIdx.z, q.C4, c4);
+#pragma unroll
+        for (int e = 0; e < 4; ++e) t1d[e] = s1[c4 * 4 + e];
+#pragma unroll
+        for (int e = 0; e < 4; ++e) t2d[e] = s2[c4 * 4 + e];
+        if (keep) kraw = keep[blockIdx.z];
+    }
     float ps = 1.f;
     if constexpr (PL == 2) {
         if (blockIdx.x == 0 && blockIdx.y == 0 && blockIdx.z == 0 && threadIdx.x == 0) *pd.inv_scale = 1.f;
@@ -382,47 +482,43 @@
         ud_h2_scale(__float_as_uint(sqrtf(gm) * 1.002f), ps, pinv);
         if (blockIdx.x == 0 && blockIdx.y == 0 && blockIdx.z == 0 && threadIdx.x == 0) *pd.inv_scale = pinv;
     }
-    int ri, c4;
-    const bool active = thread_coords(q, ri, c4);
     const In4<T> x4{x}, d4{dy}, fr4{freq};
     const Out4<T> o4{dx};
     double acc = 0.0;
     float mo = 0.f;
     f32x4 en = {0.f, 0.f, 0.f, 0.f};
     if (active) {
-        const Bn4 cb = bn_load(bn, blockIdx.z, q.C4, c4, false);
-        const float sc = keep ? keep[blockIdx.z] * inv_keep : 1.f;
-        f32x4 t1, t2;
-#pragma unroll
-        for (int e = 0; e < 4; ++e) {
-            t1[e] = (float)s1[c4 * 4 + e] * (float)bn.inv_count;
-            t2[e] = (float)s2[c4 * 4 + e] * (float)bn.inv_count;
-        }
-        if (is_updater(ri)) {
-#pragma unroll
-            for (int e = 0; e < 4; ++e) {
-                if (dbeta) dbeta[c4 * 4 + e] = (float)s1l[c4 * 4 + e];
-                if (dgamma) dgamma[c4 * 4 + e] = (float)s2l[c4 * 4 + e];
-            }
-        }
-        Rows w = rows_of(q, ri, c4);
+        Bn4 cb;
+        float sc = 1.f;
+        f32x4 t1, t2, k;
+        const Rows w = rows_of(q, ri, c4);
         uint16_t* po = PL ? pd.buf + (long)(c4 >> 3) * pd.panel + (c4 & 7) * 4 : nullptr;
         const int npad = (PL && c4 == q.C4 - 1) ? 7 - (c4 & 7) : 0;
-        long prow = (long)blockIdx.z * q.R + w.r;
-#pragma unroll kRowUnroll<T>
-        for (; w.r < w.r_end; w.r += q.rpi, w.idx += w.step, prow += q.rpi) {
+        const long prow0 = (long)blockIdx.z * q.R;
+        auto fin = [&]() UD_LAMBDA_INLINE {
+            cb = bn_finish(bn, raw);
+            if (keep) sc = kraw * inv_keep;
+            k = cb.ga * cb.is;
+#pragma unroll
+            for (int e = 0; e < 4; ++e) {
+                t1[e] = (float)t1d[e] * (float)bn.inv_count;
+                t2[e] = (float)t2d[e] * (float)bn.inv_count;
+            }
+        };
+        auto row = [&](auto mc, const f32x4& a, const f32x4& d, const f32x4* f, long idx, int r) UD_LAMBDA_INLINE {
+            constexpr int MODE = decltype(mc)::value;
             f32x4 dz, xh, o;
-            dz_terms(x4[w.idx], d4[w.idx], cb, bn.act, dy_is_dz != 0, sc, dz, xh);
-#pragma unroll
-            for (int e = 0; e < 4; ++e) o[e] = cb.ga[e] * cb.is[e] * (dz[e] - t1[e] - xh[e] * t2[e]);
+            dz_terms<MODE>(a, d, cb, sc, dz, xh);
+#pragma unroll
+            for (int e = 0; e < 4; ++e) o[e] = k[e] * __builtin_fmaf(-xh[e], t2[e], dz[e] - t1[e]);
             if constexpr (PL == 2) {
                 typedef unsigned short u16x4 __attribute__((ext_vector_type(4)));
+                const long prow = prow0 + r;
                 Quad<T>::st(reinterpret_cast<T*>(po + prow * 32), 0, o);
                 for (int z = 1; z <= npad; ++z) *reinterpret_cast<u16x4*>(po + prow * 32 + 4 * z) = u16x4{0, 0, 0, 0};
-                continue;
-            }
-            if constexpr (PL == 1) {
+            } else if constexpr (PL == 1) {
                 typedef unsigned short u16x4 __attribute__((ext_vector_type(4)));
+                const long prow = prow0 + r;
                 uint16_t h0[4], h1[4];
 #pragma unroll
                 for (int e = 0; e < 4; ++e) ud_split_h2(o[e] * ps, h0[e], h1[e]);
@@ -432,15 +528,34 @@
                     *reinterpret_cast<u16x4*>(po + prow * 32 + 4 * z) = u16x4{0, 0, 0, 0};
                     *reinterpret_cast<u16x4*>(po + prow * 32 + 4 * z + pd.plane) = u16x4{0, 0, 0, 0};
                 }
-                continue;
-            }
-            o4.st(w.idx, o);
-            mo = fmaxf(mo, fmaxf(fmaxf(fabsf(o[0]), fabsf(o[1])), fmaxf(fabsf(o[2]), fabsf(o[3]))));
-            if (MIX) {
-                f32x4 f = fr4[w.idx];
-#pragma unroll
-                for (int e = 0; e < 4; ++e) acc += (double)ud_rounded<T>(o[e]) * (double)f[e];
-                en += o * o;
+            } else {
+                o4.st(idx, o);
+                mo = fmaxf(mo, fmaxf(fmaxf(fabsf(o[0]), fabsf(o[1])), fmaxf(fabsf(o[2]), fabsf(o[3]))));
+                if constexpr (MIX) {
+#pragma unroll
+                    for (int e = 0; e < 4; ++e) acc += (double)ud_rounded<T>(o[e]) * (double)(*f)[e];
+                    en += o * o;
+                }
+            }
+        };
+        dz_switch(dy_is_dz, bn.act, [&](auto mc) UD_LAMBDA_INLINE {
+            if constexpr (MIX) {
+                const In4<T> in[3] = {x4, d4, fr4};
+                for_rows<T, 3>(w.r, w.r_end, q.rpi, w.idx, w.step, in, fin, [&](long idx, int r, const f32x4(&t)[3]) UD_LAMBDA_INLINE {
+                    row(mc, t[0], t[1], &t[2], idx, r);
+                });
+            } else {
+                const In4<T> in[2] = {x4, d4};
+                for_rows<T, 2>(w.r, w.r_end, q.rpi, w.idx, w.step, in, fin, [&](long idx, int r, const f32x4(&t)[2]) UD_LAMBDA_INLINE {
+                    row(mc, t[0], t[1], nullptr, idx, r);
+                });
+            }
+        });
+        if (is_updater(ri)) {
+#pragma unroll
+            for (int e = 0; e < 4; ++e) {
+                if (dbeta) dbeta[c4 * 4 + e] = (float)s1l[c4 * 4 + e];
+                if (dgamma) dgamma[c4 * 4 + e] = (float)s2l[c4 * 4 + e];
             }
         }
     }
@@ -488,27 +603,35 @@
     const Out4<T> o4{dzo};
     double v[8] = {0, 0, 0, 0, 0, 0, 0, 0};
     if (active) {
-        const Bn4 cb = bn_load(bn, blockIdx.z, q.C4, c4, false);
+        const BnRaw raw = bn_issue(bn, blockIdx.z, q.C4, c4);
         f32x4 gate = reinterpret_cast<const f32x4*>(s)[(long)blockIdx.z * q.C4 + c4];
-        f32x4 dp = reinterpret_cast<const f32x4*>(dpool)[(long)blockIdx.z * q.C4 + c4] * inv_hw;
-#pragma unroll
-        for (int e = 0; e < 4; ++e) gate[e] = ud_sigmoid_fast(gate[e]);
-        Rows w = rows_of(q, ri, c4);
-#pragma unroll kRowUnroll<T>
-        for (; w.r < w.r_end; w.r += q.rpi, w.idx += w.step) {
-            f32x4 a = x4[w.idx], d = d4[w.idx], dz;
-#pragma unroll
-            for (int e = 0; e < 4; ++e) {
-                const float xh = (a[e] - cb.mu[e]) * cb.is[e];
-                float g = d[e] * gate[e] + dp[e];
-                if (bn.act) g *= ud_act_grad_fast(cb.ga[e] * xh + cb.be[e], bn.act);
-                g = ud_rounded<T>(g);
-                dz[e] = g;
-                v[e] += (double)g;
-                v[4 + e] += (double)g * (double)xh;
-            }
-            o4.st(w.idx, dz);
-        }
+        f32x4 dp = reinterpret_cast<const f32x4*>(dpool)[(long)blockIdx.z * q.C4 + c4];
+        Bn4 cb;
+        const Rows w = rows_of(q, ri, c4);
+        const In4<T> in[2] = {x4, d4};
+        auto fin = [&]() UD_LAMBDA_INLINE {
+            cb = bn_finish(bn, raw);
+            dp = dp * inv_hw;
+#pragma unroll
+            for (int e = 0; e < 4; ++e) gate[e] = ud_sigmoid_fast(gate[e]);
+        };
+        act_switch(bn.act, [&](auto ac) UD_LAMBDA_INLINE {
+            constexpr int ACT = decltype(ac)::value;
+            for_rows<T, 2>(w.r, w.r_end, q.rpi, w.idx, w.step, in, fin, [&](long idx, int, const f32x4(&t)[2]) UD_LAMBDA_INLINE {
+                f32x4 dz;
+#pragma unroll
+                for (int e = 0; e < 4; ++e) {
+                    const float xh = (t[0][e] - cb.mu[e]) * cb.is[e];
+                    float g = t[1][e] * gate[e] + dp[e];
+                    if (ACT) g *= ud_act_grad_fast(cb.ga[e] * xh + cb.be[e], ACT);
+                    g = ud_rounded<T>(g);
+                    dz[e] = g;
+                    v[e] += (double)g;
+                    v[4 + e] += (double)g * (double)xh;
+                }
+                o4.st(idx, dz);
+            });
+        });
     }
     red_out<8>(q, ri, active, c4, v, s1, s2, part, false);
 }
@@ -522,25 +645,33 @@
     if (!thread_coords(q, ri, c4)) return;
     const In4<T> x4{x}, d4{dc};
     const Out4<T> o4{ddo};
-    const Bn4 cb = bn_load(bn, blockIdx.z, q.C4, c4, false);
+    const BnRaw raw = bn_issue(bn, blockIdx.z, q.C4, c4);
     f32x4 gate = reinterpret_cast<const f32x4*>(s)[(long)blockIdx.z * q.C4 + c4];
-    const f32x4 dp = reinterpret_cast<const f32x4*>(dpool)[(long)blockIdx.z * q.C4 + c4] * inv_hw;
-    const f32x4 k = cb.ga * cb.is;
-#pragma unroll
-    for (int e = 0; e < 4; ++e) gate[e] = ud_sigmoid_fast(gate[e]);
-    Rows w = rows_of(q, ri, c4);
-#pragma unroll kRowUnroll<T>
-    for (; w.r < w.r_end; w.r += q.rpi, w.idx += w.step) {
-        const f32x4 a = x4[w.idx], d = d4[w.idx];
-        f32x4 o;
-#pragma unroll
-        for (int e = 0; e < 4; ++e) {
-            float g = d[e] * gate[e] + dp[e];
-            if (bn.act) g *= ud_act_grad_fast(cb.ga[e] * ((a[e] - cb.mu[e]) * cb.is[e]) + cb.be[e], bn.act);
-            o[e] = g * k[e];
-        }
-        o4.st(w.idx, o);
-    }
+    f32x4 dp = reinterpret_cast<const f32x4*>(dpool)[(long)blockIdx.z * q.C4 + c4];
+    Bn4 cb;
+    f32x4 k;
+    const Rows w = rows_of(q, ri, c4);
+    const In4<T> in[2] = {x4, d4};
+    auto fin = [&]() UD_LAMBDA_INLINE {
+        cb = bn_finish(bn, raw);
+        dp = dp * inv_hw;
+        k = cb.ga * cb.is;
+#pragma unroll
+        for (int e = 0; e < 4; ++e) gate[e] = ud_sigmoid_fast(gate[e]);
+    };
+    act_switch(bn.act, [&](auto ac) UD_LAMBDA_INLINE {
+        constexpr int ACT = decltype(ac)::value;
+        for_rows<T, 2>(w.r, w.r_end, q.rpi, w.idx, w.step, in, fin, [&](long idx, int, const f32x4(&t)[2]) UD_LAMBDA_INLINE {
+            f32x4 o;
+#pragma unroll
+            for (int e = 0; e < 4; ++e) {
+                float g = t[1][e] * gate[e] + dp[e];
+                if (ACT) g *= ud_act_grad_fast(cb.ga[e] * ((t[0][e] - cb.mu[e]) * cb.is[e]) + cb.be[e], ACT);
+                o[e] = g * k[e];
+            }
+            o4.st(idx, o);
+        });
+    });
 }
 
 template <typename T>
@@ -550,21 +681,29 @@
     if (!thread_coords(q, ri, c4)) return;
     const In4<T> x4{x}, d4{dy};
     const Out4<T> o4{dx};
-    const Bn4 cb = bn_load(bn, blockIdx.z, q.C4, c4, false);
-    const f32x4 k = cb.ga * cb.is;
-    Rows w = rows_of(q, ri, c4);
+    const BnRaw raw = bn_issue(bn, blockIdx.z, q.C4, c4);
+    Bn4 cb;
+    f32x4 k;
+    const Rows w = rows_of(q, ri, c4);
+    auto fin = [&]() UD_LAMBDA_INLINE {
+        cb = bn_finish(bn, raw);
+        k = cb.ga * cb.is;
+    };
     if (bn.act) {
-#pragma unroll kRowUnroll<T>
-        for (; w.r < w.r_end; w.r += q.rpi, w.idx += w.step) {
-            const f32x4 a = x4[w.idx];
-            f32x4 o = d4[w.idx] * k;
-#pragma unroll
-            for (int e = 0; e < 4; ++e) o[e] *= ud_act_grad_fast(cb.ga[e] * ((a[e] - cb.mu[e]) * cb.is[e]) + cb.be[e], bn.act);
-            o4.st(w.idx, o);
-        }
+        const In4<T> in[2] = {x4, d4};
+        act_switch(bn.act, [&](auto ac) UD_LAMBDA_INLINE {
+            constexpr int ACT = decltype(ac)::value;
+            for_rows<T, 2>(w.r, w.r_end, q.rpi, w.idx, w.step, in, fin, [&](long idx, int, const f32x4(&t)[2]) UD_LAMBDA_INLINE {
+                f32x4 o = t[1] * k;
+#pragma unroll
+                for (int e = 0; e < 4; ++e) o[e] *= ud_act_grad_fast(cb.ga[e] * ((t[0][e] - cb.mu[e]) * cb.is[e]) + cb.be[e], ACT);
+                o4.st(idx, o);
+            });
+        });
     } else {
-#pragma unroll kRowUnroll<T>
-        for (; w.r < w.r_end; w.r += q.rpi, w.idx += w.step) o4.st(w.idx, d4[w.idx] * k);
+        const In4<T> in[1] = {d4};
+        for_rows<T, 1>(w.r, w.r_end, q.rpi, w.idx, w.step, in, fin,
+                       [&](long idx, int, const f32x4(&t)[1]) UD_LAMBDA_INLINE { o4.st(idx, t[0] * k); });
     }
 }
 
```
